# airl-iisc/MRFP

Measured on AMD Instinct MI355X. Metric: train images/sec, higher is better.
Workload: dtype bf16; 1 GPU; resnet-101 DeepLabV3+ + MRFP+ (HRFP+NP+ on, HRFP re-drawn every step), 768x768, 16 images/GPU, fwd+bwd+SGD, synthetic 19-class, random-init weights; global_batch=16, parallelism=dp1

## Files before the change

### include/mrfp_hip.h

```cpp
#ifndef MRFP_HIP_H
#define MRFP_HIP_H

#include <stdint.h>

#ifdef __cplusplus
extern "C" {
#endif

typedef enum { MRFP_F32 = 0, MRFP_BF16 = 1, MRFP_F16 = 2 } mrfp_dtype;

int mrfp_version(void);
const char* mrfp_last_error(void);

int64_t mrfp_stats_nslab(int64_t B, int64_t Ho);

int mrfp_stats_fwd(const void* x, int dtype, int64_t B, int64_t Ho, int64_t Wo, int64_t C,
                   int64_t Hs, int64_t Ws, const int32_t* tabH, const int32_t* tabW,
                   float* ws, void* stream);

int mrfp_stats_bwd(const void* dy, const void* x, const void* y, const float* mean,
                   const float* fA, const float* fS, int per_image, int dtype, int64_t B, int64_t Ho, int64_t Wo, int64_t C,
                   int64_t Hs, int64_t Ws, const int32_t* tabH, const int32_t* tabW,
                   float* ws, void* stream);
int mrfp_stats_bwd_mask(const void* dy, const void* x, const void* mask, const float* mean, int per_image, int dtype, int64_t B,
                        int64_t H, int64_t W, int64_t C, float* ws, void* stream);

int mrfp_bn_finalize(const float* ws, int64_t B, int64_t nslab, int64_t count, int64_t C,
                     const float* weight, const float* bias, float eps, float momentum,
                     float* running_mean, float* running_var,
                     float* mean, float* invstd, float* A, float* S, void* stream);
int mrfp_bn_eval_coef(int64_t C, const float* weight, const float* bias, const float* running_mean,
                      const float* running_var, float eps, float* A, float* S, void* stream);
int mrfp_bn_bwd_finalize(const float* ws, int64_t B, int64_t nslab, int64_t count, int64_t C,
                         const float* weight, const float* mean, const float* invstd,
                         float* dweight, float* dbias, float* P, float* Q, float* R, void* stream);

int mrfp_in_finalize(const float* ws, int64_t B, int64_t nslab, int64_t count, int64_t C,
                     const float* weight, const float* bias, float eps,
                     float* mean, float* invstd, float* A, float* S, void* stream);
int mrfp_in_bwd_finalize(const float* ws, int64_t B, int64_t nslab, int64_t count, int64_t C,
                         const float* weight, const float* mean, const float* invstd,
                         float* dweight, float* dbias, float* P, float* Q, float* R, void* stream);

int mrfp_np_finalize(const float* ws, int64_t B, int64_t nslab, int64_t count, int64_t C,
                     const float* alpha, const float* beta_noise,
                     float* mu, float* sigma, float* A, float* S, void* stream);
int mrfp_np_bwd_finalize(const float* ws, int64_t B, int64_t nslab, int64_t count, int64_t C,
                         const float* alpha, const float* beta_noise, const float* mu,
                         const float* sigma, float* Gtmp , float* K, void* stream);

int mrfp_mean_finalize(const float* ws, int64_t B, int64_t nslab, int64_t count, int64_t C,
                       float* tmp, void* out, int dtype, void* stream);

int mrfp_affine_fwd(const void* x, const void* res, void* y, int dtype,
                    int64_t B, int64_t Ho, int64_t Wo, int64_t C, int64_t Hs, int64_t Ws,
                    const int32_t* tabH, const int32_t* tabW,
                    const float* A, const float* S, int coef_per_image, int relu, void* stream);

int mrfp_affine_fwd_stats(const void* x, const void* res, void* y, int dtype, int64_t B, int64_t H, int64_t W, int64_t C,
                          const float* A, const float* S, int coef_per_image, int relu, float* ws, void* stream);
int mrfp_affine_bwd(const void* dy, const void* x, const void* y, void* dx, void* dres, int dtype,
                    int64_t B, int64_t Ho, int64_t Wo, int64_t C, int64_t Hs, int64_t Ws,
                    const int32_t* invH, const int32_t* invW,
                    const float* P, const float* Q, const float* R,
                    const float* fA, const float* fS, int coef_per_image, void* stream);
int mrfp_affine_fwd_relu_mask(const void* x, const void* res, void* y, void* mask, int dtype, int64_t B, int64_t H, int64_t W,
                              int64_t C, const float* A, const float* S, int coef_per_image, void* stream);
int mrfp_affine_bwd_mask(const void* dy, const void* x, const void* mask, void* dx, void* dres, int dtype, int64_t B, int64_t H,
                         int64_t W, int64_t C, const float* P, const float* Q, const float* R, int coef_per_image, void* stream);

int mrfp_copy_channels(const void* src, void* dst, int dtype, int64_t npix, int64_t C, int64_t ld_src, int64_t c0_src,
                       int64_t ld_dst, int64_t c0_dst, void* stream);

int mrfp_add(const void* a, const void* b, void* y, int dtype, int64_t n, void* stream);

int mrfp_bilinear_fwd(const void* x, const void* addend, void* y, int dtype,
                      int64_t B, int64_t Hi, int64_t Wi, int64_t Ho, int64_t Wo, int64_t C, int64_t ld_in,
                      void* stream);
int mrfp_bilinear_bwd(const void* dy, void* dx, int dtype,
                      int64_t B, int64_t Hi, int64_t Wi, int64_t Ho, int64_t Wo, int64_t C, int64_t ld_in,
                      void* stream);
int mrfp_bilinear_fwd_into(const void* x, void* y, int dtype, int64_t B, int64_t Hi, int64_t Wi, int64_t Ho, int64_t Wo,
                           int64_t C, int64_t ld_in, int64_t ld_out, void* stream);
int mrfp_bilinear_bwd_from(const void* dy, void* dx, int dtype, int64_t B, int64_t Hi, int64_t Wi, int64_t Ho, int64_t Wo,
                           int64_t C, int64_t ld_in, int64_t ld_dy, void* stream);

int mrfp_maxpool_fwd(const void* x, void* y, uint8_t* idx, int dtype,
                     int64_t B, int64_t H, int64_t W, int64_t C, void* stream);
int mrfp_maxpool_bwd(const void* dy, const uint8_t* idx, void* dx, int dtype,
                     int64_t B, int64_t H, int64_t W, int64_t C, void* stream);

int mrfp_maxpool_affine_fwd(const void* x, const float* A, const float* S, int coef_per_image, int relu, void* y, uint8_t* idx,
                            int dtype, int64_t B, int64_t H, int64_t W, int64_t C, void* stream);
int mrfp_pool_norm_bwd_stats(const void* dy, const uint8_t* idx, const void* x, const float* mean, const float* fA,
                             const float* fS, int coef_per_image, int relu, float* ws, int dtype,
                             int64_t B, int64_t H, int64_t W, int64_t C, void* stream);
int mrfp_pool_norm_bwd_apply(const void* dy, const uint8_t* idx, const void* x, const float* P, const float* Q, const float* R,
                             const float* fA, const float* fS, int coef_per_image, int relu, void* dx, int dtype,
                             int64_t B, int64_t H, int64_t W, int64_t C, void* stream);

int64_t mrfp_ce_nblocks(int64_t npix);
int mrfp_ce_fwd(const void* logits, const int64_t* target, int dtype, int64_t npix, int64_t C,
                int64_t ignore_index, float* ws, float* loss, void* stream);
int mrfp_ce_bwd(const void* logits, const int64_t* target, const float* loss, const float* gscale,
                void* dlogits, int dtype, int64_t npix, int64_t C, int64_t ignore_index, void* stream);

int mrfp_upsample_ce_fwd(const void* P, int64_t ld, const int64_t* target, int dtype, int64_t B, int64_t Hi, int64_t Wi,
                         int64_t H, int64_t W, int64_t C, int64_t ignore_index, float* ws, float* loss, void* stream);
int mrfp_upsample_ce_bwd(const void* P, int64_t ld, const int64_t* target, const float* loss, const float* gscale,
                         void* dlogits, int64_t Cd, int dtype, int64_t B, int64_t Hi, int64_t Wi, int64_t H, int64_t W,
                         int64_t C, int64_t ignore_index, void* stream);

typedef enum { MRFP_CE_MEAN = 0, MRFP_CE_SUM = 1, MRFP_CE_IMAGE_MEAN = 2 } mrfp_ce_mode;
int64_t mrfp_ce_w_nblocks(int64_t B, int64_t HW);
int64_t mrfp_ce_w_loss_floats(int64_t B, int mode);
int mrfp_ce_w_fwd(const void* logits, const int64_t* target, int dtype, int64_t B, int64_t HW, int64_t C,
                  int64_t ignore_index, const float* weight, int64_t wstride, float smoothing, int mode, float* ws,
                  float* loss, void* stream);
int mrfp_ce_w_bwd(const void* logits, const int64_t* target, const float* loss, const float* gscale, void* dlogits,
                  int dtype, int64_t B, int64_t HW, int64_t C, int64_t ignore_index, const float* weight, int64_t wstride,
                  float smoothing, int mode, void* stream);
int mrfp_upsample_ce_w_fwd(const void* P, int64_t ld, const int64_t* target, int dtype, int64_t B, int64_t Hi, int64_t Wi,
                           int64_t H, int64_t W, int64_t C, int64_t ignore_index, const float* weight, int64_t wstride,
                           float smoothing, int mode, float* ws, float* loss, void* stream);
int mrfp_upsample_ce_w_bwd(const void* P, int64_t ld, const int64_t* target, const float* loss, const float* gscale,
                           void* dlogits, int64_t Cd, int dtype, int64_t B, int64_t Hi, int64_t Wi, int64_t H, int64_t W,
                           int64_t C, int64_t ignore_index, const float* weight, int64_t wstride, float smoothing, int mode,
                           void* stream);

int mrfp_label_class_weights(const int64_t* target, int64_t B, int64_t HW, int64_t C, double upper_bound, int norm,
                             int batch, int64_t* counts_ws, float* weight_out, void* stream);

int64_t mrfp_relax_nblocks(int64_t B, int64_t H, int64_t W);
int mrfp_relax_labels(const int64_t* target, int64_t B, int64_t H, int64_t W, int64_t C, int64_t border, int strict_mask,
                      int32_t* words, int64_t* counts, void* stream);
int mrfp_multihot_pack(const uint8_t* multihot, int64_t B, int64_t HW, int64_t C, int32_t* words, int64_t* counts,
                       void* stream);
int mrfp_relax_word_counts(const int32_t* words, int64_t B, int64_t HW, int64_t C, int64_t* counts, void* stream);
int mrfp_relax_class_weights(const int64_t* counts, int64_t B, int64_t C, double upper_bound, int norm, int batch,
                             float* weight_out, void* stream);
int64_t mrfp_soft_nll_nblocks(int64_t B, int64_t HW);
int64_t mrfp_soft_nll_loss_floats(int64_t B);
int mrfp_soft_nll_fwd(const void* logits, const int32_t* words, int dtype, int64_t B, int64_t HW, int64_t C,
                      const float* weight, int64_t wstride, float* ws, float* loss, void* stream);
int mrfp_soft_nll_bwd(const void* logits, const int32_t* words, const float* loss, const float* gscale, void* dlogits,
                      int dtype, int64_t B, int64_t HW, int64_t C, const float* weight, int64_t wstride, void* stream);
int mrfp_upsample_soft_nll_fwd(const void* P, int64_t ld, const int32_t* words, int dtype, int64_t B, int64_t Hi, int64_t Wi,
                               int64_t H, int64_t W, int64_t C, const float* weight, int64_t wstride, float* ws, float* loss,
                               void* stream);
int mrfp_upsample_soft_nll_bwd(const void* P, int64_t ld, const int32_t* words, const float* loss, const float* gscale,
                               void* dlogits, int64_t Cd, int dtype, int64_t B, int64_t Hi, int64_t Wi, int64_t H, int64_t W,
                               int64_t C, const float* weight, int64_t wstride, void* stream);

int mrfp_argmax_hist(const void* logits, const int64_t* target, int dtype, int64_t npix, int64_t C,
                     int64_t* hist, uint8_t* pred, void* stream);

int mrfp_pack_weight(const float* w, void* wf, void* wd, int dtype, int64_t N, int64_t C, int64_t R, int64_t S,
                     int64_t Npad, int64_t Cpad, void* stream);
int mrfp_pack_weights_batched(const void* jobs, const int64_t* prefix, int64_t njobs, int64_t total, int dtype, void* stream);
int mrfp_conv_fwd(const void* x, const void* wpack, const float* bias, void* y, int dtype,
                  int64_t B, int64_t H, int64_t W, int64_t C, int64_t N, int64_t ldy, int64_t R, int64_t S,
                  int64_t Ho, int64_t Wo, int64_t stride, int64_t pad_h, int64_t pad_w, int64_t dil,
                  int64_t sstride, const void* addend, float* colstats, void* stream);
int mrfp_conv_fwd_act(const void* x, const void* wpack, const float* bias, void* y, int dtype,
                      int64_t B, int64_t H, int64_t W, int64_t C, int64_t N, int64_t ldy, int64_t R, int64_t S,
                      int64_t Ho, int64_t Wo, int64_t stride, int64_t pad_h, int64_t pad_w, int64_t dil,
                      int64_t sstride, const void* addend, int act, void* stream);
int mrfp_pack_weight_folded(const float* w, void* wf, const float* conv_bias, const float* bn_weight, const float* bn_bias,
                            const float* running_mean, const float* running_var, float eps, float* bias_out, int dtype,
                            int64_t N, int64_t C, int64_t R, int64_t S, int64_t Npad, int64_t Cpad, void* stream);
int mrfp_pack_weights_folded_batched(const void* jobs, const int64_t* prefix, int64_t njobs, int64_t total, int dtype, void* stream);
int mrfp_conv_stats_layout(int dtype, int64_t B, int64_t H, int64_t W, int64_t C, int64_t N, int64_t ldy, int64_t R, int64_t S,
                           int64_t Ho, int64_t Wo, int64_t stride, int64_t pad_h, int64_t pad_w, int64_t dil, int64_t sstride, int wstats,
                           int64_t* out);
int64_t mrfp_conv_stats_block_rows(int dtype, int64_t B, int64_t H, int64_t W, int64_t C, int64_t N, int64_t R, int64_t S, int64_t Ho,
                                   int64_t Wo, int64_t stride, int64_t pad_h, int64_t pad_w, int64_t dil, int64_t sstride);
int mrfp_conv_single_launch(int64_t B, int64_t image_bytes);
int mrfp_conv_fwd_wstats(const void* x, const void* wpack, const float* bias, void* y, int dtype,
                         int64_t B, int64_t H, int64_t W, int64_t C, int64_t N, int64_t ldy, int64_t R, int64_t S,
                         int64_t Ho, int64_t Wo, int64_t stride, int64_t pad_h, int64_t pad_w, int64_t dil,
                         const uint8_t* rowweight, float* colstats, void* stream);
int mrfp_conv_fwd_gated(const void* x, const void* wpack, const float* bias, void* y, int dtype,
                        int64_t B, int64_t H, int64_t W, int64_t C, int64_t N, int64_t ldy, int64_t R, int64_t S,
                        int64_t Ho, int64_t Wo, int64_t stride, int64_t pad_h, int64_t pad_w, int64_t dil,
                        int64_t sstride, const void* addend, const void* addend_mask, void* stream);
int mrfp_conv_fwd_lowrank(const void* x, const void* wpack, const float* bias, void* y, int dtype,
                          int64_t B, int64_t H, int64_t W, int64_t C, int64_t N, int64_t ldy, int64_t R, int64_t S,
                          int64_t Ho, int64_t Wo, int64_t stride, int64_t pad_h, int64_t pad_w, int64_t dil,
                          int64_t sstride, const void* addend, float* colstats, const void* lr_x, const void* lr_w, int64_t lr_k,
                          void* stream);
int mrfp_conv_lowrank_ok(int dtype, int64_t B, int64_t H, int64_t W, int64_t C, int64_t N, int64_t ldy, int64_t R, int64_t S,
                         int64_t Ho, int64_t Wo, int64_t stride, int64_t pad_h, int64_t pad_w, int64_t dil);
int mrfp_debug_clock_stamps(int family, uint64_t* out, int64_t n);
int64_t mrfp_conv_wgrad_ws_bytes(int64_t M, int64_t N, int64_t Q);
int mrfp_conv_wgrad(const void* x, const void* dy, float* dw, void* ws, int dtype,
                    int64_t B, int64_t H, int64_t W, int64_t C, int64_t Ctrue, int64_t N, int64_t ldn,
                    int64_t R, int64_t S, int64_t Ho, int64_t Wo, int64_t stride, int64_t pad_h, int64_t pad_w,
                    int64_t dil, void* stream);
int64_t mrfp_conv_wgrad_group_max(void);
int64_t mrfp_conv_wgrad_grouped_ws_bytes(int64_t M, int64_t N, int64_t Q, int64_t count);
int mrfp_conv_wgrad_plan(int dtype, int64_t B, int64_t H, int64_t W, int64_t C, int64_t N, int64_t ldn, int64_t R, int64_t S, int64_t Ho,
                         int64_t Wo, int64_t stride, int64_t pad_h, int64_t pad_w, int64_t dil, int64_t count, int64_t* out);
int mrfp_conv_wgrad_grouped(const void* const* xs, const void* const* dys, float* const* dws, int64_t count, void* ws, int dtype,
                            int64_t B, int64_t H, int64_t W, int64_t C, int64_t Ctrue, int64_t N, int64_t ldn,
                            int64_t R, int64_t S, int64_t Ho, int64_t Wo, int64_t stride, int64_t pad_h, int64_t pad_w,
                            int64_t dil, void* stream);
int mrfp_nchw_to_nhwc_pad(const float* x, void* y, int dtype, int64_t B, int64_t C, int64_t H, int64_t W,
                          int64_t Cpad, void* stream);

int mrfp_sgd_step(float* p, const float* g, float* m, int64_t n, float lr, float momentum,
                  float weight_decay, float gscale, int first, void* stream);

int64_t mrfp_grad_check_nblocks(int64_t n);
int mrfp_grad_check(const float* g, int64_t n, float gscale, void* ws, void* state, int dynamic, float growth,
                    float backoff, int growth_interval, float max_norm, void* stream);
int mrfp_sgd_step_checked(float* p, const float* g, float* m, int64_t n, float lr, float momentum,
                          float weight_decay, const void* state, void* stream);

int64_t mrfp_group_moments_ws_bytes(int64_t B, int64_t HW, int64_t C);
int mrfp_group_moments(const void* a, const void* b, float* M, float* sum_a, void* ws, int dtype, int64_t B, int64_t HW,
                       int64_t C, void* stream);
int mrfp_group_apply(const void* x, const float* Wm, const void* z, const float* Vm, const float* shift, void* y, int dtype,
                     int64_t B, int64_t HW, int64_t C, void* stream);
int mrfp_group_isqrt_fwd(const float* cov, float* wm, int64_t n, int T, void* stream);
int mrfp_group_isqrt_bwd(const float* cov, const float* dwm, float* dcov, int64_t n, int T, void* stream);

int64_t mrfp_fourier_spectrum_bytes(int64_t B, int64_t H, int64_t W, int64_t C);
int64_t mrfp_fourier_stored_bins(int64_t H, int64_t W, float radius, int high);
int mrfp_fourier_mix(const void* x, void* y, const int64_t* perm, void* S, void* S3, float* ratio, int load_ratio,
                     const void* twH, const void* twW, int dtype, int64_t B, int64_t H, int64_t W, int64_t C,
                     float radius, float lam, int high, void* stream);

int mrfp_resample_u8(const void* src, void* dst, int64_t Hin, int64_t Win, int64_t Hout, int64_t Wout, int64_t C,
                     const int32_t* bounds, const int32_t* coefs, int ksize, int vertical, int flip, void* stream);
int mrfp_input_assemble(const void* img, const void* lab, const int32_t* ytab, const int32_t* xtab, int64_t Hs, int64_t Ws,
                        int64_t Hl, int64_t Wl, int flip, int pad_x, int pad_y, int x1, int y1, int64_t Hc, int64_t Wc, int ignore,
                        float* out_img, void* out_u8, int64_t* out_lab, void* stream);
int mrfp_box_blur3_u8(const void* src, void* dst, int64_t H, int64_t W, int64_t C, int64_t ww, int64_t fw, int vertical,
// ... 53 lines not shown
```

### mrfp_amd/csrc/affine.hip

```cpp
#include "common.hpp"

namespace mrfp {

template <typename T, int VEC, bool RESIZE>
__global__ __launch_bounds__(kThreads) void affine_fwd_kernel(const T* __restrict__ x, const T* __restrict__ res,
                                                              T* __restrict__ y, RowGeom g, int ly,
                                                              const float* __restrict__ A, const float* __restrict__ S,
                                                              int coef_per_image, int relu, uint8_t* __restrict__ mask_out) {
    const int b = blockIdx.x / ly, j = blockIdx.x % ly;
    const Lanes L = make_lanes(g.C, VEC);
    const int t = threadIdx.x;
    const int tcol = t % L.colthreads, trow = t / L.colthreads;
    if (trow >= L.rowthreads) return;
    const size_t cbase = (size_t)(coef_per_image ? b : 0) * g.C;
    for (int cv = tcol; cv < L.lpr; cv += kThreads) {
        float a[VEC], s[VEC];
#pragma unroll
        for (int i = 0; i < VEC; ++i) { a[i] = 1.f; s[i] = 0.f; }
        if (A) load_coef<VEC>(A + cbase + (size_t)cv * VEC, a);
        if (S) load_coef<VEC>(S + cbase + (size_t)cv * VEC, s);
        for (int oh = j; oh < g.Ho; oh += ly) {
            const int ih = RESIZE ? g.tabH[oh] : oh;
            const T* xl = x ? x + ((size_t)b * g.Hs + ih) * g.Ws * g.C + (size_t)cv * VEC : nullptr;
            const size_t dl = ((size_t)b * g.Ho + oh) * g.Wo * g.C + (size_t)cv * VEC;
// ... 159 lines not shown
            load_coef<VEC>(fA + cbase + (size_t)cv * VEC, fa);
            load_coef<VEC>(fS + cbase + (size_t)cv * VEC, fs);
        }
        if (KR < 0) {
            for (int ih = j; ih < g.Hs; ih += ly) {
                const size_t sl = ((size_t)b * g.Hs + ih) * g.Ws * g.C + (size_t)cv * VEC;
                for (int iw0 = trow; iw0 < g.Ws; iw0 += 4 * L.rowthreads) {
                    VecT<T, VEC> dr[4], xr[4], yr[4];
                    unsigned mb[4] = {0u, 0u, 0u, 0u};
#pragma unroll
                    for (int u = 0; u < 4; ++u) {
                        const int iw = min(iw0 + u * L.rowthreads, g.Ws - 1);
                        dr[u] = load_raw_nt<T, VEC>(dy + sl + (size_t)iw * g.C);
                        if (x && (Q || remask)) xr[u] = load_raw_nt<T, VEC>(x + sl + (size_t)iw * g.C);
                        if constexpr (YM) mb[u] = reinterpret_cast<const uint8_t*>(y)[(sl + (size_t)iw * g.C) >> 3];
                        else if (y) yr[u] = load_raw_nt<T, VEC>(y + sl + (size_t)iw * g.C);
                    }
#pragma unroll
                    for (int u = 0; u < 4; ++u) {
                        const int iw = iw0 + u * L.rowthreads;
                        if (iw >= g.Ws) continue;
                        float dv[VEC], xv[VEC], o[VEC];
                        cvt_f<T, VEC>(dr[u], dv);
#pragma unroll
                        for (int i = 0; i < VEC; ++i) xv[i] = 0.f;
                        if (x && (Q || remask)) cvt_f<T, VEC>(xr[u], xv);
                        if constexpr (YM) {
#pragma unroll
                            for (int i = 0; i < VEC; ++i) dv[i] = ((mb[u] >> i) & 1u) ? dv[i] : 0.f;
                        } else if (y) {
                            float yv[VEC];
                            cvt_f<T, VEC>(yr[u], yv);
#pragma unroll
                            for (int i = 0; i < VEC; ++i) dv[i] = yv[i] > 0.f ? dv[i] : 0.f;
                        } else if (remask) {
#pragma unroll
                            for (int i = 0; i < VEC; ++i) dv[i] = (xv[i] * fa[i] + fs[i] > 0.f) ? dv[i] : 0.f;
                        }
                        if (dres) store_f<T, VEC>(dres + sl + (size_t)iw * g.C, dv);
#pragma unroll
                        for (int i = 0; i < VEC; ++i) o[i] = p[i] * dv[i] + (q[i] * xv[i] + r[i]);
                        store_f<T, VEC>(dx + sl + (size_t)iw * g.C, o);
                    }
                }
            }
            continue;
        }
        if (KR >= 0)
        for (int ih = j; ih < g.Hs; ih += ly) {
            const int oh0 = invH ? invH[2 * ih] : ih, oh1 = invH ? invH[2 * ih + 1] : ih + 1;
            const size_t sl = ((size_t)b * g.Hs + ih) * g.Ws * g.C + (size_t)cv * VEC;
            const bool need_x = x && (Q || remask);
            auto slow_pixel = [&](int iw, int ow0, int ow1) {
                float acc[VEC], xv[VEC];
#pragma unroll
                for (int i = 0; i < VEC; ++i) { acc[i] = 0.f; xv[i] = 0.f; }
                const float n = (float)((oh1 - oh0) * (ow1 - ow0));
                if (need_x) load_f<T, VEC>(x + sl + (size_t)iw * g.C, xv);
                for (int oh = oh0; oh < oh1; ++oh) {
                    const size_t dl = ((size_t)b * g.Ho + oh) * g.Wo * g.C + (size_t)cv * VEC;
                    for (int ow = ow0; ow < ow1; ++ow) {
                        float dv[VEC];
                        load_f<T, VEC>(dy + dl + (size_t)ow * g.C, dv);
                        if (y) {
                            float yv[VEC];
                            load_f<T, VEC>(y + dl + (size_t)ow * g.C, yv);
#pragma unroll
                            for (int i = 0; i < VEC; ++i) dv[i] = yv[i] > 0.f ? dv[i] : 0.f;
                        } else if (remask) {
#pragma unroll
                            for (int i = 0; i < VEC; ++i) dv[i] = (xv[i] * fa[i] + fs[i] > 0.f) ? dv[i] : 0.f;
                        }
                        if (dres) store_f<T, VEC>(dres + dl + (size_t)ow * g.C, dv);
#pragma unroll
                        for (int i = 0; i < VEC; ++i) acc[i] += dv[i];
                    }
                }
                float o[VEC];
                if (x && Q) {
#pragma unroll
                    for (int i = 0; i < VEC; ++i) o[i] = p[i] * acc[i] + n * (q[i] * xv[i] + r[i]);
                } else {
#pragma unroll
                    for (int i = 0; i < VEC; ++i) o[i] = p[i] * acc[i] + n * r[i];
                }
                store_f<T, VEC>(dx + sl + (size_t)iw * g.C, o);
            };
            if constexpr (KR > 0) {
                constexpr int U = KR == 1 ? 4 : 1;
                for (int iw0 = trow; iw0 < g.Ws; iw0 += U * L.rowthreads) {
                    int iwu[U], ow0[U], ow1[U];
                    bool fast = oh1 - oh0 <= KR;
#pragma unroll
                    for (int u = 0; u < U; ++u) {
                        iwu[u] = min(iw0 + u * L.rowthreads, g.Ws - 1);
                        ow0[u] = invW[2 * iwu[u]];
                        ow1[u] = invW[2 * iwu[u] + 1];
                        fast = fast && ow1[u] - ow0[u] <= KR;
                    }
                    if (!fast) {
#pragma unroll
                        for (int u = 0; u < U; ++u)
                            if (iw0 + u * L.rowthreads < g.Ws) slow_pixel(iwu[u], ow0[u], ow1[u]);
                        continue;
                    }
                    VecT<T, VEC> xr[U], dr[U][KR * KR];
#pragma unroll
                    for (int u = 0; u < U; ++u) {
                        if (need_x) xr[u] = KR == 1 ? load_raw_nt<T, VEC>(x + sl + (size_t)iwu[u] * g.C) : load_raw<T, VEC>(x + sl + (size_t)iwu[u] * g.C);
#pragma unroll
                        for (int kh = 0; kh < KR; ++kh) {
                            const int oh = min(oh0 + kh, g.Ho - 1);
                            const size_t dl = ((size_t)b * g.Ho + oh) * g.Wo * g.C + (size_t)cv * VEC;
#pragma unroll
                            for (int kw = 0; kw < KR; ++kw)
                                dr[u][kh * KR + kw] = KR == 1 ? load_raw_nt<T, VEC>(dy + dl + (size_t)min(ow0[u] + kw, g.Wo - 1) * g.C)
                                                              : load_raw<T, VEC>(dy + dl + (size_t)min(ow0[u] + kw, g.Wo - 1) * g.C);
                        }
                    }
#pragma unroll
                    for (int u = 0; u < U; ++u) {
                        if (iw0 + u * L.rowthreads >= g.Ws) continue;
                        float acc[VEC], xv[VEC], keep[VEC];
#pragma unroll
                        for (int i = 0; i < VEC; ++i) { acc[i] = 0.f; xv[i] = 0.f; }
                        if (need_x) cvt_f<T, VEC>(xr[u], xv);
#pragma unroll
                        for (int i = 0; i < VEC; ++i) keep[i] = (!remask || xv[i] * fa[i] + fs[i] > 0.f) ? 1.f : 0.f;
#pragma unroll
                        for (int kh = 0; kh < KR; ++kh)
#pragma unroll
                            for (int kw = 0; kw < KR; ++kw) {
                                const bool have = oh0 + kh < oh1 && ow0[u] + kw < ow1[u];
                                float dv[VEC];
                                cvt_f<T, VEC>(dr[u][kh * KR + kw], dv);
#pragma unroll
                                for (int i = 0; i < VEC; ++i) acc[i] += (have && keep[i] != 0.f) ? dv[i] : 0.f;
                            }
                        const float n = (float)((oh1 - oh0) * (ow1[u] - ow0[u]));
                        float o[VEC];
                        if (x && Q) {
#pragma unroll
                            for (int i = 0; i < VEC; ++i) o[i] = p[i] * acc[i] + n * (q[i] * xv[i] + r[i]);
                        } else {
#pragma unroll
                            for (int i = 0; i < VEC; ++i) o[i] = p[i] * acc[i] + n * r[i];
                        }
                        store_f<T, VEC>(dx + sl + (size_t)iwu[u] * g.C, o);
                    }
                }
            } else {
                for (int iw = trow; iw < g.Ws; iw += L.rowthreads)
                    slow_pixel(iw, invW ? invW[2 * iw] : iw, invW ? invW[2 * iw + 1] : iw + 1);
            }
        }
    }
}

template <typename T, int VEC>
__global__ __launch_bounds__(kThreads) void add_kernel(const T* __restrict__ a, const T* __restrict__ b,
                                                       T* __restrict__ y, int64_t nvec) {
    for (int64_t i = (int64_t)blockIdx.x * kThreads + threadIdx.x; i < nvec; i += (int64_t)gridDim.x * kThreads) {
        float u[VEC], v[VEC];
        load_f<T, VEC>(a + i * VEC, u);
        load_f<T, VEC>(b + i * VEC, v);
#pragma unroll
        for (int k = 0; k < VEC; ++k) u[k] += v[k];
        store_f<T, VEC>(y + i * VEC, u);
    }
}

template <typename T, int VEC>
__global__ __launch_bounds__(kThreads) void copy_channels_kernel(const T* __restrict__ src, T* __restrict__ dst, int64_t npix,
                                                                  int C, int lds, int c0s, int ldd, int c0d) {
    const int cpr = C / VEC;
    const int64_t total = npix * cpr;
    const int64_t stride = (int64_t)gridDim.x * kThreads;
    for (int64_t i0 = (int64_t)blockIdx.x * kThreads + threadIdx.x; i0 < total; i0 += 4 * stride) {
        VecT<T, VEC> r[4];
#pragma unroll
        for (int u = 0; u < 4; ++u) {
            const int64_t i = min(i0 + u * stride, total - 1);
            const int64_t pix = i / cpr;
            const int ch = (int)(i - pix * cpr);
            r[u] = load_raw<T, VEC>(src + pix * lds + c0s + ch * VEC);
        }
#pragma unroll
        for (int u = 0; u < 4; ++u) {
            const int64_t i = i0 + u * stride;
            if (i < total) {
                const int64_t pix = i / cpr;
                const int ch = (int)(i - pix * cpr);
                *reinterpret_cast<VecT<T, VEC>*>(dst + pix * ldd + c0d + ch * VEC) = r[u];
            }
        }
    }
}

template <typename T>
static int launch_copy_channels(const void* src, void* dst, int64_t npix, int64_t C, int64_t lds, int64_t c0s, int64_t ldd,
                                int64_t c0d, hipStream_t st) {
    const int full = FullVec<T>::value;
    const bool vec_ok = C % full == 0 && lds % full == 0 && ldd % full == 0 && c0s % full == 0 && c0d % full == 0 &&
                        aligned16(src) && aligned16(dst);
    const int64_t total = npix * (vec_ok ? C / full : C);
    int64_t blocks = (total + 4 * kThreads - 1) / (4 * kThreads);
    if (blocks > 16384) blocks = 16384;
    if (blocks < 1) blocks = 1;
    MRFP_LAUNCH_VEC(vec_ok, (copy_channels_kernel<T, FullVec<T>::value>), (copy_channels_kernel<T, 1>), dim3((unsigned)blocks), st,
                    (const T*)src, (T*)dst, npix, (int)C, (int)lds, (int)c0s, (int)ldd, (int)c0d);
    return 0;
}

template <typename T>
static int launch_affine_fwd(const void* x, const void* res, void* y, int64_t B, int64_t Ho, int64_t Wo, int64_t C,
                             int64_t Hs, int64_t Ws, const int32_t* tabH, const int32_t* tabW, const float* A,
                             const float* S, int cpi, int relu, hipStream_t st, uint8_t* mask_out = nullptr) {
    RowGeom g{(int)B, (int)Ho, (int)Wo, (int)C, (int)Hs, (int)Ws, tabH, tabW};
    const int ly = lines_per_image(B, Ho);
    dim3 grid((unsigned)(B * ly));
    const bool vec_ok = pick_vec<T>(C) > 1 && (!x || aligned16(x)) && aligned16(y) && (!res || aligned16(res)) &&
                        (!A || aligned16(A)) && (!S || aligned16(S));
    if (mask_out && !(vec_ok && FullVec<T>::value == 8)) { set_error("affine_fwd_mask: 16-bit activations with C %% 8 == 0, 16-byte aligned"); return -1; }
    const bool resize = tabH != nullptr || tabW != nullptr;
    if (resize && !(tabH && tabW)) { set_error("affine_fwd: both index tables or none"); return -1; }
    auto launch = [&](auto rs) {
        constexpr bool RS = decltype(rs)::value != 0;
        MRFP_LAUNCH_VEC(vec_ok, (affine_fwd_kernel<T, FullVec<T>::value, RS>), (affine_fwd_kernel<T, 1, RS>), grid, st, (const T*)x,
                        (const T*)res, (T*)y, g, ly, A, S, cpi, relu, mask_out);
        return 0;
    };
    return resize ? launch(Int<1>{}) : launch(Int<0>{});
}

template <typename T>
static int launch_affine_bwd(const void* dy, const void* x, const void* y, void* dx, void* dres, int64_t B, int64_t Ho,
                             int64_t Wo, int64_t C, int64_t Hs, int64_t Ws, const int32_t* invH, const int32_t* invW,
                             const float* P, const float* Q, const float* R, const float* fA, const float* fS, int cpi,
                             hipStream_t st, bool ymask = false) {
    RowGeom g{(int)B, (int)Ho, (int)Wo, (int)C, (int)Hs, (int)Ws, nullptr, nullptr};
    const int ly = lines_per_image(B, Hs);
    dim3 grid((unsigned)(B * ly));
    const bool vec_ok = pick_vec<T>(C) > 1 && aligned16(dy) && aligned16(dx) && (!x || aligned16(x)) &&
                        (!y || aligned16(y)) && (!dres || aligned16(dres)) && (!P || aligned16(P)) &&
                        (!Q || aligned16(Q)) && (!R || aligned16(R)) && (!fA || (aligned16(fA) && aligned16(fS)));
    int kr = 0;
    if (invH && invW && !y && !dres) {
        const int64_t kh = (Ho + Hs - 1) / Hs, kw = (Wo + Ws - 1) / Ws;
        const int64_t k = kh > kw ? kh : kw;
        kr = k <= 3 ? (int)k : 0;
    }
    const bool identity = !invH && !invW;
    if (ymask) {
        if constexpr (FullVec<T>::value == 8) {
            if (!(vec_ok && identity && y)) { set_error("affine_bwd_mask: 16-bit activations, C %% 8 == 0, identity geometry"); return -1; }
            hipLaunchKernelGGL((affine_bwd_kernel<T, 8, -1, true>), grid, dim3(kThreads), 0, st, (const T*)dy, (const T*)x, (const T*)y,
                               (T*)dx, (T*)dres, g, ly, invH, invW, P, Q, R, fA, fS, cpi);
            MRFP_LAUNCH_CHECK();
            return 0;
        } else {
            set_error("affine_bwd_mask: 16-bit activations only");
            return -1;
        }
    }
    auto launch = [&](auto k) {
        constexpr int KR = decltype(k)::value;
        MRFP_LAUNCH_VEC(vec_ok, (affine_bwd_kernel<T, FullVec<T>::value, KR>), (affine_bwd_kernel<T, 1, KR>), grid, st, (const T*)dy,
                        (const T*)x, (const T*)y, (T*)dx, (T*)dres, g, ly, invH, invW, P, Q, R, fA, fS, cpi);
        return 0;
    };
    if (identity) return launch(Int<-1>{});
    if (kr == 1) return launch(Int<1>{});
    if (kr == 2) return launch(Int<2>{});
    if (kr == 3) return launch(Int<3>{});
    return launch(Int<0>{});
}

template <typename T>
static int launch_add(const void* a, const void* b, void* y, int64_t n, hipStream_t st) {
    const int full = FullVec<T>::value;
    const bool vec_ok = n % full == 0 && aligned16(a) && aligned16(b) && aligned16(y);
    const int64_t nvec = vec_ok ? n / full : n;
    int64_t blocks = (nvec + kThreads - 1) / kThreads;
    if (blocks > 4096) blocks = 4096;
    if (blocks < 1) blocks = 1;
    MRFP_LAUNCH_VEC(vec_ok, (add_kernel<T, FullVec<T>::value>), (add_kernel<T, 1>), dim3((unsigned)blocks), st, (const T*)a,
                    (const T*)b, (T*)y, nvec);
    return 0;
}

}

using namespace mrfp;

extern "C" {

int mrfp_affine_fwd(const void* x, const void* res, void* y, int dtype, int64_t B, int64_t Ho, int64_t Wo, int64_t C,
                    int64_t Hs, int64_t Ws, const int32_t* tabH, const int32_t* tabW, const float* A, const float* S,
                    int coef_per_image, int relu, void* stream) {
    MRFP_CHECK(y && B > 0 && Ho > 0 && Wo > 0 && C > 0 && Hs > 0 && Ws > 0, "affine_fwd: bad arguments");
    MRFP_CHECK(x || S, "affine_fwd: neither x nor S given");
    MRFP_CHECK((tabH && tabW) || (Hs == Ho && Ws == Wo), "affine_fwd: resize geometry without index tables");
    hipStream_t st = (hipStream_t)stream;
    return by_dtype(dtype, "affine_fwd", [&](auto t) {
        using T = typename decltype(t)::type;
        return launch_affine_fwd<T>(x, res, y, B, Ho, Wo, C, Hs, Ws, tabH, tabW, A, S, coef_per_image, relu, st);
    });
}

int mrfp_affine_fwd_stats(const void* x, const void* res, void* y, int dtype, int64_t B, int64_t H, int64_t W, int64_t C,
                          const float* A, const float* S, int coef_per_image, int relu, float* ws, void* stream) {
    MRFP_CHECK(x && y && ws && B > 0 && H > 0 && W > 0 && C > 0, "affine_fwd_stats: bad arguments");
    hipStream_t st = (hipStream_t)stream;
    RowGeom g{(int)B, (int)H, (int)W, (int)C, (int)H, (int)W, nullptr, nullptr};
    const int ly = lines_per_image(B, H);
    const bool al = aligned16(x) && aligned16(y) && (!res || aligned16(res)) && (!A || aligned16(A)) && (!S || aligned16(S));
    return by_dtype(dtype, "affine_fwd_stats", [&](auto t) {
        using T = typename decltype(t)::type;
        MRFP_DISPATCH_VEC(T, C, al, affine_fwd_stats_kernel, dim3((unsigned)(B * ly)), st, (const T*)x, (const T*)res, (T*)y, g, ly, A, S,
                          coef_per_image, relu, ws);
        return 0;
    });
}

int mrfp_affine_bwd(const void* dy, const void* x, const void* y, void* dx, void* dres, int dtype, int64_t B,
                    int64_t Ho, int64_t Wo, int64_t C, int64_t Hs, int64_t Ws, const int32_t* invH, const int32_t* invW,
                    const float* P, const float* Q, const float* R, const float* fA, const float* fS, int coef_per_image,
                    void* stream) {
    MRFP_CHECK(!fA == !fS, "affine_bwd: fA and fS go together");
    MRFP_CHECK(dy && dx && B > 0 && Ho > 0 && Wo > 0 && C > 0 && Hs > 0 && Ws > 0, "affine_bwd: bad arguments");
    MRFP_CHECK((invH && invW) || (Hs == Ho && Ws == Wo), "affine_bwd: resize geometry without inverse tables");
    MRFP_CHECK(!dres || (!invH && !invW), "affine_bwd: dres is not supported behind a resize");
    hipStream_t st = (hipStream_t)stream;
    return by_dtype(dtype, "affine_bwd", [&](auto t) {
        using T = typename decltype(t)::type;
        return launch_affine_bwd<T>(dy, x, y, dx, dres, B, Ho, Wo, C, Hs, Ws, invH, invW, P, Q, R, fA, fS, coef_per_image, st);
    });
}

int mrfp_affine_fwd_relu_mask(const void* x, const void* res, void* y, void* mask, int dtype, int64_t B, int64_t H, int64_t W,
                              int64_t C, const float* A, const float* S, int coef_per_image, void* stream) {
    MRFP_CHECK(x && y && mask && A && S && B > 0 && H > 0 && W > 0 && C > 0 && (C & 7) == 0, "affine_fwd_relu_mask: bad arguments");
    hipStream_t st = (hipStream_t)stream;
    return by_dtype16(dtype, "affine_fwd_relu_mask", [&](auto t) {
        using T = typename decltype(t)::type;
        return launch_affine_fwd<T>(x, res, y, B, H, W, C, H, W, nullptr, nullptr, A, S, coef_per_image, 1, st, (uint8_t*)mask);
    });
}

int mrfp_affine_bwd_mask(const void* dy, const void* x, const void* mask, void* dx, void* dres, int dtype, int64_t B, int64_t H,
                         int64_t W, int64_t C, const float* P, const float* Q, const float* R, int coef_per_image, void* stream) {
    MRFP_CHECK(dy && dx && mask && B > 0 && H > 0 && W > 0 && C > 0 && (C & 7) == 0, "affine_bwd_mask: bad arguments");
    hipStream_t st = (hipStream_t)stream;
    return by_dtype16(dtype, "affine_bwd_mask", [&](auto t) {
        using T = typename decltype(t)::type;
        return launch_affine_bwd<T>(dy, x, mask, dx, dres, B, H, W, C, H, W, nullptr, nullptr, P, Q, R, nullptr, nullptr, coef_per_image, st, true);
    });
}

int mrfp_copy_channels(const void* src, void* dst, int dtype, int64_t npix, int64_t C, int64_t ld_src, int64_t c0_src,
                       int64_t ld_dst, int64_t c0_dst, void* stream) {
    MRFP_CHECK(src && dst && npix > 0 && C > 0 && c0_src >= 0 && c0_dst >= 0 && c0_src + C <= ld_src && c0_dst + C <= ld_dst,
               "copy_channels: bad arguments");
    hipStream_t st = (hipStream_t)stream;
    return by_dtype(dtype, "copy_channels", [&](auto t) {
        using T = typename decltype(t)::type;
        return launch_copy_channels<T>(src, dst, npix, C, ld_src, c0_src, ld_dst, c0_dst, st);
    });
}

int mrfp_add(const void* a, const void* b, void* y, int dtype, int64_t n, void* stream) {
    MRFP_CHECK(a && b && y && n > 0, "add: bad arguments");
    hipStream_t st = (hipStream_t)stream;
    return by_dtype(dtype, "add", [&](auto t) {
        using T = typename decltype(t)::type;
        return launch_add<T>(a, b, y, n, st);
    });
}

}
```

### mrfp_amd/csrc/common.hpp

```cpp
#pragma once
#include <hip/hip_runtime.h>
#include <hip/hip_bf16.h>
#include <stdint.h>
#include <stdio.h>
#include <stdarg.h>
#include <stdlib.h>
#include <type_traits>
#include "../../include/mrfp_hip.h"

namespace mrfp {

void set_error(const char* fmt, ...);

#define MRFP_CHECK(cond, ...)                      \
    do {                                           \
        if (!(cond)) {                             \
            ::mrfp::set_error(__VA_ARGS__);        \
            return -1;                             \
        }                                          \
    } while (0)

#define MRFP_LAUNCH_CHECK()                                                   \
    do {                                                                      \
        hipError_t e__ = hipGetLastError();                                   \
        if (e__ != hipSuccess) {                                              \
            ::mrfp::set_error("%s:%d launch failed: %s", __FILE__, __LINE__,  \
                              hipGetErrorString(e__));                        \
            return -2;                                                        \
        }                                                                     \
    } while (0)

typedef __hip_bfloat16 bf16;
typedef _Float16 f16;

__device__ __forceinline__ float to_f(float v) { return v; }
__device__ __forceinline__ float to_f(bf16 v) { return __bfloat162float(v); }
__device__ __forceinline__ float to_f(f16 v) { return (float)v; }
template <typename T> __device__ __forceinline__ T from_f(float v);
template <> __device__ __forceinline__ float from_f<float>(float v) { return v; }
template <> __device__ __forceinline__ bf16 from_f<bf16>(float v) { return __float2bfloat16(v); }
template <> __device__ __forceinline__ f16 from_f<f16>(float v) { return (f16)v; }
template <int ACT> __device__ __forceinline__ float act_f(float v) {
    if constexpr (ACT == 1) return fmaxf(v, 0.f);
    else if constexpr (ACT == 2) return fminf(fmaxf(v, 0.f), 6.f);
    else return v;
}

template <typename T, int VEC> struct alignas(sizeof(T) * VEC) VecT { T v[VEC]; };

template <typename T> struct FullVec { static constexpr int value = 16 / sizeof(T); };

template <typename T, int VEC>
__device__ __forceinline__ void load_f(const T* p, float (&out)[VEC]) {
    VecT<T, VEC> t = *reinterpret_cast<const VecT<T, VEC>*>(p);
#pragma unroll
    for (int i = 0; i < VEC; ++i) out[i] = to_f(t.v[i]);
}
template <typename T, int VEC>
__device__ __forceinline__ void store_f(T* p, const float (&in)[VEC]) {
    VecT<T, VEC> t;
#pragma unroll
    for (int i = 0; i < VEC; ++i) t.v[i] = from_f<T>(in[i]);
    *reinterpret_cast<VecT<T, VEC>*>(p) = t;
}
template <typename T, int VEC>
__device__ __forceinline__ VecT<T, VEC> load_raw(const T* p) { return *reinterpret_cast<const VecT<T, VEC>*>(p); }
#ifndef MRFP_NT
#define MRFP_NT 1
#endif
template <typename T, int VEC>
__device__ __forceinline__ VecT<T, VEC> load_raw_nt(const T* p) {
    if constexpr (MRFP_NT != 0 && sizeof(T) * VEC == 16) {
        typedef unsigned __attribute__((ext_vector_type(4))) nt_u32x4;
        const nt_u32x4 v = __builtin_nontemporal_load(reinterpret_cast<const nt_u32x4*>(p));
        return __builtin_bit_cast(VecT<T, VEC>, v);
    } else {
        return *reinterpret_cast<const VecT<T, VEC>*>(p);
    }
}
template <typename T, int VEC>
__device__ __forceinline__ void cvt_f(const VecT<T, VEC>& t, float (&out)[VEC]) {
#pragma unroll
    for (int i = 0; i < VEC; ++i) out[i] = to_f(t.v[i]);
}

template <int VEC>
__device__ __forceinline__ void load_coef(const float* p, float (&out)[VEC]) {
    VecT<float, VEC> t = *reinterpret_cast<const VecT<float, VEC>*>(p);
#pragma unroll
    for (int i = 0; i < VEC; ++i) out[i] = t.v[i];
}

__device__ __forceinline__ float wave_sum(float v) {
#pragma unroll
    for (int o = 32; o > 0; o >>= 1) v += __shfl_xor(v, o, 64);
    return v;
}
__device__ __forceinline__ double wave_sum(double v) {
#pragma unroll
    for (int o = 32; o > 0; o >>= 1) v += __shfl_xor(v, o, 64);
    return v;
}

struct RowGeom {
    int B, Ho, Wo, C, Hs, Ws;
    const int32_t* tabH;
    const int32_t* tabW;
};

constexpr int kThreads = 256;
constexpr int kCUs = 256;

struct Lanes {
    int lpr;
    int colthreads;
    int rowthreads;
};
__host__ __device__ inline Lanes make_lanes(int C, int VEC) {
    Lanes l;
    l.lpr = C / VEC;
    l.colthreads = l.lpr < kThreads ? l.lpr : kThreads;
    l.rowthreads = kThreads / l.colthreads;
    return l;
}

inline bool aligned16(const void* p) { return (reinterpret_cast<uintptr_t>(p) & 15) == 0; }

inline int env_switch(const char* name, int dflt) {
    const char* e = getenv(name);
    return e ? atoi(e) : dflt;
}

template <typename T> inline int pick_vec(int64_t C) {
    const int full = FullVec<T>::value;
    return (C % full == 0) ? full : 1;
}

template <typename T> struct Tag { using type = T; };
template <int V> using Int = std::integral_constant<int, V>;

inline bool dtype_known(int dtype) { return dtype == MRFP_F32 || dtype == MRFP_BF16 || dtype == MRFP_F16; }
inline int dtype_bytes(int dtype) { return dtype == MRFP_F32 ? 4 : 2; }

template <typename F> inline int by_dtype16(int dtype, const char* who, F&& f) {
    if (dtype == MRFP_BF16) return f(Tag<bf16>{});
    if (dtype == MRFP_F16) return f(Tag<f16>{});
    MRFP_CHECK(false, "%s: 16-bit activations only (dtype %d)", who, dtype);
}
template <typename F> inline int by_dtype(int dtype, const char* who, F&& f) {
    if (dtype == MRFP_F32) return f(Tag<float>{});
    if (dtype == MRFP_BF16) return f(Tag<bf16>{});
    if (dtype == MRFP_F16) return f(Tag<f16>{});
    MRFP_CHECK(false, "%s: unknown dtype %d", who, dtype);
}

#define MRFP_LAUNCH_VEC(vec, KFULL, KONE, grid, st, ...)                                \
    do {                                                                                \
        if (vec) hipLaunchKernelGGL(KFULL, grid, dim3(kThreads), 0, st, __VA_ARGS__);   \
        else hipLaunchKernelGGL(KONE, grid, dim3(kThreads), 0, st, __VA_ARGS__);        \
        MRFP_LAUNCH_CHECK();                                                            \
    } while (0)
#define MRFP_DISPATCH_VEC(T, C, ok, KERNEL, grid, st, ...) \
    MRFP_LAUNCH_VEC(pick_vec<T>(C) > 1 && (ok), (KERNEL<T, FullVec<T>::value>), (KERNEL<T, 1>), grid, st, __VA_ARGS__)

inline int lines_per_image(int64_t B, int64_t Ho) {
    static const int set = env_switch("MRFP_ROW_BLOCKS", 2048);
    const int total = set < 64 ? 2048 : set;
    int64_t cap = total / (B > 0 ? B : 1);
    if (cap < 1) cap = 1;
    if (Ho <= cap) return (int)Ho;
    const int64_t per = (Ho + cap - 1) / cap;
    return (int)((Ho + per - 1) / per);
}

}
```

### mrfp_amd/csrc/resize_pool.hip

```cpp
#include "common.hpp"

namespace mrfp {

__device__ __forceinline__ float ac_scale(int in, int out) { return out > 1 ? (float)(in - 1) / (float)(out - 1) : 0.f; }
struct Tap { int i0, i1; float l0, l1; };
__device__ __forceinline__ Tap ac_tap(float scale, int dst, int in) {
    const float src = scale * (float)dst;
    Tap t;
    t.i0 = (int)src;
    t.i1 = t.i0 + (t.i0 < in - 1 ? 1 : 0);
    t.l1 = src - (float)t.i0;
    t.l0 = 1.f - t.l1;
    return t;
}

template <typename T, int VEC>
__global__ __launch_bounds__(kThreads) void bilinear_fwd_kernel(const T* __restrict__ x, const T* __restrict__ addend,
                                                                T* __restrict__ y, int B, int Hi, int Wi, int Ho, int Wo,
                                                                int C, int ldi, int ly, int ldo) {
    const int b = blockIdx.x / ly, j = blockIdx.x % ly;
    const Lanes L = make_lanes(C, VEC);
    const int t = threadIdx.x;
    const int tcol = t % L.colthreads, trow = t / L.colthreads;
    if (trow >= L.rowthreads) return;
    const float sh = ac_scale(Hi, Ho), sw = ac_scale(Wi, Wo);
    for (int cv = tcol; cv < L.lpr; cv += kThreads) {
        for (int oh = j; oh < Ho; oh += ly) {
            const Tap th = ac_tap(sh, oh, Hi);
            const T* r0 = x + ((size_t)b * Hi + th.i0) * Wi * ldi + (size_t)cv * VEC;
            const T* r1 = x + ((size_t)b * Hi + th.i1) * Wi * ldi + (size_t)cv * VEC;
            const size_t dl = ((size_t)b * Ho + oh) * Wo * ldo + (size_t)cv * VEC;
            for (int ow0 = trow; ow0 < Wo; ow0 += 4 * L.rowthreads) {
                Tap tw[4];
                VecT<T, VEC> ra[4], rb[4], rc[4], rd[4], re[4];
#pragma unroll
                for (int u = 0; u < 4; ++u) {
                    const int ow = min(ow0 + u * L.rowthreads, Wo - 1);
                    tw[u] = ac_tap(sw, ow, Wi);
                    ra[u] = load_raw<T, VEC>(r0 + (size_t)tw[u].i0 * ldi);
                    rb[u] = load_raw<T, VEC>(r0 + (size_t)tw[u].i1 * ldi);
                    rc[u] = load_raw<T, VEC>(r1 + (size_t)tw[u].i0 * ldi);
                    rd[u] = load_raw<T, VEC>(r1 + (size_t)tw[u].i1 * ldi);
                    if (addend) re[u] = load_raw<T, VEC>(addend + dl + (size_t)ow * ldo);
                }
#pragma unroll
                for (int u = 0; u < 4; ++u) {
                    const int ow = ow0 + u * L.rowthreads;
                    if (ow >= Wo) continue;
                    float a[VEC], bb[VEC], c[VEC], d[VEC], o[VEC];
                    cvt_f<T, VEC>(ra[u], a);
                    cvt_f<T, VEC>(rb[u], bb);
                    cvt_f<T, VEC>(rc[u], c);
                    cvt_f<T, VEC>(rd[u], d);
#pragma unroll
                    for (int i = 0; i < VEC; ++i)
                        o[i] = th.l0 * (tw[u].l0 * a[i] + tw[u].l1 * bb[i]) + th.l1 * (tw[u].l0 * c[i] + tw[u].l1 * d[i]);
                    if (addend) {
                        float e[VEC];
                        cvt_f<T, VEC>(re[u], e);
#pragma unroll
                        for (int i = 0; i < VEC; ++i) o[i] += e[i];
                    }
                    store_f<T, VEC>(y + dl + (size_t)ow * ldo, o);
                }
            }
        }
    }
}

__device__ __forceinline__ float ac_weight(float scale, int dst, int in, int src) {
    const Tap t = ac_tap(scale, dst, in);
    return (t.i0 == src ? t.l0 : 0.f) + (t.i1 == src ? t.l1 : 0.f);
}
__device__ __forceinline__ void ac_range(int in, int out, int src, int& lo, int& hi) {
    if (in <= 1 || out <= 1) { lo = 0; hi = out - 1; return; }
    const long long a = in - 1, b = out - 1;
    lo = src >= 1 ? (int)(((long long)(src - 1) * b) / a) : 0;
    hi = (int)(((long long)(src + 1) * b + a - 1) / a);
    if (lo < 0) lo = 0;
    if (hi > out - 1) hi = out - 1;
}

template <typename T, int VEC, int KW, int KN = 0>
__global__ __launch_bounds__(kThreads) void bilinear_bwd_kernel(const T* __restrict__ dy, T* __restrict__ dx, int B,
                                                                int Hi, int Wi, int Ho, int Wo, int C, int ldi, int ly, int ldd) {
    const int b = blockIdx.x / ly, j = blockIdx.x % ly;
    const Lanes L = make_lanes(C, VEC);
    const int t = threadIdx.x;
    const int tcol = t % L.colthreads, trow = t / L.colthreads;
    if (trow >= L.rowthreads) return;
    const float sh = ac_scale(Hi, Ho), sw = ac_scale(Wi, Wo);
    for (int cv = tcol; cv < L.lpr; cv += kThreads) {
        for (int ih = j; ih < Hi; ih += ly) {
            int oh0, oh1;
            ac_range(Hi, Ho, ih, oh0, oh1);
            for (int iw = trow; iw < Wi; iw += L.rowthreads) {
                int ow0, ow1;
                ac_range(Wi, Wo, iw, ow0, ow1);
                float acc[VEC];
#pragma unroll
                for (int i = 0; i < VEC; ++i) acc[i] = 0.f;
                bool windowed = false;
                if constexpr (KW > 0 && KN > 0) {
                    const int kf = ac_weight(sw, ow0, Wi, iw) != 0.f ? 0 : 1;
                    float wn[KN > 0 ? KN : 1];
#pragma unroll
                    for (int k = 0; k < KN; ++k) wn[k] = (ow0 + kf + k <= ow1) ? ac_weight(sw, ow0 + kf + k, Wi, iw) : 0.f;
                    bool more = false;
#pragma unroll
                    for (int k = KN; k < KW; ++k) more = more || (ow0 + kf + k <= ow1 && ac_weight(sw, ow0 + kf + k, Wi, iw) != 0.f);
                    if (__builtin_amdgcn_ballot_w64(more) == 0) {
                        windowed = true;
                        for (int oh = oh0; oh <= oh1; ++oh) {
                            const float wh = ac_weight(sh, oh, Hi, ih);
                            if (wh == 0.f) continue;
                            const T* dl = dy + ((size_t)b * Ho + oh) * Wo * ldd + (size_t)cv * VEC;
                            VecT<T, VEC> r[KN > 0 ? KN : 1];
#pragma unroll
                            for (int k = 0; k < KN; ++k) r[k] = load_raw<T, VEC>(dl + (size_t)min(ow0 + kf + k, ow1) * ldd);
#pragma unroll
                            for (int k = 0; k < KN - 1; ++k) {
                                const float w = wh * wn[k];
                                float dv[VEC];
                                cvt_f<T, VEC>(r[k], dv);
#pragma unroll
                                for (int i = 0; i < VEC; ++i) acc[i] += (wn[k] != 0.f) ? w * dv[i] : 0.f;
                            }
                            if (wn[KN - 1] != 0.f) {
                                const float w = wh * wn[KN - 1];
                                float dv[VEC];
                                cvt_f<T, VEC>(r[KN - 1], dv);
#pragma unroll
                                for (int i = 0; i < VEC; ++i) acc[i] += w * dv[i];
                            }
                        }
                    }
                }
                if (windowed) {
                } else if (KW > 0) {
                    float ww[KW > 0 ? KW : 1];
#pragma unroll
                    for (int k = 0; k < KW; ++k) ww[k] = (ow0 + k <= ow1) ? ac_weight(sw, ow0 + k, Wi, iw) : 0.f;
                    for (int oh = oh0; oh <= oh1; ++oh) {
                        const float wh = ac_weight(sh, oh, Hi, ih);
                        if (wh == 0.f) continue;
                        const T* dl = dy + ((size_t)b * Ho + oh) * Wo * ldd + (size_t)cv * VEC;
                        VecT<T, VEC> r[KW > 0 ? KW : 1];
#pragma unroll
                        for (int k = 0; k < KW; ++k) r[k] = load_raw<T, VEC>(dl + (size_t)min(ow0 + k, ow1) * ldd);
#pragma unroll
                        for (int k = 0; k < KW; ++k) {
                            const float w = wh * ww[k];
                            float dv[VEC];
                            cvt_f<T, VEC>(r[k], dv);
#pragma unroll
                            for (int i = 0; i < VEC; ++i) acc[i] += (ww[k] != 0.f) ? w * dv[i] : 0.f;
                        }
                    }
                } else {
                    for (int oh = oh0; oh <= oh1; ++oh) {
                        const float wh = ac_weight(sh, oh, Hi, ih);
                        if (wh == 0.f) continue;
                        const T* dl = dy + ((size_t)b * Ho + oh) * Wo * ldd + (size_t)cv * VEC;
                        for (int ow = ow0; ow <= ow1; ++ow) {
                            const float w = wh * ac_weight(sw, ow, Wi, iw);
                            if (w == 0.f) continue;
                            float dv[VEC];
                            load_f<T, VEC>(dl + (size_t)ow * ldd, dv);
#pragma unroll
                            for (int i = 0; i < VEC; ++i) acc[i] += w * dv[i];
                        }
                    }
                }
                store_f<T, VEC>(dx + (((size_t)b * Hi + ih) * Wi + iw) * ldi + (size_t)cv * VEC, acc);
            }
        }
    }
}

template <typename T, int VEC>
__global__ __launch_bounds__(kThreads) void maxpool_fwd_kernel(const T* __restrict__ x, T* __restrict__ y,
                                                               uint8_t* __restrict__ idx, int B, int H, int W, int Ho,
                                                               int Wo, int C, int ly, const float* __restrict__ A,
                                                               const float* __restrict__ S, int coef_per_image, int relu) {
    const int b = blockIdx.x / ly, j = blockIdx.x % ly;
    const Lanes L = make_lanes(C, VEC);
    const int t = threadIdx.x;
    const int tcol = t % L.colthreads, trow = t / L.colthreads;
    if (trow >= L.rowthreads) return;
    const bool aff = A != nullptr;
    const size_t cbase = (size_t)(coef_per_image ? b : 0) * C;
    for (int cv = tcol; cv < L.lpr; cv += kThreads) {
        float ca[VEC], cs[VEC];
#pragma unroll
        for (int i = 0; i < VEC; ++i) { ca[i] = 1.f; cs[i] = 0.f; }
        if (aff) {
            load_coef<VEC>(A + cbase + (size_t)cv * VEC, ca);
            load_coef<VEC>(S + cbase + (size_t)cv * VEC, cs);
        }
        for (int oh = j; oh < Ho; oh += ly) {
            for (int op = trow; 2 * op < Wo; op += L.rowthreads) {
                const int ow0 = 2 * op;
                float best[2][VEC];
                uint8_t bi[2][VEC];
#pragma unroll
                for (int q = 0; q < 2; ++q)
#pragma unroll
                    for (int i = 0; i < VEC; ++i) { best[q][i] = -INFINITY; bi[q][i] = 0; }
                VecT<T, VEC> win[15];
#pragma unroll
                for (int r = 0; r < 3; ++r) {
                    const int ih = min(max(2 * oh - 1 + r, 0), H - 1);
#pragma unroll
                    for (int s = 0; s < 5; ++s) {
                        const int iw = min(max(2 * ow0 - 1 + s, 0), W - 1);
                        win[r * 5 + s] = load_raw<T, VEC>(x + (((size_t)b * H + ih) * W + iw) * C + (size_t)cv * VEC);
// ... 51 lines not shown
    const int iw0 = 2 * ip;
    const int owa = min(ip, Wo - 1), owb = min(ip + 1, Wo - 1);
    VecT<T, VEC> dr[2][2];
    VecT<uint8_t, VEC> pr[2][2];
#pragma unroll
    for (int rr = 0; rr < 2; ++rr) {
        if (rr < nrow) {
            const size_t ol = ((size_t)b * Ho + (oh0 + rr)) * Wo * C + (size_t)cv * VEC;
            dr[rr][0] = load_raw<T, VEC>(dy + ol + (size_t)owa * C);
            dr[rr][1] = load_raw<T, VEC>(dy + ol + (size_t)owb * C);
            pr[rr][0] = *reinterpret_cast<const VecT<uint8_t, VEC>*>(idx + ol + (size_t)owa * C);
            pr[rr][1] = *reinterpret_cast<const VecT<uint8_t, VEC>*>(idx + ol + (size_t)owb * C);
        }
    }
#pragma unroll
    for (int q = 0; q < 2; ++q)
#pragma unroll
        for (int i = 0; i < VEC; ++i) acc[q][i] = 0.f;
#pragma unroll
    for (int rr = 0; rr < 2; ++rr) {
        if (rr >= nrow) continue;
        const int oh = oh0 + rr;
        const int r = ih - (2 * oh - 1);
#pragma unroll
        for (int cc = 0; cc < 2; ++cc) {
            const int ow = ip + cc;
            float dv[VEC];
            cvt_f<T, VEC>(dr[rr][cc], dv);
#pragma unroll
            for (int q = 0; q < 2; ++q) {
                const int sft = iw0 + q - (2 * ow - 1);
                const bool in_win = ow < Wo && sft >= 0 && sft <= 2 && iw0 + q < W;
                const uint8_t want = (uint8_t)(r * 3 + sft);
#pragma unroll
                for (int i = 0; i < VEC; ++i) acc[q][i] += (in_win && pr[rr][cc].v[i] == want) ? dv[i] : 0.f;
            }
        }
    }
}

template <typename T, int VEC>
__global__ __launch_bounds__(kThreads) void maxpool_bwd_kernel(const T* __restrict__ dy, const uint8_t* __restrict__ idx,
                                                               T* __restrict__ dx, int B, int H, int W, int Ho, int Wo,
                                                               int C, int ly) {
    const int b = blockIdx.x / ly, j = blockIdx.x % ly;
    const Lanes L = make_lanes(C, VEC);
    const int t = threadIdx.x;
    const int tcol = t % L.colthreads, trow = t / L.colthreads;
    if (trow >= L.rowthreads) return;
    for (int cv = tcol; cv < L.lpr; cv += kThreads) {
        for (int ih = j; ih < H; ih += ly) {
            for (int ip = trow; 2 * ip < W; ip += L.rowthreads) {
                float acc[2][VEC];
                pool_grad_pair<T, VEC>(dy, idx, b, ih, ip, W, Ho, Wo, C, cv, acc);
#pragma unroll
                for (int q = 0; q < 2; ++q)
                    if (2 * ip + q < W) store_f<T, VEC>(dx + (((size_t)b * H + ih) * W + 2 * ip + q) * C + (size_t)cv * VEC, acc[q]);
            }
        }
    }
}

template <typename T, int VEC, int PASS>
__global__ __launch_bounds__(kThreads) void pool_norm_bwd_kernel(const T* __restrict__ dy, const uint8_t* __restrict__ idx,
                                                                 const T* __restrict__ x, T* __restrict__ dx,
                                                                 float* __restrict__ ws, int B, int H, int W, int Ho, int Wo,
                                                                 int C, int ly, const float* __restrict__ mean,
                                                                 const float* __restrict__ fA, const float* __restrict__ fS,
                                                                 const float* __restrict__ P, const float* __restrict__ Q,
                                                                 const float* __restrict__ R, int coef_per_image, int relu) {
    __shared__ float sm[PASS == 0 ? kThreads * 2 * VEC : 1];
    const int b = blockIdx.x / ly, j = blockIdx.x % ly;
    const Lanes L = make_lanes(C, VEC);
    const int t = threadIdx.x;
    const int tcol = t % L.colthreads, trow = t / L.colthreads;
    const bool active = trow < L.rowthreads;
    const size_t cbase = (size_t)(coef_per_image ? b : 0) * C;
    for (int cv0 = 0; cv0 < L.lpr; cv0 += kThreads) {
        const int cv = cv0 + tcol;
        const bool on = active && cv < L.lpr;
        float s[VEC], q2[VEC], mu[VEC], fa[VEC], fs[VEC], p[VEC], qq[VEC], r[VEC];
#pragma unroll
        for (int i = 0; i < VEC; ++i) { s[i] = 0.f; q2[i] = 0.f; mu[i] = 0.f; fa[i] = 0.f; fs[i] = 1.f; p[i] = 1.f; qq[i] = 0.f; r[i] = 0.f; }
        if (on) {
            const size_t co = cbase + (size_t)cv * VEC;
            if (relu) { load_coef<VEC>(fA + co, fa); load_coef<VEC>(fS + co, fs); }
            if (PASS == 0) {
                load_coef<VEC>(mean + co, mu);
            } else {
                load_coef<VEC>(P + co, p);
                load_coef<VEC>(Q + co, qq);
                load_coef<VEC>(R + co, r);
            }
            for (int ih = j; ih < H; ih += ly) {
                const size_t sl = ((size_t)b * H + ih) * W * C + (size_t)cv * VEC;
                for (int ip = trow; 2 * ip < W; ip += L.rowthreads) {
                    const int iw1 = min(2 * ip + 1, W - 1);
                    VecT<T, VEC> xr[2];
                    if (PASS == 0) {
                        xr[0] = load_raw<T, VEC>(x + sl + (size_t)(2 * ip) * C);
                        xr[1] = load_raw<T, VEC>(x + sl + (size_t)iw1 * C);
                    } else {
                        xr[0] = load_raw_nt<T, VEC>(x + sl + (size_t)(2 * ip) * C);
                        xr[1] = load_raw_nt<T, VEC>(x + sl + (size_t)iw1 * C);
                    }
                    float acc[2][VEC];
                    pool_grad_pair<T, VEC>(dy, idx, b, ih, ip, W, Ho, Wo, C, cv, acc);
#pragma unroll
                    for (int qd = 0; qd < 2; ++qd) {
                        const bool inside = 2 * ip + qd < W;
                        float xv[VEC], o[VEC];
                        cvt_f<T, VEC>(xr[qd], xv);
#pragma unroll
                        for (int i = 0; i < VEC; ++i) {
                            const float gate = xv[i] * fa[i] + fs[i];
                            const float d = (inside && gate > 0.f) ? to_f(from_f<T>(acc[qd][i])) : 0.f;
                            if (PASS == 0) {
                                s[i] += d;
                                q2[i] += d * (xv[i] - mu[i]);
                            } else {
                                o[i] = p[i] * d + (qq[i] * xv[i] + r[i]);
                            }
                        }
                        if (PASS == 1 && inside) store_f<T, VEC>(dx + sl + (size_t)(2 * ip + qd) * C, o);
                    }
                }
            }
        }
        if constexpr (PASS == 0) {
            __syncthreads();
#pragma unroll
            for (int i = 0; i < VEC; ++i) {
                sm[(t * 2 + 0) * VEC + i] = s[i];
                sm[(t * 2 + 1) * VEC + i] = q2[i];
            }
            __syncthreads();
            float* out = ws + (size_t)blockIdx.x * 2 * C;
            const int nout = L.colthreads * 2 * VEC;
            for (int o = t; o < nout; o += kThreads) {
                const int oc = o / (2 * VEC), rest = o % (2 * VEC);
                if (cv0 + oc < L.lpr) {
                    float a = 0.f;
                    for (int rr = 0; rr < L.rowthreads; ++rr) a += sm[((rr * L.colthreads + oc) * 2) * VEC + rest];
                    const int stat = rest / VEC, i = rest % VEC;
                    out[(size_t)stat * C + (size_t)(cv0 + oc) * VEC + i] = a;
                }
            }
        }
    }
}

template <typename T>
static int do_bilinear_fwd(const void* x, const void* addend, void* y, int64_t B, int64_t Hi, int64_t Wi, int64_t Ho,
                           int64_t Wo, int64_t C, int64_t ldi, hipStream_t st, int64_t ldo = 0) {
    const int ly = lines_per_image(B, Ho);
    if (ldo <= 0) ldo = C;
    const bool ok = aligned16(x) && aligned16(y) && (!addend || aligned16(addend)) && ldi % FullVec<T>::value == 0 &&
                    ldo % FullVec<T>::value == 0;
    MRFP_DISPATCH_VEC(T, C, ok, bilinear_fwd_kernel, dim3((unsigned)(B * ly)), st, (const T*)x, (const T*)addend, (T*)y,
                      (int)B, (int)Hi, (int)Wi, (int)Ho, (int)Wo, (int)C, (int)ldi, ly, (int)ldo);
    return 0;
}
template <typename T>
static int do_bilinear_bwd(const void* dy, void* dx, int64_t B, int64_t Hi, int64_t Wi, int64_t Ho, int64_t Wo,
                           int64_t C, int64_t ldi, hipStream_t st, int64_t ldd = 0) {
    const int ly = lines_per_image(B, Hi);
    if (ldd <= 0) ldd = C;
    const bool ok = aligned16(dy) && aligned16(dx) && ldi % FullVec<T>::value == 0 && ldd % FullVec<T>::value == 0;
    const int64_t kw = (Wi > 1 && Wo > 1) ? (2 * (Wo - 1) + (Wi - 1) - 1) / (Wi - 1) + 2 : (int64_t)1 << 30;
    const dim3 grid((unsigned)(B * ly));
    const bool vec = ok && pick_vec<T>(C) > 1;
    auto launch = [&](auto kwv, auto knv) {
        constexpr int KW = decltype(kwv)::value, KN = decltype(knv)::value;
        MRFP_LAUNCH_VEC(vec, (bilinear_bwd_kernel<T, FullVec<T>::value, KW, KN>), (bilinear_bwd_kernel<T, 1, KW>), grid, st, (const T*)dy,
                        (T*)dx, (int)B, (int)Hi, (int)Wi, (int)Ho, (int)Wo, (int)C, (int)ldi, ly, (int)ldd);
        return 0;
    };
    static const int win = env_switch("MRFP_BILINEAR_WINDOW", 1);
    if (kw <= 4) return launch(Int<4>{}, Int<0>{});
    if (kw == 7 && win) return launch(Int<8>{}, Int<5>{});
    if (kw <= 8) return launch(Int<8>{}, Int<0>{});
    if (kw == 11 && win) return launch(Int<12>{}, Int<9>{});
    if (kw <= 12) return launch(Int<12>{}, Int<0>{});
    return launch(Int<0>{}, Int<0>{});
}
template <typename T>
static int do_maxpool_fwd(const void* x, void* y, uint8_t* idx, int64_t B, int64_t H, int64_t W, int64_t C,
                          hipStream_t st, const float* A = nullptr, const float* S = nullptr, int per_image = 0,
                          int relu = 0) {
    const int Ho = (int)((H + 2 - 3) / 2 + 1), Wo = (int)((W + 2 - 3) / 2 + 1);
    const int ly = lines_per_image(B, Ho);
    const bool ok = aligned16(x) && aligned16(y) && ((uintptr_t)idx % FullVec<T>::value) == 0 &&
                    (!A || (aligned16(A) && aligned16(S) && C % 4 == 0));
    MRFP_DISPATCH_VEC(T, C, ok, maxpool_fwd_kernel, dim3((unsigned)(B * ly)), st, (const T*)x, (T*)y, idx, (int)B, (int)H,
                      (int)W, Ho, Wo, (int)C, ly, A, S, per_image, relu);
    return 0;
}
template <typename T>
static int do_pool_norm_bwd(int pass, const void* dy, const uint8_t* idx, const void* x, void* dx, float* ws, int64_t B,
                            int64_t H, int64_t W, int64_t C, const float* mean, const float* fA, const float* fS,
                            const float* P, const float* Q, const float* R, int per_image, int relu, hipStream_t st) {
    const int Ho = (int)((H + 2 - 3) / 2 + 1), Wo = (int)((W + 2 - 3) / 2 + 1);
    const int ly = lines_per_image(B, H);
    bool ok = aligned16(dy) && aligned16(x) && (!dx || aligned16(dx)) && ((uintptr_t)idx % FullVec<T>::value) == 0 && C % 4 == 0;
    for (const float* c : {mean, fA, fS, P, Q, R}) ok = ok && (!c || aligned16(c));
    const dim3 grid((unsigned)(B * ly));
    const bool vec = pick_vec<T>(C) > 1 && ok;
    auto launch = [&](auto pv) {
        constexpr int PASS = decltype(pv)::value;
        MRFP_LAUNCH_VEC(vec, (pool_norm_bwd_kernel<T, FullVec<T>::value, PASS>), (pool_norm_bwd_kernel<T, 1, PASS>), grid, st, (const T*)dy,
                        idx, (const T*)x, (T*)dx, ws, (int)B, (int)H, (int)W, Ho, Wo, (int)C, ly, mean, fA, fS, P, Q, R, per_image, relu);
        return 0;
    };
    return pass == 0 ? launch(Int<0>{}) : launch(Int<1>{});
}
template <typename T>
static int do_maxpool_bwd(const void* dy, const uint8_t* idx, void* dx, int64_t B, int64_t H, int64_t W, int64_t C,
                          hipStream_t st) {
    const int Ho = (int)((H + 2 - 3) / 2 + 1), Wo = (int)((W + 2 - 3) / 2 + 1);
    const int ly = lines_per_image(B, H);
    const bool ok = aligned16(dy) && aligned16(dx) && ((uintptr_t)idx % FullVec<T>::value) == 0;
    MRFP_DISPATCH_VEC(T, C, ok, maxpool_bwd_kernel, dim3((unsigned)(B * ly)), st, (const T*)dy, idx, (T*)dx, (int)B, (int)H,
                      (int)W, Ho, Wo, (int)C, ly);
    return 0;
}

}

using namespace mrfp;

extern "C" {

int mrfp_bilinear_fwd(const void* x, const void* addend, void* y, int dtype, int64_t B, int64_t Hi, int64_t Wi,
                      int64_t Ho, int64_t Wo, int64_t C, int64_t ld_in, void* stream) {
    MRFP_CHECK(x && y && B > 0 && Hi > 0 && Wi > 0 && Ho > 0 && Wo > 0 && C > 0 && ld_in >= C, "bilinear_fwd: bad arguments");
    return by_dtype(dtype, "bilinear_fwd", [&](auto t) {
        using T = typename decltype(t)::type;
        return do_bilinear_fwd<T>(x, addend, y, B, Hi, Wi, Ho, Wo, C, ld_in, (hipStream_t)stream);
    });
}
int mrfp_bilinear_bwd(const void* dy, void* dx, int dtype, int64_t B, int64_t Hi, int64_t Wi, int64_t Ho, int64_t Wo,
                      int64_t C, int64_t ld_in, void* stream) {
    MRFP_CHECK(dy && dx && B > 0 && Hi > 0 && Wi > 0 && Ho > 0 && Wo > 0 && C > 0 && ld_in >= C, "bilinear_bwd: bad arguments");
    return by_dtype(dtype, "bilinear_bwd", [&](auto t) {
        using T = typename decltype(t)::type;
        return do_bilinear_bwd<T>(dy, dx, B, Hi, Wi, Ho, Wo, C, ld_in, (hipStream_t)stream);
    });
}
int mrfp_bilinear_fwd_into(const void* x, void* y, int dtype, int64_t B, int64_t Hi, int64_t Wi, int64_t Ho, int64_t Wo,
                           int64_t C, int64_t ld_in, int64_t ld_out, void* stream) {
    MRFP_CHECK(x && y && B > 0 && Hi > 0 && Wi > 0 && Ho > 0 && Wo > 0 && C > 0 && ld_in >= C && ld_out >= C, "bilinear_fwd_into: bad arguments");
    return by_dtype(dtype, "bilinear_fwd_into", [&](auto t) {
        using T = typename decltype(t)::type;
        return do_bilinear_fwd<T>(x, nullptr, y, B, Hi, Wi, Ho, Wo, C, ld_in, (hipStream_t)stream, ld_out);
    });
}
int mrfp_bilinear_bwd_from(const void* dy, void* dx, int dtype, int64_t B, int64_t Hi, int64_t Wi, int64_t Ho, int64_t Wo,
                           int64_t C, int64_t ld_in, int64_t ld_dy, void* stream) {
    MRFP_CHECK(dy && dx && B > 0 && Hi > 0 && Wi > 0 && Ho > 0 && Wo > 0 && C > 0 && ld_in >= C && ld_dy >= C, "bilinear_bwd_from: bad arguments");
    return by_dtype(dtype, "bilinear_bwd_from", [&](auto t) {
        using T = typename decltype(t)::type;
        return do_bilinear_bwd<T>(dy, dx, B, Hi, Wi, Ho, Wo, C, ld_in, (hipStream_t)stream, ld_dy);
    });
}
int mrfp_maxpool_fwd(const void* x, void* y, uint8_t* idx, int dtype, int64_t B, int64_t H, int64_t W, int64_t C,
                     void* stream) {
    MRFP_CHECK(x && y && idx && B > 0 && H > 0 && W > 0 && C > 0, "maxpool_fwd: bad arguments");
    return by_dtype(dtype, "maxpool_fwd", [&](auto t) {
        using T = typename decltype(t)::type;
        return do_maxpool_fwd<T>(x, y, idx, B, H, W, C, (hipStream_t)stream);
    });
}
int mrfp_maxpool_affine_fwd(const void* x, const float* A, const float* S, int coef_per_image, int relu, void* y, uint8_t* idx,
                            int dtype, int64_t B, int64_t H, int64_t W, int64_t C, void* stream) {
    MRFP_CHECK(x && A && S && y && idx && B > 0 && H > 0 && W > 0 && C > 0, "maxpool_affine_fwd: bad arguments");
    return by_dtype(dtype, "maxpool_affine_fwd", [&](auto t) {
        using T = typename decltype(t)::type;
        return do_maxpool_fwd<T>(x, y, idx, B, H, W, C, (hipStream_t)stream, A, S, coef_per_image, relu);
    });
}
int mrfp_pool_norm_bwd_stats(const void* dy, const uint8_t* idx, const void* x, const float* mean, const float* fA,
                             const float* fS, int coef_per_image, int relu, float* ws, int dtype, int64_t B, int64_t H,
                             int64_t W, int64_t C, void* stream) {
    MRFP_CHECK(dy && idx && x && mean && ws && (!relu || (fA && fS)) && B > 0 && H > 0 && W > 0 && C > 0,
               "pool_norm_bwd_stats: bad arguments");
    return by_dtype(dtype, "pool_norm_bwd_stats", [&](auto t) {
        using T = typename decltype(t)::type;
        return do_pool_norm_bwd<T>(0, dy, idx, x, nullptr, ws, B, H, W, C, mean, fA, fS, nullptr, nullptr, nullptr, coef_per_image, relu,
                                   (hipStream_t)stream);
    });
}
int mrfp_pool_norm_bwd_apply(const void* dy, const uint8_t* idx, const void* x, const float* P, const float* Q, const float* R,
                             const float* fA, const float* fS, int coef_per_image, int relu, void* dx, int dtype, int64_t B,
                             int64_t H, int64_t W, int64_t C, void* stream) {
    MRFP_CHECK(dy && idx && x && P && Q && R && dx && (!relu || (fA && fS)) && B > 0 && H > 0 && W > 0 && C > 0,
               "pool_norm_bwd_apply: bad arguments");
    return by_dtype(dtype, "pool_norm_bwd_apply", [&](auto t) {
        using T = typename decltype(t)::type;
        return do_pool_norm_bwd<T>(1, dy, idx, x, dx, nullptr, B, H, W, C, nullptr, fA, fS, P, Q, R, coef_per_image, relu,
                                   (hipStream_t)stream);
    });
}
int mrfp_maxpool_bwd(const void* dy, const uint8_t* idx, void* dx, int dtype, int64_t B, int64_t H, int64_t W,
                     int64_t C, void* stream) {
    MRFP_CHECK(dy && dx && idx && B > 0 && H > 0 && W > 0 && C > 0, "maxpool_bwd: bad arguments");
    return by_dtype(dtype, "maxpool_bwd", [&](auto t) {
        using T = typename decltype(t)::type;
        return do_maxpool_bwd<T>(dy, idx, dx, B, H, W, C, (hipStream_t)stream);
    });
}

}
```

### mrfp_amd/csrc/stats.hip

```cpp
#include "common.hpp"

namespace mrfp {

static thread_local char g_err[512] = "";
void set_error(const char* fmt, ...) {
    va_list ap;
    va_start(ap, fmt);
    vsnprintf(g_err, sizeof(g_err), fmt, ap);
    va_end(ap);
}

template <typename T, int VEC, int MODE, bool RESIZE, bool YM = false>
__global__ __launch_bounds__(kThreads) void stats_kernel(const T* __restrict__ x, const T* __restrict__ dy,
                                                         const T* __restrict__ y, const float* __restrict__ mean,
                                                         const float* __restrict__ fA, const float* __restrict__ fS,
                                                         int per_image, RowGeom g, int ly, float* __restrict__ ws) {
    __shared__ float sm[kThreads * 2 * VEC];
    const int b = blockIdx.x / ly, j = blockIdx.x % ly;
    const Lanes L = make_lanes(g.C, VEC);
    const int t = threadIdx.x;
    const int tcol = t % L.colthreads, trow = t / L.colthreads;
    const bool active = trow < L.rowthreads;
    float* out = ws + (size_t)blockIdx.x * 2 * g.C;

    for (int cv0 = 0; cv0 < L.lpr; cv0 += kThreads) {
        const int cv = cv0 + tcol;
        const bool on = active && cv < L.lpr;
        float s[VEC], q[VEC], mu[VEC], fa[VEC], fs[VEC];
#pragma unroll
        for (int i = 0; i < VEC; ++i) { s[i] = 0.f; q[i] = 0.f; mu[i] = 0.f; fa[i] = 0.f; fs[i] = 1.f; }
        if (MODE == 1 && on) {
            const size_t co = (size_t)(per_image ? b : 0) * g.C + (size_t)cv * VEC;
            if (mean != nullptr) {
#pragma unroll
                for (int i = 0; i < VEC; ++i) mu[i] = mean[co + i];
            }
            if (fA != nullptr) {
#pragma unroll
                for (int i = 0; i < VEC; ++i) { fa[i] = fA[co + i]; fs[i] = fS[co + i]; }
            }
        }
        const bool remask = MODE == 1 && y == nullptr && fA != nullptr;
        if (on) {
            for (int oh = j; oh < g.Ho; oh += ly) {
                const int ih = RESIZE ? g.tabH[oh] : oh;
                const T* xl = x + ((size_t)b * g.Hs + ih) * g.Ws * g.C + (size_t)cv * VEC;
                const size_t dl = ((size_t)b * g.Ho + oh) * g.Wo * g.C + (size_t)cv * VEC;
                for (int ow0 = trow; ow0 < g.Wo; ow0 += 4 * L.rowthreads) {
                    VecT<T, VEC> xr[4], dr[4], yr[4];
                    unsigned mb[4] = {0u, 0u, 0u, 0u};
                    int owc[4], iwv[4];
#pragma unroll
                    for (int u = 0; u < 4; ++u) {
                        owc[u] = min(ow0 + u * L.rowthreads, g.Wo - 1);
                        iwv[u] = RESIZE ? g.tabW[owc[u]] : owc[u];
                    }
#pragma unroll
                    for (int u = 0; u < 4; ++u) {
                        xr[u] = load_raw<T, VEC>(xl + (size_t)iwv[u] * g.C);
                        if (MODE == 1) {
                            dr[u] = load_raw<T, VEC>(dy + dl + (size_t)owc[u] * g.C);
                            if constexpr (YM) mb[u] = reinterpret_cast<const uint8_t*>(y)[(dl + (size_t)owc[u] * g.C) >> 3];
                            else if (y != nullptr) yr[u] = load_raw<T, VEC>(y + dl + (size_t)owc[u] * g.C);
                        }
                    }
                    const bool use_y = MODE == 1 && y != nullptr && !YM;
#pragma unroll
                    for (int u = 0; u < 4; ++u) {
                        const bool inside = ow0 + u * L.rowthreads < g.Wo;
                        float xv[VEC];
                        cvt_f<T, VEC>(xr[u], xv);
                        if (MODE == 0) {
#pragma unroll
                            for (int i = 0; i < VEC; ++i) {
                                const float v = inside ? xv[i] : 0.f;
                                s[i] += v;
                                q[i] += v * v;
                            }
                        } else {
                            float dv[VEC], yv[VEC];
                            cvt_f<T, VEC>(dr[u], dv);
                            if (use_y) {
                                cvt_f<T, VEC>(yr[u], yv);
                            } else {
#pragma unroll
                                for (int i = 0; i < VEC; ++i) yv[i] = 1.f;
                            }
#pragma unroll
                            for (int i = 0; i < VEC; ++i) {
                                const float gate = YM ? (((mb[u] >> i) & 1u) ? 1.f : 0.f)
                                                      : use_y ? yv[i] : (remask ? xv[i] * fa[i] + fs[i] : 1.f);
                                const float d = (inside && gate > 0.f) ? dv[i] : 0.f;
                                s[i] += d;
                                q[i] += d * (xv[i] - mu[i]);
                            }
                        }
                    }
                }
            }
        }
        __syncthreads();
#pragma unroll
        for (int i = 0; i < VEC; ++i) {
            sm[(t * 2 + 0) * VEC + i] = s[i];
            sm[(t * 2 + 1) * VEC + i] = q[i];
        }
        __syncthreads();
        const int nout = L.colthreads * 2 * VEC;
        for (int o = t; o < nout; o += kThreads) {
            const int oc = o / (2 * VEC), rest = o % (2 * VEC);
            if (cv0 + oc < L.lpr) {
                float acc = 0.f;
                for (int r = 0; r < L.rowthreads; ++r) acc += sm[((r * L.colthreads + oc) * 2) * VEC + rest];
                const int stat = rest / VEC, i = rest % VEC;
                out[(size_t)stat * g.C + (size_t)(cv0 + oc) * VEC + i] = acc;
            }
        }
    }
}

template <typename T, int MODE>
static int launch_stats(const void* x, const void* dy, const void* y, const float* mean, const float* fA,
                        const float* fS, int per_image,
                        int64_t B, int64_t Ho, int64_t Wo, int64_t C, int64_t Hs, int64_t Ws,
                        const int32_t* tabH, const int32_t* tabW, float* ws, hipStream_t st, bool ymask = false) {
    RowGeom g{(int)B, (int)Ho, (int)Wo, (int)C, (int)Hs, (int)Ws, tabH, tabW};
    const int ly = lines_per_image(B, Ho);
    dim3 grid((unsigned)(B * ly));
    const bool vec_ok = pick_vec<T>(C) > 1 && aligned16(x) && (MODE == 0 || (aligned16(dy) && (y == nullptr || ymask || aligned16(y))));
    const bool resize = tabH != nullptr || tabW != nullptr;
    if (resize && !(tabH && tabW)) { set_error("stats: both index tables or none"); return -1; }
    if (ymask) {
        if constexpr (MODE == 1 && FullVec<T>::value == 8) {
            if (!(vec_ok && !resize && y)) { set_error("stats_bwd_mask: 16-bit activations, C %% 8 == 0, identity geometry"); return -1; }
            hipLaunchKernelGGL((stats_kernel<T, 8, 1, false, true>), grid, dim3(kThreads), 0, st, (const T*)x, (const T*)dy, (const T*)y, mean,
                               fA, fS, per_image, g, ly, ws);
            MRFP_LAUNCH_CHECK();
            return 0;
        } else {
            set_error("stats_bwd_mask: 16-bit activations only");
            return -1;
        }
    }
    auto launch = [&](auto rs) {
        constexpr bool RS = decltype(rs)::value != 0;
        MRFP_LAUNCH_VEC(vec_ok, (stats_kernel<T, FullVec<T>::value, MODE, RS>), (stats_kernel<T, 1, MODE, RS>), grid, st, (const T*)x,
                        (const T*)dy, (const T*)y, mean, fA, fS, per_image, g, ly, ws);
        return 0;
    };
    return resize ? launch(Int<1>{}) : launch(Int<0>{});
}

struct Red { double s, q; };

#ifndef MRFP_FC
#define MRFP_FC 8
#define MRFP_FL 128
#endif
constexpr int kFC = MRFP_FC, kFL = MRFP_FL;
constexpr int kFold = 8;
__device__ __forceinline__ Red reduce_partials(const float* ws, int64_t first, int64_t n, int64_t C, int c, bool valid,
                                               double (*sm)[2][kFC]) {
    const int ty = threadIdx.y, tx = threadIdx.x;
    double s = 0.0, q = 0.0;
    if (valid) {
        float fs[4] = {0.f, 0.f, 0.f, 0.f}, fq[4] = {0.f, 0.f, 0.f, 0.f};
        int64_t p = first + ty;
        for (; p + 3 * kFL < first + n; p += 4 * kFL) {
#pragma unroll
            for (int u = 0; u < 4; ++u) {
                fs[u] = ws[((p + u * kFL) * 2 + 0) * C + c];
                fq[u] = ws[((p + u * kFL) * 2 + 1) * C + c];
            }
#pragma unroll
            for (int u = 0; u < 4; ++u) { s += (double)fs[u]; q += (double)fq[u]; }
        }
        for (; p < first + n; p += kFL) {
            s += (double)ws[(p * 2 + 0) * C + c];
            q += (double)ws[(p * 2 + 1) * C + c];
        }
    }
    __syncthreads();
    sm[ty][0][tx] = s;
    sm[ty][1][tx] = q;
    __syncthreads();
    double s1 = 0.0, q1 = 0.0;
    if (ty < kFL / kFold) {
#pragma unroll
        for (int k = 0; k < kFold; ++k) { s1 += sm[ty * kFold + k][0][tx]; q1 += sm[ty * kFold + k][1][tx]; }
    }
    __syncthreads();
    if (ty < kFL / kFold) { sm[ty][0][tx] = s1; sm[ty][1][tx] = q1; }
    __syncthreads();
    Red r{0.0, 0.0};
    if (ty == 0) {
#pragma unroll
        for (int k = 0; k < kFL / kFold; ++k) { r.s += sm[k][0][tx]; r.q += sm[k][1][tx]; }
    }
    return r;
}

__global__ void bn_finalize_kernel(const float* ws, int64_t nparts, double count, int C, const float* weight,
                                   const float* bias, float eps, float momentum, float* running_mean,
                                   float* running_var, float* mean, float* invstd, float* A, float* S) {
    __shared__ double sm[kFL][2][kFC];
    const int c = blockIdx.x * kFC + threadIdx.x;
    const bool valid = c < C;
    Red r = reduce_partials(ws, 0, nparts, C, c, valid, sm);
    if (threadIdx.y == 0 && valid) {
        const double m = r.s / count;
        double var = r.q / count - m * m;
        if (var < 0.0) var = 0.0;
        const double is = 1.0 / sqrt(var + (double)eps);
        const float w = weight ? weight[c] : 1.f, bb = bias ? bias[c] : 0.f;
        mean[c] = (float)m;
        invstd[c] = (float)is;
        const float a = (float)(w * is);
        A[c] = a;
        S[c] = (float)(bb - m * (double)a);
        if (running_mean) {
            const double unb = count > 1.0 ? var * count / (count - 1.0) : var;
            running_mean[c] = (float)((1.0 - momentum) * running_mean[c] + momentum * m);
            running_var[c] = (float)((1.0 - momentum) * running_var[c] + momentum * unb);
        }
    }
}

__global__ void bn_eval_coef_kernel(int C, const float* weight, const float* bias, const float* rm, const float* rv,
                                    float eps, float* A, float* S) {
    const int c = blockIdx.x * blockDim.x + threadIdx.x;
    if (c >= C) return;
    const float is = 1.0f / sqrtf(rv[c] + eps);
    const float a = (weight ? weight[c] : 1.f) * is;
    A[c] = a;
    S[c] = (bias ? bias[c] : 0.f) - rm[c] * a;
}

__device__ __forceinline__ void norm_bwd_coef(double Ss, double Sq, double count, float w, float mean, float invstd,
                                              float& P, float& Q, float& R) {
    const double is = invstd;
    const double p = (double)w * is;
    const double qq = -(double)w * is * is * is * Sq / count;
    P = (float)p;
    Q = (float)qq;
    R = (float)(-p * Ss / count - qq * (double)mean);
}

__global__ void bn_bwd_finalize_kernel(const float* ws, int64_t nparts, double count, int C, const float* weight,
                                       const float* mean, const float* invstd, float* dweight, float* dbias,
                                       float* P, float* Q, float* R) {
    __shared__ double sm[kFL][2][kFC];
    const int c = blockIdx.x * kFC + threadIdx.x;
    const bool valid = c < C;
    Red r = reduce_partials(ws, 0, nparts, C, c, valid, sm);
    if (threadIdx.y == 0 && valid) {
        if (dbias) dbias[c] = (float)r.s;
        if (dweight) dweight[c] = (float)(r.q * (double)invstd[c]);
        norm_bwd_coef(r.s, r.q, count, weight ? weight[c] : 1.f, mean[c], invstd[c], P[c], Q[c], R[c]);
    }
}

__global__ void in_finalize_kernel(const float* ws, int64_t nslab, double count, int C, const float* weight,
                                   const float* bias, float eps, float* mean, float* invstd, float* A, float* S) {
    __shared__ double sm[kFL][2][kFC];
    const int c = blockIdx.x * kFC + threadIdx.x, b = blockIdx.y;
    const bool valid = c < C;
    Red r = reduce_partials(ws, (int64_t)b * nslab, nslab, C, c, valid, sm);
    if (threadIdx.y == 0 && valid) {
        const double m = r.s / count;
        double var = r.q / count - m * m;
        if (var < 0.0) var = 0.0;
        const double is = 1.0 / sqrt(var + (double)eps);
        const size_t o = (size_t)b * C + c;
        mean[o] = (float)m;
        invstd[o] = (float)is;
        const float a = (float)((weight ? weight[c] : 1.f) * is);
        A[o] = a;
        S[o] = (float)((bias ? bias[c] : 0.f) - m * (double)a);
    }
}

constexpr int kIL = 8;
__global__ void in_bwd_finalize_kernel(const float* ws, int B, int64_t nslab, double count, int C, const float* weight,
                                       const float* mean, const float* invstd, float* dweight, float* dbias,
                                       float* P, float* Q, float* R) {
    __shared__ double sm[kFL][2][kFC];
    const int tx = threadIdx.x, ty = threadIdx.y;
    const int c = blockIdx.x * kFC + tx;
    const bool valid = c < C;
    constexpr int G = kFL / kIL;
    const int gi = ty / kIL, gl = ty % kIL;
    double dw = 0.0, db = 0.0;
    for (int b0 = 0; b0 < B; b0 += G) {
        const int b = b0 + gi;
        const bool mine = valid && b < B;
        double s = 0.0, q = 0.0;
        if (mine) {
            const float* base = ws + ((size_t)b * nslab * 2) * C + c;
            int64_t p = gl;
            for (; p + 3 * kIL < nslab; p += 4 * kIL) {
                float fs[4], fq[4];
#pragma unroll
                for (int u = 0; u < 4; ++u) {
                    fs[u] = base[((p + u * kIL) * 2 + 0) * C];
                    fq[u] = base[((p + u * kIL) * 2 + 1) * C];
                }
#pragma unroll
                for (int u = 0; u < 4; ++u) { s += (double)fs[u]; q += (double)fq[u]; }
            }
            for (; p < nslab; p += kIL) {
                s += (double)base[(p * 2 + 0) * C];
                q += (double)base[(p * 2 + 1) * C];
            }
        }
        __syncthreads();
        sm[ty][0][tx] = s;
        sm[ty][1][tx] = q;
        __syncthreads();
        if (gl == 0 && mine) {
            double rs = 0.0, rq = 0.0;
#pragma unroll
            for (int k = 0; k < kIL; ++k) { rs += sm[ty + k][0][tx]; rq += sm[ty + k][1][tx]; }
            const size_t o = (size_t)b * C + c;
            norm_bwd_coef(rs, rq, count, weight ? weight[c] : 1.f, mean[o], invstd[o], P[o], Q[o], R[o]);
            sm[ty][0][tx] = rs;
            sm[ty][1][tx] = rq * (double)invstd[o];
        }
        __syncthreads();
        if (ty == 0 && valid) {
            for (int g = 0; g < G && b0 + g < B; ++g) { db += sm[g * kIL][0][tx]; dw += sm[g * kIL][1][tx]; }
        }
    }
    if (ty == 0 && valid) {
        if (dweight) dweight[c] = (float)dw;
        if (dbias) dbias[c] = (float)db;
    }
}

__global__ void plane_sum_kernel(const float* ws, int64_t nslab, double scale, int C, float* out) {
    __shared__ double sm[kFL][2][kFC];
    const int c = blockIdx.x * kFC + threadIdx.x, b = blockIdx.y;
    const bool valid = c < C;
    Red r = reduce_partials(ws, (int64_t)b * nslab, nslab, C, c, valid, sm);
    if (threadIdx.y == 0 && valid) out[(size_t)b * C + c] = (float)(r.s * scale);
}

template <typename T>
__global__ void cast_out_kernel(const float* in, T* out, int64_t n) {
    const int64_t i = (int64_t)blockIdx.x * blockDim.x + threadIdx.x;
    if (i < n) out[i] = from_f<T>(in[i]);
}

__device__ __forceinline__ float block_max(float v, float* sm) {
    const int t = threadIdx.x;
    sm[t] = v;
    __syncthreads();
    for (int s = kThreads / 2; s > 0; s >>= 1) {
        if (t < s) sm[t] = fmaxf(sm[t], sm[t + s]);
        __syncthreads();
    }
    const float r = sm[0];
    __syncthreads();
    return r;
}
__device__ __forceinline__ double block_sum(double v, double* sm) {
    const int t = threadIdx.x;
    sm[t] = v;
    __syncthreads();
    for (int s = kThreads / 2; s > 0; s >>= 1) {
        if (t < s) sm[t] += sm[t + s];
        __syncthreads();
    }
    const double r = sm[0];
    __syncthreads();
    return r;
}

__global__ __launch_bounds__(kThreads) void np_coef_kernel(int B, int C, const float* alpha, const float* beta_noise,
                                                           const float* mu, float* sigma, float* A, float* S) {
    __shared__ float smf[kThreads];
    float lmax = -INFINITY;
    for (int c = threadIdx.x; c < C; c += kThreads) {
        double m = 0.0;
        for (int b = 0; b < B; ++b) m += (double)mu[(size_t)b * C + c];
        m /= B;
        double v = 0.0;
        for (int b = 0; b < B; ++b) { const double d = (double)mu[(size_t)b * C + c] - m; v += d * d; }
        const float sg = (float)sqrt(v / (double)(B - 1));
        sigma[c] = sg;
        lmax = fmaxf(lmax, sg);
        if (sg != sg) lmax = sg;
    }
    const float M = block_max(lmax, smf);
    for (int c = threadIdx.x; c < C; c += kThreads) {
        const float scale = sigma[c] / M * 1.5f;
        for (int b = 0; b < B; ++b) {
            const size_t o = (size_t)b * C + c;
            const float beta = 1.f + beta_noise[o] * scale;
            A[o] = alpha[o];
            S[o] = (beta - alpha[o]) * mu[o];
        }
    }
}

__global__ __launch_bounds__(kThreads) void np_bwd_coef_kernel(int B, int C, double hw, const float* alpha,
                                                               const float* beta_noise, const float* mu,
                                                               const float* sigma, const float* G, float* K) {
    __shared__ float smf[kThreads];
    __shared__ double smd[kThreads];
    float lmax = -INFINITY;
    for (int c = threadIdx.x; c < C; c += kThreads) lmax = fmaxf(lmax, sigma[c]);
    const float M = block_max(lmax, smf);
    int larg = 0x7fffffff;
    for (int c = threadIdx.x; c < C; c += kThreads)
        if (sigma[c] == M && c < larg) larg = c;
    const int cstar = -(int)block_max(-(float)larg, smf);
    double lt = 0.0;
    for (int c = threadIdx.x; c < C; c += kThreads) {
        double ds = 0.0;
        for (int b = 0; b < B; ++b) {
            const size_t o = (size_t)b * C + c;
            ds += (double)mu[o] * (double)G[o] * (double)beta_noise[o];
        }
        lt += ds * (double)sigma[c];
    }
    const double T = block_sum(lt, smd);
    const double Md = (double)M;
    for (int c = threadIdx.x; c < C; c += kThreads) {
        double ds = 0.0, mbar = 0.0;
        for (int b = 0; b < B; ++b) {
            const size_t o = (size_t)b * C + c;
            ds += (double)mu[o] * (double)G[o] * (double)beta_noise[o];
            mbar += (double)mu[o];
        }
        mbar /= B;
        double dsig = 1.5 * ds / Md;
        if (c == cstar) dsig -= 1.5 * T / (Md * Md);
        const double scale = (double)sigma[c] / Md * 1.5;
        for (int b = 0; b < B; ++b) {
            const size_t o = (size_t)b * C + c;
            const double beta = 1.0 + (double)beta_noise[o] * scale;
            double dmu = (beta - (double)alpha[o]) * (double)G[o];
            dmu += dsig * ((double)mu[o] - mbar) / ((double)(B - 1) * (double)sigma[c]);
            K[o] = (float)(dmu / hw);
        }
    }
}

}

using namespace mrfp;

extern "C" {

int mrfp_version(void) { return 100; }
const char* mrfp_last_error(void) { return mrfp::g_err; }

int64_t mrfp_stats_nslab(int64_t B, int64_t Ho) { return lines_per_image(B, Ho); }

int mrfp_stats_fwd(const void* x, int dtype, int64_t B, int64_t Ho, int64_t Wo, int64_t C, int64_t Hs, int64_t Ws,
                   const int32_t* tabH, const int32_t* tabW, float* ws, void* stream) {
    MRFP_CHECK(x && ws && B > 0 && Ho > 0 && Wo > 0 && C > 0, "stats_fwd: bad arguments");
    MRFP_CHECK(C <= 65536 && B * Ho < (1LL << 31), "stats_fwd: shape out of range");
    hipStream_t st = (hipStream_t)stream;
    return by_dtype(dtype, "stats_fwd", [&](auto t) {
        using T = typename decltype(t)::type;
        return launch_stats<T, 0>(x, nullptr, nullptr, nullptr, nullptr, nullptr, 0, B, Ho, Wo, C, Hs, Ws, tabH, tabW, ws, st);
    });
}

int mrfp_stats_bwd(const void* dy, const void* x, const void* y, const float* mean, const float* fA, const float* fS,
                   int per_image, int dtype,
                   int64_t B, int64_t Ho, int64_t Wo, int64_t C, int64_t Hs, int64_t Ws, const int32_t* tabH,
                   const int32_t* tabW, float* ws, void* stream) {
    MRFP_CHECK(dy && x && ws && B > 0 && Ho > 0 && Wo > 0 && C > 0, "stats_bwd: bad arguments");
    hipStream_t st = (hipStream_t)stream;
    return by_dtype(dtype, "stats_bwd", [&](auto t) {
        using T = typename decltype(t)::type;
        return launch_stats<T, 1>(x, dy, y, mean, fA, fS, per_image, B, Ho, Wo, C, Hs, Ws, tabH, tabW, ws, st);
    });
}

int mrfp_stats_bwd_mask(const void* dy, const void* x, const void* mask, const float* mean, int per_image, int dtype, int64_t B,
                        int64_t H, int64_t W, int64_t C, float* ws, void* stream) {
    MRFP_CHECK(dy && x && mask && ws && B > 0 && H > 0 && W > 0 && C > 0 && (C & 7) == 0, "stats_bwd_mask: bad arguments");
    hipStream_t st = (hipStream_t)stream;
    return by_dtype16(dtype, "stats_bwd_mask", [&](auto t) {
        using T = typename decltype(t)::type;
        return launch_stats<T, 1>(x, dy, mask, mean, nullptr, nullptr, per_image, B, H, W, C, H, W, nullptr, nullptr, ws, st, true);
    });
}

int mrfp_bn_finalize(const float* ws, int64_t B, int64_t nslab, int64_t count, int64_t C, const float* weight,
                     const float* bias, float eps, float momentum, float* running_mean, float* running_var,
                     float* mean, float* invstd, float* A, float* S, void* stream) {
    MRFP_CHECK(ws && mean && invstd && A && S && C > 0 && count > 0, "bn_finalize: bad arguments");
    hipLaunchKernelGGL(bn_finalize_kernel, dim3((unsigned)((C + mrfp::kFC - 1) / mrfp::kFC)), dim3(mrfp::kFC, mrfp::kFL), 0, (hipStream_t)stream, ws,
                       B * nslab, (double)count, (int)C, weight, bias, eps, momentum, running_mean, running_var, mean,
                       invstd, A, S);
    MRFP_LAUNCH_CHECK();
    return 0;
}

int mrfp_bn_eval_coef(int64_t C, const float* weight, const float* bias, const float* running_mean,
                      const float* running_var, float eps, float* A, float* S, void* stream) {
    MRFP_CHECK(running_mean && running_var && A && S && C > 0, "bn_eval_coef: bad arguments");
    hipLaunchKernelGGL(bn_eval_coef_kernel, dim3((unsigned)((C + 255) / 256)), dim3(256), 0, (hipStream_t)stream, (int)C,
                       weight, bias, running_mean, running_var, eps, A, S);
    MRFP_LAUNCH_CHECK();
    return 0;
}

int mrfp_bn_bwd_finalize(const float* ws, int64_t B, int64_t nslab, int64_t count, int64_t C, const float* weight,
                         const float* mean, const float* invstd, float* dweight, float* dbias, float* P, float* Q,
                         float* R, void* stream) {
    MRFP_CHECK(ws && mean && invstd && P && Q && R && C > 0 && count > 0, "bn_bwd_finalize: bad arguments");
    hipLaunchKernelGGL(bn_bwd_finalize_kernel, dim3((unsigned)((C + mrfp::kFC - 1) / mrfp::kFC)), dim3(mrfp::kFC, mrfp::kFL), 0, (hipStream_t)stream, ws,
                       B * nslab, (double)count, (int)C, weight, mean, invstd, dweight, dbias, P, Q, R);
    MRFP_LAUNCH_CHECK();
    return 0;
}

int mrfp_in_finalize(const float* ws, int64_t B, int64_t nslab, int64_t count, int64_t C, const float* weight,
                     const float* bias, float eps, float* mean, float* invstd, float* A, float* S, void* stream) {
    MRFP_CHECK(ws && mean && invstd && A && S && C > 0 && count > 0 && B > 0 && B < 65536, "in_finalize: bad arguments");
    hipLaunchKernelGGL(in_finalize_kernel, dim3((unsigned)((C + mrfp::kFC - 1) / mrfp::kFC), (unsigned)B), dim3(mrfp::kFC, mrfp::kFL), 0,
                       (hipStream_t)stream, ws, nslab, (double)count, (int)C, weight, bias, eps, mean, invstd, A, S);
    MRFP_LAUNCH_CHECK();
    return 0;
}

int mrfp_in_bwd_finalize(const float* ws, int64_t B, int64_t nslab, int64_t count, int64_t C, const float* weight,
                         const float* mean, const float* invstd, float* dweight, float* dbias, float* P, float* Q,
                         float* R, void* stream) {
    MRFP_CHECK(ws && mean && invstd && P && Q && R && C > 0 && count > 0, "in_bwd_finalize: bad arguments");
    hipLaunchKernelGGL(in_bwd_finalize_kernel, dim3((unsigned)((C + mrfp::kFC - 1) / mrfp::kFC)), dim3(mrfp::kFC, mrfp::kFL), 0, (hipStream_t)stream, ws,
                       (int)B, nslab, (double)count, (int)C, weight, mean, invstd, dweight, dbias, P, Q, R);
    MRFP_LAUNCH_CHECK();
    return 0;
}

int mrfp_np_finalize(const float* ws, int64_t B, int64_t nslab, int64_t count, int64_t C, const float* alpha,
                     const float* beta_noise, float* mu, float* sigma, float* A, float* S, void* stream) {
    MRFP_CHECK(ws && alpha && beta_noise && mu && sigma && A && S && C > 0 && B > 0 && B < 65536, "np_finalize: bad arguments");
    hipStream_t st = (hipStream_t)stream;
    hipLaunchKernelGGL(plane_sum_kernel, dim3((unsigned)((C + mrfp::kFC - 1) / mrfp::kFC), (unsigned)B), dim3(mrfp::kFC, mrfp::kFL), 0, st, ws, nslab,
                       1.0 / (double)count, (int)C, mu);
    MRFP_LAUNCH_CHECK();
    hipLaunchKernelGGL(np_coef_kernel, dim3(1), dim3(kThreads), 0, st, (int)B, (int)C, alpha, beta_noise, mu, sigma, A, S);
    MRFP_LAUNCH_CHECK();
    return 0;
}

int mrfp_np_bwd_finalize(const float* ws, int64_t B, int64_t nslab, int64_t count, int64_t C, const float* alpha,
                         const float* beta_noise, const float* mu, const float* sigma, float* Gtmp, float* K,
                         void* stream) {
    MRFP_CHECK(ws && alpha && beta_noise && mu && sigma && Gtmp && K && C > 0 && B > 0 && B < 65536, "np_bwd_finalize: bad arguments");
    hipStream_t st = (hipStream_t)stream;
    hipLaunchKernelGGL(plane_sum_kernel, dim3((unsigned)((C + mrfp::kFC - 1) / mrfp::kFC), (unsigned)B), dim3(mrfp::kFC, mrfp::kFL), 0, st, ws, nslab, 1.0,
                       (int)C, Gtmp);
    MRFP_LAUNCH_CHECK();
    hipLaunchKernelGGL(np_bwd_coef_kernel, dim3(1), dim3(kThreads), 0, st, (int)B, (int)C, (double)count, alpha,
                       beta_noise, mu, sigma, Gtmp, K);
    MRFP_LAUNCH_CHECK();
    return 0;
}

int mrfp_mean_finalize(const float* ws, int64_t B, int64_t nslab, int64_t count, int64_t C, float* tmp, void* out,
                       int dtype, void* stream) {
    MRFP_CHECK(ws && out && tmp && C > 0 && B > 0 && B < 65536, "mean_finalize: bad arguments");
    hipStream_t st = (hipStream_t)stream;
    return by_dtype(dtype, "mean_finalize", [&](auto t) {
        using T = typename decltype(t)::type;
        constexpr bool cast = !std::is_same<T, float>::value;
        hipLaunchKernelGGL(plane_sum_kernel, dim3((unsigned)((C + mrfp::kFC - 1) / mrfp::kFC), (unsigned)B), dim3(mrfp::kFC, mrfp::kFL), 0, st, ws,
                           nslab, 1.0 / (double)count, (int)C, cast ? tmp : (float*)out);
        MRFP_LAUNCH_CHECK();
        if constexpr (cast) {
            const int64_t n = B * C;
            hipLaunchKernelGGL((cast_out_kernel<T>), dim3((unsigned)((n + 255) / 256)), dim3(256), 0, st, tmp, (T*)out, n);
            MRFP_LAUNCH_CHECK();
        }
        return 0;
    });
}

}
```

### mrfp_amd/deepv3.py

```python
from __future__ import annotations

import math
import random

import torch
from torch import nn

from . import ops
from .config import cfg
from .conv import wgrad_boundary
from .loss import fused_ce_kwargs, fused_loss
from .network import Resnet
from .network.mynn import (HipBatchNorm2d, HipConv2d, HipInstanceNorm2d, Norm2d, Upsample, conv_norm, initialize_weights,
                           initialize_weights_kaimingnormal_forOC)

__all__ = ["_AtrousSpatialPyramidPoolingModule", "MRFPPlus", "simpleDeepV3Plus", "ReferenceRandom", "InjectedRandom"]


class ReferenceRandom:

    _py = random

    def toggles(self):
        return self._py.random(), self._py.random(), self._py.random()

    def seed_toggles(self, seed):
        self._py = random.Random(seed)

    def reinit_hrfp(self, model):
        flat = _hrfp_arena(model)
        if flat is not None:
            flat[0].normal_()
            flat[0].mul_(flat[1])
        else:
            for conv, bn in model.hrfp_layers():
                initialize_weights_kaimingnormal_forOC(conv)
                initialize_weights_kaimingnormal_forOC(bn)
        from . import conv as conv_mod
        conv_mod.repack_weights([c.weight for c, _ in model.hrfp_layers()], tag="hrfp",
                                biases=[c.bias for c, _ in model.hrfp_layers()])

    def np_noise(self, which, B, C, device):
        z = torch.randn(2, B, C, 1, 1, device=device).mul_(0.75)
        alpha, beta_noise = z[0], z[1]
        alpha.add_(1.0)
        return alpha, beta_noise


_HRFP_ARENA = __import__("os").environ.get("MRFP_HRFP_ARENA", "1") != "0"


def _hrfp_arena(model):
    layers = model.hrfp_layers()
    first = layers[0][0].weight
    if not first.is_cuda or not _HRFP_ARENA:
        return None
    params, stds = [], []
    for conv, bn in layers:
        fan_in = conv.weight.shape[1] * conv.weight.shape[2] * conv.weight.shape[3]
        params += [conv.weight, conv.bias, bn.weight, bn.bias]
        stds += [math.sqrt(2.0 / fan_in), 0.0, 0.5, 0.0]
    if any(p is None or p.dtype != torch.float32 for p in params):
        return None
    st = getattr(model, "_hrfp_arena_state", None)
    if st is not None and st[0].device == first.device and st[2] == tuple(p.data_ptr() for p in params):
        return st
    offs, n = [], 0
    for p in params:
        offs.append(n)
        n += (p.numel() + 3) // 4 * 4
    flat = torch.zeros(n, dtype=torch.float32, device=first.device)
    std = torch.zeros(n, dtype=torch.float32, device=first.device)
    with torch.no_grad():
        for p, o, sd in zip(params, offs, stds):
            v = flat[o:o + p.numel()].view(p.shape)
            v.copy_(p.data)
            p.data = v
            std[o:o + p.numel()] = sd
    st = model._hrfp_arena_state = (flat, std, tuple(p.data_ptr() for p in params))
    from . import conv as conv_mod
    conv_mod.invalidate_packs()
    return st


class InjectedRandom(ReferenceRandom):

    def __init__(self, toggles=(True, True, True), noise=None, reinit=False):
        self._t, self._noise, self._reinit = toggles, noise, reinit

    def toggles(self):
        return tuple(0.25 if t else 0.75 for t in self._t)

    def reinit_hrfp(self, model):
        if self._reinit:
            super().reinit_hrfp(model)

    def np_noise(self, which, B, C, device):
        if self._noise is None:
            return super().np_noise(which, B, C, device)
        return self._noise[which + "_alpha"].to(device), self._noise[which + "_beta"].to(device)


class _ConvBnRelu(nn.Sequential):

    def __init__(self, cin, cout, k, padding=0, dilation=1):
        super().__init__(HipConv2d(cin, cout, kernel_size=k, padding=padding, dilation=dilation, bias=False),
                         Norm2d(cout), nn.ReLU(inplace=True))

    def forward(self, x):
        return conv_norm(self[0], self[1], x, relu=True)

    def forward_skip(self, x):
        return conv_norm(self[0], self[1], x, want_skip=True, relu=True)


class _AtrousSpatialPyramidPoolingModule(nn.Module):

    def __init__(self, in_dim, reduction_dim=256, output_stride=16, rates=(6, 12, 18)):
        super().__init__()
        print("output_stride = ", output_stride)
        if output_stride == 8:
            rates = [2 * r for r in rates]
        elif output_stride == 4:
            rates = [4 * r for r in rates]
        elif output_stride == 16:
            pass
        elif output_stride == 32:
            rates = [r // 2 for r in rates]
        else:
            raise TypeError("output stride of {} not supported".format(output_stride))
        feats = [_ConvBnRelu(in_dim, reduction_dim, 1)]
        feats += [_ConvBnRelu(in_dim, reduction_dim, 3, padding=r, dilation=r) for r in rates]
        self.features = nn.ModuleList(feats)
        self.img_pooling = nn.AdaptiveAvgPool2d(1)
        self.img_conv = _ConvBnRelu(in_dim, 256, 1)

    def forward(self, x):
        outs, cur = [], x
        for f in self.features:
            y, cur = f.forward_skip(cur)
            outs.append(y)
        img = self.img_conv(ops.global_avg_pool(cur))
        return ops.concat_channels([Upsample(img, x.shape[2:])] + outs)


class _DeepLabBase(nn.Module):
    def _build_trunk_and_head(self, num_classes, trunk, wt_layer):
        if trunk == "wider_resnet38_a2" and self._allow_101:
            return self._build_wrn_trunk_and_head(num_classes)
        if trunk == "resnet-50":
            resnet = Resnet.resnet50(wt_layer=wt_layer)
        elif trunk == "resnet-101" and self._allow_101:
            resnet = Resnet.resnet101(wt_layer=wt_layer)
        else:
            raise ValueError("Not a valid network arch")
        if isinstance(resnet, Resnet.ResNet3X3):
            resnet.layer0 = nn.Sequential(resnet.conv1, resnet.bn1, resnet.relu1, resnet.conv2, resnet.bn2,
                                          resnet.relu2, resnet.conv3, resnet.bn3, resnet.relu3, resnet.maxpool)
        else:
            resnet.layer0 = nn.Sequential(resnet.conv1, resnet.bn1, resnet.relu, resnet.maxpool)
        self._trunk = [resnet]
        self.layer0 = resnet.layer0
        self.layer1, self.layer2, self.layer3, self.layer4 = resnet.layer1, resnet.layer2, resnet.layer3, resnet.layer4
        if self.variant == "D16":
            for n, m in self.layer4.named_modules():
                if "conv2" in n:
                    m.dilation, m.padding, m.stride = (2, 2), (2, 2), (1, 1)
                elif "downsample.0" in n:
                    m.stride = (1, 1)
        else:
            print("Not using Dilation ")
        self.output_stride = 16
        self._build_head(num_classes, 2048)

    def _build_wrn_trunk_and_head(self, num_classes):
        from .network import wider_resnet
        wrn = wider_resnet.wider_resnet38_a2(classes=0, dilation=True)
        self._trunk = [wrn]
        for name in ("mod1", "pool2", "mod2", "pool3", "mod3", "mod4", "mod5", "mod6", "mod7", "bn_out"):
            setattr(self, name, getattr(wrn, name))
        self.output_stride = 8
        self._build_head(num_classes, 4096)

    def _build_head(self, num_classes, trunk_channels):
        self.aspp = _AtrousSpatialPyramidPoolingModule(trunk_channels, 256, output_stride=self.output_stride)
        self.bot_fine = _ConvBnRelu(256, 48, 1)
        self.bot_aspp = _ConvBnRelu(1280, 256, 1)
        self.final1 = nn.Sequential(HipConv2d(304, 256, kernel_size=3, padding=1, bias=False), Norm2d(256),
                                    nn.ReLU(inplace=True),
                                    HipConv2d(256, 256, kernel_size=3, padding=1, bias=False), Norm2d(256),
                                    nn.ReLU(inplace=True))
        self.final2 = nn.Sequential(HipConv2d(256, num_classes, kernel_size=1, bias=True))

    def _init_head(self):
        initialize_weights(self.aspp)
        initialize_weights(self.bot_aspp)
        initialize_weights(self.bot_fine)
        initialize_weights(self.final1)
        initialize_weights(self.final2)
        self.eps = 1e-5
        self.whitening = False
        self.three_input_layer = False

    _taps = None

    def _tap(self, name, t):
        if self._taps is not None:
            self._taps[name] = t.detach()

    def _stem(self, x):
        trunk = self._trunk[0]
        w_arr = []
        if not isinstance(trunk, (Resnet.ResNet, Resnet.ResNet3X3)):
            return trunk.stem(x), w_arr
        if isinstance(trunk, Resnet.ResNet3X3):
            return trunk.stem(x, w_arr), w_arr
        return Resnet._conv_norm_relu_pool(self.layer0[0], self.layer0[1], trunk.wt_layer[2], ops.as_activation(x), w_arr), w_arr

    def _low(self, t, w_arr):
        if hasattr(self, "layer1"):
            return self.layer1([wgrad_boundary(t), w_arr])[0]
        return self.mod3(wgrad_boundary(t))

    def _high(self, t, w_arr, fourier=None):
        if hasattr(self, "layer1"):
            t = self.layer2([wgrad_boundary(t), w_arr])
            if fourier is not None:
                t[0] = fourier.at("layer2", t[0])
            self._tap("layer2", t[0])
            t[0] = wgrad_boundary(t[0])
            t = self.layer3(t)
            self._tap("layer3", t[0])
            t[0] = wgrad_boundary(t[0])
            return wgrad_boundary(self.layer4(t)[0])
        t = self.mod7(self.mod6(self.mod5(wgrad_boundary(self.mod4(wgrad_boundary(t))))))
        return wgrad_boundary(self.bn_out[0].fused(t, relu=True))

    def _final1(self, d):
        d = conv_norm(self.final1[0], self.final1[1], d, relu=True)
        return conv_norm(self.final1[3], self.final1[4], d, relu=True)

    def _head(self, dec1, size, gts, training, low_res=False):
        f2 = self.final2[0]
        nc = f2.out_channels
        pitch = (nc + 31) // 32 * 32
        dec2 = ops.conv2d(dec1, f2.weight, f2.bias, f2.stride, f2.padding, f2.dilation, phys_out=pitch)
        if low_res:
            if training:
                raise ValueError("low_res is an eval-path option (training=False)")
            return dec2
        if training and cfg.MODEL.FUSE_UPSAMPLE_CE and fused_ce_kwargs(self.criterion) is not None:
            return fused_loss(self.criterion, dec2, gts, size, nc)
        main_out = ops.upsample_bilinear(dec2, size, channels=nc)
        if training:
            return self._loss(main_out, gts)
        return main_out.float()

    def _head_o2(self, dec1, oc_dec, size, gts, training):
        from . import conv
        f2 = self.final2[0]
        nc = f2.out_channels
        pitch = (nc + 31) // 32 * 32
        p_low, p_half = conv.shared_conv1x1_pair(dec1, oc_dec, f2.weight, f2.bias, pitch)
        dec2 = ops.upsample_bilinear(p_low, (oc_dec.shape[2], oc_dec.shape[3]), addend=p_half)
        if training and cfg.MODEL.FUSE_UPSAMPLE_CE and fused_ce_kwargs(self.criterion) is not None:
            return fused_loss(self.criterion, dec2, gts, size, nc)
        main_out = ops.upsample_bilinear(dec2, size, channels=nc)
        if training:
            return self._loss(main_out, gts)
        return main_out.float()

    def _loss(self, main_out, gts):
        loss = fused_loss(self.criterion, main_out, gts)
        if loss is None:
            loss = self.criterion(main_out.float(), gts)
        return loss


class MRFPPlus(_DeepLabBase):
    _allow_101 = True

    def __init__(self, num_classes, trunk="resnet-50", criterion=None, criterion_aux=None,
                 variant="D16", wt_layer=[0, 0, 4, 4, 4, 0, 0], use_wtloss=False):
        super().__init__()
        self.criterion = criterion
        self.criterion_aux = criterion_aux
        self.variant = variant
        self.wt_layer = wt_layer
        self.use_wtloss = use_wtloss
        self.trunk = trunk
        self._build_trunk_and_head(num_classes, trunk, wt_layer)

        stem_c = 64 if trunk == "resnet-50" else 128
        enc = [(stem_c, 64, 1), (64, 64, 1), (64, 128, 2), (128, 256, 2)]
        dec = [(256, 128, 1), (128, 64, 1), (64, 64, 2), (64, stem_c, 2)]
        for i, (ci, co, d) in enumerate(enc, 1):
            setattr(self, "OClayer%d" % i, HipConv2d(ci, co, kernel_size=3, stride=1, padding=d, dilation=d).requires_grad_(False))
            setattr(self, "OC%d_bn" % i, HipBatchNorm2d(co).requires_grad_(False))
        for i, (ci, co, d) in enumerate(dec, 1):
            setattr(self, "OCdeclayer%d" % i, HipConv2d(ci, co, kernel_size=3, stride=1, padding=d, dilation=d).requires_grad_(False))
            setattr(self, "OC%d_decbn" % i, HipBatchNorm2d(co).requires_grad_(False))
        for conv, bn in self.hrfp_layers():
            initialize_weights_kaimingnormal_forOC(conv)
            initialize_weights_kaimingnormal_forOC(bn)
        self._init_head()
        self.rng = ReferenceRandom()
        self.fourier_perturb = None

    def _fold_skips_hrfp(self):
        return (getattr(self, "_mrfp_fold", False) and not self.training and not torch.is_grad_enabled())

    def hrfp_layers(self):
        enc = [(getattr(self, "OClayer%d" % i), getattr(self, "OC%d_bn" % i)) for i in range(1, 5)]
        dec = [(getattr(self, "OCdeclayer%d" % i), getattr(self, "OC%d_decbn" % i)) for i in range(1, 5)]
        return enc + dec

    def Normalization_Perturbation_Plus(self, feat, which="np1", res=None):
        B, C = feat.shape[0], feat.shape[1]
        alpha, beta_noise = self.rng.np_noise(which, B, C, feat.device)
        return ops.np_plus(feat, alpha, beta_noise, res)

    def _hrfp(self, xp, h, w, need_out=True, need_dec=True):
        lazy = (cfg.MODEL.HRFP_LAZY or self._fold_skips_hrfp()) and self._taps is None
        if lazy and not (need_out or need_dec):
            return None, None, xp
        resize = [dict(scale=1.205), dict(scale=1.2), dict(scale=1.2), dict(size=(int(h / 2), int(w / 2))),
                  dict(size=(int(h / 2), int(w / 2))), dict(scale=0.838), dict(scale=0.798),
                  dict(size=(math.ceil(h / 4), math.ceil(w / 4)))]
        t, dec, xp_alias = xp, None, xp
        for i, ((conv, bn), rs) in enumerate(zip(self.hrfp_layers(), resize)):
            if i == 4 and lazy and not need_out:
                return t, None, xp_alias
            plan = ops.nearest_plan(t.shape[2], t.shape[3], device=t.device, **rs)
            stat_resize = plan if bn.training else None
            if i == 0:
                t, xp_alias = conv.forward_skip(t, stat_resize=stat_resize)
            elif i == 4:
                t, dec = conv.forward_skip(t, stat_resize=stat_resize)
            else:
                t = conv(t, stat_resize=stat_resize)
            if (plan.Hs, plan.Ws) != tuple(t.shape[2:]):
                plan = ops.nearest_plan(t.shape[2], t.shape[3], device=t.device, **rs)
            t = bn.fused(t, relu=True, plan=plan)
            self._tap("hrfp%d" % i, t)
        return dec, t, xp_alias

    def forward(self, x, gts=None, training=True, low_res=False):
        if low_res and training:
            raise ValueError("low_res is an eval-path option (training=False)")
        p, p2, p3 = self.rng.toggles()
        h, w = x.shape[2], x.shape[3]
        o1, npp, o2 = (training == True and p < 0.5), (training == True and p2 < 0.5), (training == True and p3 < 0.5)
        if o1:
            self.rng.reinit_hrfp(self)

        xp, w_arr = self._stem(x)
        fourier = None
        if training == True and self.fourier_perturb is not None:
            fp = self.fourier_perturb
            if hasattr(fp, "begin"):
                fp.begin(x.shape[0], True)
                xp = fp.at("stem", xp)
                fourier = fp
            else:
                xp = fp(xp)
        self._tap("stem", xp)
        OCout_dec, OCout, xp = self._hrfp(xp, h, w, o1, o2)
        t = xp
        if npp and o1 and self._taps is None:
            t = self.Normalization_Perturbation_Plus(xp, "np1", res=OCout)
        else:
            if npp:
                t = self.Normalization_Perturbation_Plus(xp, "np1")
                self._tap("np1", t)
            if o1:
                t = ops.add(OCout, t)
        tap = getattr(self.layer1[-1], "instance_norm_layer", None) if hasattr(self, "layer1") else None
        if isinstance(tap, HipInstanceNorm2d):
            tap._emit_plane_stats = bool(npp) and fourier is None
        t = self._low(t, w_arr)
        if fourier is not None:
            t = fourier.at("layer1", t)
        if npp:
            t = self.Normalization_Perturbation_Plus(t, "np2")
        self._tap("layer1", t)
        dec0_fine, low_level = self.bot_fine.forward_skip(t)
        t = self._high(low_level, w_arr, fourier)
        if self.use_wtloss:
            self.w_arr = w_arr
        self._tap("layer4", t)
        t = self.aspp(t)
        self._tap("aspp", t)
        dec0_up = self.bot_aspp(t)
        dec1 = self._final1(ops.concat_upsample(dec0_fine, dec0_up, low_level.shape[2:], cfg.MODEL.DECODER_PAD))
        self._tap("dec1", dec1)
        if o2:
            if cfg.MODEL.COMMUTE_O2:
                return self._head_o2(dec1, OCout_dec, (h, w), gts, training)
            dec1 = ops.upsample_bilinear(dec1, (int(h / 2), int(w / 2)), addend=OCout_dec)
        return self._head(dec1, (h, w), gts, training, low_res)


class simpleDeepV3Plus(_DeepLabBase):
    _allow_101 = False

    def __init__(self, num_classes, trunk="resnet-50", criterion=None, criterion_aux=None,
                 variant="D16", wt_layer=[0, 0, 0, 0, 0, 0, 0], use_wtloss=False):
        super().__init__()
        self.criterion = criterion
        self.criterion_aux = criterion_aux
        self.variant = variant
        self.wt_layer = wt_layer
        self.use_wtloss = use_wtloss
        self.trunk = trunk
        self._build_trunk_and_head(num_classes, trunk, wt_layer)
        self._init_head()

    def forward(self, x, gts=None, training=False, low_res=False):
        h, w = x.shape[2], x.shape[3]
        t, w_arr = self._stem(x)
        x_tuple = self.layer1([t, w_arr])
        low_level = x_tuple[0]
        x_tuple = self.layer4(self.layer3(self.layer2(x_tuple)))
        dec0_up = self.bot_aspp(self.aspp(x_tuple[0]))
        dec0_fine = self.bot_fine(low_level)
        dec1 = self._final1(ops.concat_upsample(dec0_fine, dec0_up, low_level.shape[2:], cfg.MODEL.DECODER_PAD))
        return self._head(dec1, (h, w), gts, training, low_res)
```

### mrfp_amd/ops.py

```python
from __future__ import annotations

import collections
import math
import os
import weakref
from functools import lru_cache
from typing import Optional, Tuple

import numpy as np
import torch

from . import _lib
from ._lib import call, dt, ptr, stream

CL = torch.channels_last

GRAD_NOTIFY = [None]
GRAD_DEFERRED = set()


def wgrad_workspace(M, N, Q, device, n=1):
    return torch.empty(int(_lib.lib().mrfp_conv_wgrad_grouped_ws_bytes(M, N, Q, n)), dtype=torch.uint8, device=device)


def grad_sink(param):
    if param is not None and getattr(param, "_mrfp_direct", False) and param.grad is not None \
            and param.grad.dtype == torch.float32 and param.grad.is_contiguous():
        return param.grad
    return None


def notify_grad(param):
    if GRAD_NOTIFY[0] is not None:
        GRAD_NOTIFY[0](param)


def to_cl(x: torch.Tensor) -> torch.Tensor:
    if x.dim() != 4:
        raise ValueError("expected a 4-D activation, got %s" % (tuple(x.shape),))
    return x.contiguous(memory_format=CL)


def empty_cl(B, C, H, W, dtype, device) -> torch.Tensor:
    return torch.empty((B, C, H, W), dtype=dtype, device=device, memory_format=CL)


def zeros_cl(B, C, H, W, dtype, device) -> torch.Tensor:
    return torch.zeros((B, H, W, C), dtype=dtype, device=device).permute(0, 3, 1, 2)


def _chk(x: torch.Tensor, name="x") -> torch.Tensor:
    if not x.is_cuda:
        raise _lib.MrfpHipError("%s must live on the GPU (got %s): the HIP path has no CPU fallback" % (name, x.device))
    uses = getattr(x, "_mrfp_uses", None)
    if uses is not None:
        uses[0] += 1
    if x.dim() != 4 or not x.is_contiguous(memory_format=CL):
        x = to_cl(x)
    return x


def _f32(t: Optional[torch.Tensor]) -> Optional[torch.Tensor]:
    if t is None:
        return None
    return t.detach().float().contiguous()


def nearest_out_size(in_size: int, scale: float) -> int:
    return int(math.floor(float(in_size) * scale))


def _nearest_table(in_size: int, out_size: int, scale: Optional[float]) -> np.ndarray:
    s = np.float32(1.0 / scale) if scale is not None else np.float32(in_size) / np.float32(out_size)
    src = np.floor(np.arange(out_size, dtype=np.float32) * s).astype(np.int64)
    return np.minimum(src, in_size - 1).astype(np.int32)


def _inverse_table(tab: np.ndarray, in_size: int) -> np.ndarray:
    lo = np.searchsorted(tab, np.arange(in_size), side="left")
    hi = np.searchsorted(tab, np.arange(in_size), side="right")
    return np.stack([lo, hi], 1).astype(np.int32).reshape(-1)


class NearestPlan:

    def __init__(self, Hs, Ws, Ho, Wo, scale, device):
        self.Hs, self.Ws, self.Ho, self.Wo = Hs, Ws, Ho, Wo
        th, tw = _nearest_table(Hs, Ho, scale), _nearest_table(Ws, Wo, scale)
        self.tabH = torch.from_numpy(th).to(device)
        self.tabW = torch.from_numpy(tw).to(device)
        self.invH = torch.from_numpy(_inverse_table(th, Hs)).to(device)
        self.invW = torch.from_numpy(_inverse_table(tw, Ws)).to(device)
        mh, mw = np.bincount(th, minlength=Hs), np.bincount(tw, minlength=Ws)
        self._mult = np.outer(mh, mw)
        self._mult_dev = {}

    def multiplicity(self, B):
        if B not in self._mult_dev:
            if self._mult.max() > 255:
                self._mult_dev[B] = None
            else:
                flat = np.zeros(B * self.Hs * self.Ws + 256, dtype=np.uint8)
                flat[:B * self.Hs * self.Ws] = np.tile(self._mult.astype(np.uint8).reshape(-1), B)
                self._mult_dev[B] = torch.from_numpy(flat).to(self.tabH.device)
        return self._mult_dev[B]


@lru_cache(maxsize=256)
def _plan_cached(Hs, Ws, Ho, Wo, scale, device_str):
    return NearestPlan(Hs, Ws, Ho, Wo, scale, torch.device(device_str))


def nearest_plan(Hs: int, Ws: int, *, scale: Optional[float] = None, size: Optional[Tuple[int, int]] = None,
                 device="cuda") -> NearestPlan:
    if scale is not None:
        Ho, Wo = nearest_out_size(Hs, scale), nearest_out_size(Ws, scale)
    else:
        Ho, Wo = int(size[0]), int(size[1])
    return _plan_cached(Hs, Ws, Ho, Wo, scale, str(device))


def _geom(x, plan: Optional[NearestPlan]):
    B, C, Hs, Ws = x.shape
    if plan is None:
        return B, Hs, Ws, C, Hs, Ws, None, None, None, None
    if (plan.Hs, plan.Ws) != (Hs, Ws):
        raise _lib.MrfpHipError("resize plan %dx%d does not match input %dx%d" % (plan.Hs, plan.Ws, Hs, Ws))
    return B, plan.Ho, plan.Wo, C, Hs, Ws, plan.tabH, plan.tabW, plan.invH, plan.invW


def _stats_ws(B, Ho, C, device):
    nslab = int(_lib.lib().mrfp_stats_nslab(B, Ho))
    return nslab, torch.empty(B * nslab * 2 * C, dtype=torch.float32, device=device)


def _stats_fwd(x, plan):
    B, Ho, Wo, C, Hs, Ws, tH, tW, _, _ = _geom(x, plan)
    nslab, ws = _stats_ws(B, Ho, C, x.device)
    call("mrfp_stats_fwd", ptr(x), dt(x), B, Ho, Wo, C, Hs, Ws, ptr(tH), ptr(tW), ptr(ws), stream())
    return nslab, ws


def _stats_bwd(dy, x, y, mean, per_image, plan, fA=None, fS=None):
    B, Ho, Wo, C, Hs, Ws, tH, tW, _, _ = _geom(x, plan)
    nslab, ws = _stats_ws(B, Ho, C, x.device)
    call("mrfp_stats_bwd", ptr(dy), ptr(x), ptr(y), ptr(mean), ptr(fA), ptr(fS), int(per_image), dt(x), B, Ho, Wo, C,
         Hs, Ws, ptr(tH), ptr(tW), ptr(ws), stream())
    return nslab, ws


PLANE_STATS = [os.environ.get("MRFP_PLANE_STATS", "1") != "0"]
PLANE_STATS_HITS = [0]


def _take_planestats(x):
# ... 168 lines not shown
        mean, invstd, A, S = coef[0:C], coef[C:2 * C], coef[2 * C:3 * C], coef[3 * C:4 * C]
        if training:
            fused = _serving_colstats(x, C, B * Ho * Wo, plan, False)
            if fused is not None:
                ws, nb_, nslab = fused.final, 1, fused.final_count
            else:
                nslab, ws = _stats_fwd(x, plan)
                nb_ = B
            count = B * Ho * Wo
            ctx.sync = _sync_bn_group() if may_sync else None
            if ctx.sync is not None:
                ws, count = _allreduce_stats(ws, nb_ * nslab, C, count, ctx.sync)
                nb_, nslab = 1, 2
            ctx.count = count
            call("mrfp_bn_finalize", ptr(ws), nb_, nslab, count, C, ptr(w32), ptr(b32), float(eps),
                 float(momentum), ptr(running_mean), ptr(running_var), ptr(mean), ptr(invstd), ptr(A), ptr(S), stream())
        else:
            ctx.sync, ctx.count = None, B * Ho * Wo
            call("mrfp_bn_eval_coef", C, ptr(w32), ptr(b32), ptr(running_mean), ptr(running_var), float(eps),
                 ptr(A), ptr(S), stream())
            if x.requires_grad or (weight is not None and weight.requires_grad):
                mean.copy_(running_mean)
                torch.rsqrt(running_var.float() + eps, out=invstd)
        ctx.plan, ctx.act, ctx.training, ctx.has_res = plan, act, training, res is not None
        ctx.keep_y = relu and res is not None
        ctx.remask = relu and res is None
        ctx.ymask = _keeps_sign_mask(x, relu, res, plan)
        ctx.gate_skip = bool(ctx.ymask and GATED_SKIP[0] and getattr(res, "_mrfp_skip_alias", False))
        ctx.gate_ok = bool(act == ACT_NONE and res is None and plan is None and training and x.element_size() == 2 and C % 8 == 0)
        ctx.alias_uses = getattr(res, "_mrfp_uses", None)
        keep = None
        if relu6:
            y = empty_cl(B, C, Ho, Wo, x.dtype, dev)
            keep = torch.empty((B * Ho * Wo * C + 7) // 8, dtype=torch.uint8, device=dev)
            call("mrfp_affine_fwd_relu6_mask", ptr(x), ptr(y), ptr(keep), dt(x), B * Ho * Wo, C, ptr(A), ptr(S), stream())
        elif ctx.ymask:
            y = empty_cl(B, C, Ho, Wo, x.dtype, dev)
            keep = torch.empty(B * Ho * Wo * C // 8, dtype=torch.uint8, device=dev)
            call("mrfp_affine_fwd_relu_mask", ptr(x), ptr(res), ptr(y), ptr(keep), dt(x), B, Ho, Wo, C, ptr(A), ptr(S), 0, stream())
        else:
            y = _affine_fwd(x, res, A, S, False, relu, plan, stats=stats)
            if ctx.keep_y:
                keep = y
        ctx.wparam, ctx.bparam = weight, bias
        ctx.save_for_backward(x, keep, w32, mean, invstd, A, S)
        return y

    @staticmethod
    def backward(ctx, dy):
        x, keep, w32, mean, invstd, A, S = ctx.saved_tensors
        gate = None
        cell = getattr(ctx, "_mrfp_cell", None)
        g = getattr(dy, "_mrfp_gate", None)
        if cell is not None and cell[1]:
            if g is None or g[1] != dy._version:
                raise _lib.MrfpHipError("a gated gradient reached its BatchNorm without its gate: the layer's output was also "
                                        "consumed by an operator outside mrfp_amd.ops (set MRFP_GATED_SKIP=0)")
            cell[1] = False
        if g is not None:
            if (g[1] == dy._version and ctx.gate_ok and dy.dtype == x.dtype and dy.shape == x.shape
                    and dy.is_contiguous(memory_format=CL)):
                gate = g[0]
            else:
                from .conv import ungate
                dy = ungate(dy)
        dy = _chk(dy, "dy")
        plan = ctx.plan
        B, Ho, Wo, C, *_ = _geom(x, plan)
        fA, fS = (A, S) if ctx.remask else (None, None)
        mask = y = None
        if gate is not None:
            mask = gate
            GATED_BN_HITS[0] += 1
        elif ctx.ymask:
            mask = keep
        elif ctx.act == ACT_RELU6:
            if x.element_size() == 2 and C % 8 == 0 and dy.dtype == x.dtype:
                mask = keep
            else:
                gated = torch.empty_like(dy, memory_format=CL)
                call("mrfp_mask_gate", ptr(dy), ptr(keep), ptr(gated), dt(dy), dy.numel(), stream())
                dy = gated
                RELU6_GATE_HITS[0] += 1
        else:
            y = keep
        if mask is not None:
            nslab, ws = _stats_ws(B, Ho, C, x.device)
            call("mrfp_stats_bwd_mask", ptr(dy), ptr(x), ptr(mask), ptr(mean), 0, dt(x), B, Ho, Wo, C, ptr(ws), stream())
        else:
            nslab, ws = _stats_bwd(dy, x, y, mean, False, plan, fA, fS)
        out = torch.empty(5 * C, dtype=torch.float32, device=dy.device)
        dw, db, P, Q, R = (out[i * C:(i + 1) * C] for i in range(5))
        dw = _grad_dest(ctx.wparam, ctx.needs_input_grad[1], dw)
        db = _grad_dest(ctx.bparam, ctx.needs_input_grad[2], db)
        call("mrfp_bn_bwd_finalize", ptr(ws), B, nslab, B * Ho * Wo, C, ptr(w32), ptr(mean), ptr(invstd),
             ptr(dw), ptr(db), ptr(P), ptr(Q), ptr(R), stream())
        if ctx.sync is not None:
            gws, _ = _allreduce_stats(ws, B * nslab, C, 0, ctx.sync)
            call("mrfp_bn_bwd_finalize", ptr(gws), 1, 2, ctx.count, C, ptr(w32), ptr(mean), ptr(invstd), None, None,
                 ptr(P), ptr(Q), ptr(R), stream())
        if not ctx.training:
            Q.zero_()
            R.zero_()
        if mask is not None:
            dx = empty_cl(B, C, Ho, Wo, dy.dtype, dy.device)
            dres = dres_out = None
            if ctx.ymask:
                if ctx.gate_skip and ctx.needs_input_grad[5] and ctx.alias_uses is not None and ctx.alias_uses[0] == 1:
                    dres = dy.view_as(dy)
                    dres._mrfp_gate = (mask, dres._version)
                    ctx.alias_uses[1] = True
                else:
                    dres = dres_out = empty_cl(B, C, Ho, Wo, dy.dtype, dy.device)
            call("mrfp_affine_bwd_mask", ptr(dy), ptr(x), ptr(mask), ptr(dx), ptr(dres_out), dt(dy), B, Ho, Wo, C, ptr(P), ptr(Q),
                 ptr(R), 0, stream())
        else:
            dx, dres = _affine_bwd(dy, x, y, P, Q, R, False, plan, ctx.has_res, x, fA, fS)
        return (dx, _grad_result(ctx.wparam, dw), _grad_result(ctx.bparam, db), None, None, dres) + (None,) * 7


RUNNING_STATS_EPOCH = [0]


def batch_norm_act(x, weight, bias, running_mean, running_var, *, training, momentum=0.1, eps=1e-5,
                   relu=False, res=None, plan=None, emit_stats=False):
    if training and running_mean is not None:
        RUNNING_STATS_EPOCH[0] += 1
    ps = _planestats_rows(x, emit_stats and plan is None and not _keeps_sign_mask(x, relu, res, plan))
    y = _BatchNormAct.apply(x, weight, bias, running_mean, running_var, res, training, momentum, eps,
                            ACT_RELU if relu else ACT_NONE, plan, True, ps[1] if ps is not None else None)
    _tag_planestats(y, ps)
    if (GATED_BN[0] and GATED_SKIP[0] and SIGN_MASK[0] and not relu and res is None and plan is None and training and y.grad_fn is not None
            and y.element_size() == 2 and y.shape[1] % 8 == 0):
        y._mrfp_skip_alias = True
        y._mrfp_uses = [0, False]
        y.grad_fn._mrfp_cell = y._mrfp_uses
    return y


def local_batch_norm_act(x, weight, bias, running_mean, running_var, *, training, momentum=0.1, eps=1e-5, act=None):
    if act not in (None, "relu6"):
        raise _lib.MrfpHipError("local_batch_norm_act: act must be None or 'relu6' (got %r)" % (act,))
    if training and running_mean is not None:
        RUNNING_STATS_EPOCH[0] += 1
    return _BatchNormAct.apply(x, weight, bias, running_mean, running_var, None, bool(training), momentum, eps,
                               ACT_RELU6 if act == "relu6" else ACT_NONE, None, False, None)


def batch_norm_relu6(x, weight, bias, running_mean, running_var, *, training, momentum=0.1, eps=1e-5):
    return local_batch_norm_act(x, weight, bias, running_mean, running_var, training=training, momentum=momentum, eps=eps,
                                act="relu6")


IN_FUSED_STATS = [os.environ.get("MRFP_IN_FUSED_STATS", "1") != "0"]
IN_FUSED_HITS = [0]


def _in_plane_sums(x):
    ps = _take_planestats(x)
    x = _chk(x)
    B, C, H, W = x.shape
    fused = _serving_colstats(x, C, B * H * W, None, True)
    rb = fused.block_rows if fused is not None else 0
    if rb < 0 and B * (-rb) == fused.row_blocks:
        IN_FUSED_HITS[0] += 1
        return x, -rb, fused.rows
    if rb > 0 and (H * W) % rb == 0 and B * ((H * W) // rb) <= fused.row_blocks:
        IN_FUSED_HITS[0] += 1
        return x, (H * W) // rb, fused.rows
    if ps is not None:
        return x, ps[0], ps[1]
    nslab, ws = _stats_fwd(x, None)
    return x, nslab, ws


def _in_finalize(x, nslab, ws, weight, bias, eps):
    B, C, H, W = x.shape
    w32, b32 = _f32(weight), _f32(bias)
    n = B * C
    coef = torch.empty(4 * n, dtype=torch.float32, device=x.device)
    mean, invstd, A, S = coef[0:n], coef[n:2 * n], coef[2 * n:3 * n], coef[3 * n:4 * n]
    call("mrfp_in_finalize", ptr(ws), B, nslab, H * W, C, ptr(w32), ptr(b32), float(eps), ptr(mean),
         ptr(invstd), ptr(A), ptr(S), stream())
    return w32, mean, invstd, A, S


def _in_bwd_finalize(ctx, x, nslab, ws, w32, mean, invstd):
    B, C, H, W = x.shape
    n = B * C
    pqr = torch.empty(3 * n, dtype=torch.float32, device=x.device)
    P, Q, R = pqr[0:n], pqr[n:2 * n], pqr[2 * n:3 * n]
    dwb = torch.empty(2 * C, dtype=torch.float32, device=x.device)
    dw = _grad_dest(ctx.wparam, ctx.wparam is not None, dwb[:C])
    db = _grad_dest(ctx.bparam, ctx.bparam is not None, dwb[C:])
    call("mrfp_in_bwd_finalize", ptr(ws), B, nslab, H * W, C, ptr(w32), ptr(mean), ptr(invstd), ptr(dw), ptr(db),
         ptr(P), ptr(Q), ptr(R), stream())
    return P, Q, R, dw, db


class _InstanceNormAct(torch.autograd.Function):

    @staticmethod
    def forward(ctx, x, weight, bias, eps, relu, stats):
        x, nslab, ws = _in_plane_sums(x)
        w32, mean, invstd, A, S = _in_finalize(x, nslab, ws, weight, bias, eps)
        y = _affine_fwd(x, None, A, S, True, relu, None, stats=stats)
        ctx.relu = relu
        ctx.wparam, ctx.bparam = weight, bias
        ctx.save_for_backward(x, w32, mean, invstd, A, S)
        return y

    @staticmethod
    def backward(ctx, dy):
        x, w32, mean, invstd, A, S = ctx.saved_tensors
        dy = _chk(dy, "dy")
        fA, fS = (A, S) if ctx.relu else (None, None)
        nslab, ws = _stats_bwd(dy, x, None, mean, True, None, fA, fS)
        P, Q, R, dw, db = _in_bwd_finalize(ctx, x, nslab, ws, w32, mean, invstd)
        dx, _ = _affine_bwd(dy, x, None, P, Q, R, True, None, False, x, fA, fS)
        return dx, _grad_result(ctx.wparam, dw), _grad_result(ctx.bparam, db), None, None, None


def instance_norm_act(x, weight, bias, *, eps=1e-5, relu=False, emit_stats=False):
    ps = _planestats_rows(x, emit_stats)
    return _tag_planestats(_InstanceNormAct.apply(x, weight, bias, eps, relu, ps[1] if ps is not None else None), ps)


class _NPPlus(torch.autograd.Function):

    @staticmethod
    def forward(ctx, x, alpha, beta_noise, res=None):
        ps = _take_planestats(x)
        x = _chk(x)
        res = _chk(res, "res") if res is not None else None
        B, C, H, W = x.shape
        a32 = alpha.detach().float().reshape(B, C).contiguous()
        n32 = beta_noise.detach().float().reshape(B, C).contiguous()
        buf = torch.empty(3 * B * C + C, dtype=torch.float32, device=x.device)
        n = B * C
        mu, A, S, sigma = buf[0:n], buf[n:2 * n], buf[2 * n:3 * n], buf[3 * n:3 * n + C]
        nslab, ws = ps if ps is not None else _stats_fwd(x, None)
        call("mrfp_np_finalize", ptr(ws), B, nslab, H * W, C, ptr(a32), ptr(n32), ptr(mu), ptr(sigma), ptr(A),
             ptr(S), stream())
        y = _affine_fwd(x, res, A, S, True, False, None)
        ctx.save_for_backward(a32, n32, mu, sigma)
        ctx.shape = (B, C, H, W)
        ctx.has_res = res is not None
        return y

    @staticmethod
    def backward(ctx, dy):
        a32, n32, mu, sigma = ctx.saved_tensors
        dy = _chk(dy, "dy")
        B, C, H, W = ctx.shape
        nslab, ws = _stats_bwd(dy, dy, None, None, True, None)
        tmp = torch.empty(2 * B * C, dtype=torch.float32, device=dy.device)
        G, K = tmp[:B * C], tmp[B * C:]
        call("mrfp_np_bwd_finalize", ptr(ws), B, nslab, H * W, C, ptr(a32), ptr(n32), ptr(mu), ptr(sigma),
             ptr(G), ptr(K), stream())
        dx = empty_cl(B, C, H, W, dy.dtype, dy.device)
        call("mrfp_affine_fwd", ptr(dy), None, ptr(dx), dt(dy), B, H, W, C, H, W, None, None, ptr(a32), ptr(K), 1, 0,
             stream())
        return dx, None, None, (dy if ctx.has_res else None)


def np_plus(x, alpha, beta_noise, res=None):
    return _NPPlus.apply(x, alpha, beta_noise, res)


class _Bilinear(torch.autograd.Function):

    @staticmethod
    def forward(ctx, x, addend, Ho, Wo, channels):
        x = _chk(x)
        addend = _chk(addend, "addend") if addend is not None else None
        B, ld, Hi, Wi = x.shape
        C = ld if channels is None else int(channels)
        y = empty_cl(B, C, Ho, Wo, x.dtype, x.device)
        call("mrfp_bilinear_fwd", ptr(x), ptr(addend), ptr(y), dt(x), B, Hi, Wi, Ho, Wo, C, ld, stream())
        ctx.dims = (B, C, ld, Hi, Wi, Ho, Wo)
        ctx.has_add = addend is not None
        return y

    @staticmethod
    def backward(ctx, dy):
        dy = _chk(dy, "dy")
        B, C, ld, Hi, Wi, Ho, Wo = ctx.dims
        if ld == C:
            dx = empty_cl(B, ld, Hi, Wi, dy.dtype, dy.device)
        else:
            dx = zeros_cl(B, ld, Hi, Wi, dy.dtype, dy.device)
        call("mrfp_bilinear_bwd", ptr(dy), ptr(dx), dt(dy), B, Hi, Wi, Ho, Wo, C, ld, stream())
        return dx, (dy if ctx.has_add else None), None, None, None


class _Broadcast(torch.autograd.Function):

    @staticmethod
    def forward(ctx, x, Ho, Wo):
        x = _chk(x)
        B, C = x.shape[0], x.shape[1]
        S = x.detach().float().reshape(B, C).contiguous()
        y = empty_cl(B, C, Ho, Wo, x.dtype, x.device)
        call("mrfp_affine_fwd", None, None, ptr(y), dt(x), B, Ho, Wo, C, Ho, Wo, None, None, None, ptr(S), 1, 0, stream())
        ctx.dims = (B, C, Ho, Wo)
        return y
# ... 588 lines not shown
def _chk_u8(who, name, t, dev=None):
    if not isinstance(t, torch.Tensor) or not t.is_cuda or (dev is not None and t.device != dev):
        raise _lib.MrfpHipError("%s: %s must be a uint8 tensor on the GPU%s: the HIP path has no CPU fallback"
                                % (who, name, "" if dev is None else " of pred"))
    if t.dtype != torch.uint8 or not t.is_contiguous():
        raise _lib.MrfpHipError("%s: %s must be a contiguous uint8 tensor (got %s, strides %s)" % (who, name, t.dtype, tuple(t.stride())))


def colorize(pred_u8, palette, image_u8=None, alpha=0.5, out=None):
    who = "colorize"
    _chk_u8(who, "pred_u8", pred_u8)
    dev = pred_u8.device
    _chk_u8(who, "palette", palette, dev)
    if tuple(palette.shape) != (256, 3):
        raise _lib.MrfpHipError("%s: palette must be uint8 [256,3], got %s" % (who, tuple(palette.shape)))
    shape = tuple(pred_u8.shape) + (3,)
    a = 256
    if image_u8 is not None:
        _chk_u8(who, "image_u8", image_u8, dev)
        if tuple(image_u8.shape) != shape:
            raise _lib.MrfpHipError("%s: image_u8 must be uint8 %s, got %s" % (who, shape, tuple(image_u8.shape)))
        if not 0.0 <= float(alpha) <= 1.0:
            raise ValueError("%s: alpha must be in [0, 1], got %r" % (who, alpha))
        a = int(round(float(alpha) * 256))
    if out is None:
        out = torch.empty(shape, dtype=torch.uint8, device=dev)
    else:
        _chk_u8(who, "out", out, dev)
        if tuple(out.shape) != shape:
            raise _lib.MrfpHipError("%s: out must be uint8 %s, got %s" % (who, shape, tuple(out.shape)))
        lo, hi = out.data_ptr(), out.data_ptr() + out.numel()
        for t in (pred_u8, image_u8):
            if t is not None and t.data_ptr() < hi and lo < t.data_ptr() + t.numel():
                raise _lib.MrfpHipError("%s: out overlaps an input" % who)
    if pred_u8.numel():
        call("mrfp_colorize_u8", ptr(pred_u8), ptr(palette), ptr(image_u8), ptr(out), pred_u8.numel(), a, stream())
    return out


class _ReLU(torch.autograd.Function):

    @staticmethod
    def forward(ctx, x):
        x = _chk(x)
        y = _affine_fwd(x, None, None, None, False, True, None)
        ctx.save_for_backward(y)
        return y

    @staticmethod
    def backward(ctx, dy):
        (y,) = ctx.saved_tensors
        dy = _chk(dy, "dy")
        dx, _ = _affine_bwd(dy, None, y, None, None, None, False, None, False, y)
        return dx


def relu(x):
    return _ReLU.apply(x)


def as_activation(x: torch.Tensor) -> torch.Tensor:
    from .config import cfg
    if not x.is_cuda:
        raise _lib.MrfpHipError("input must live on the GPU (got %s): the HIP path has no CPU fallback" % x.device)
    from . import conv
    return conv.pad_input_channels(x, cfg.MODEL.ACT_DTYPE)


def conv2d_skip(x, weight, bias, stride, padding, dilation, stat_resize=None):
    from . import conv
    return conv.conv2d(_chk(x), weight, bias, stride, padding, dilation, None, True, stat_resize=stat_resize)


def conv2d(x, weight, bias, stride, padding, dilation, phys_out=None, stat_resize=None):
    from . import conv
    return conv.conv2d(_chk(x), weight, bias, stride, padding, dilation, phys_out, stat_resize=stat_resize)


class _ConcatChannels(torch.autograd.Function):

    @staticmethod
    def forward(ctx, *tensors):
        ts = [_chk(t) for t in tensors]
        B, _, H, W = ts[0].shape
        Cs = [int(t.shape[1]) for t in ts]
        Ct = sum(Cs)
        y = empty_cl(B, Ct, H, W, ts[0].dtype, ts[0].device)
        c0 = 0
        for t, C in zip(ts, Cs):
            if tuple(t.shape) != (B, C, H, W) or t.dtype != y.dtype:
                raise _lib.MrfpHipError("concat_channels: shape / dtype mismatch")
            call("mrfp_copy_channels", ptr(t), ptr(y), dt(t), B * H * W, C, C, 0, Ct, c0, stream())
            c0 += C
        ctx.Cs = Cs
        return y

    @staticmethod
    def backward(ctx, dy):
        dy = _chk(dy, "dy")
        B, Ct, H, W = dy.shape
        out, c0 = [], 0
        for i, C in enumerate(ctx.Cs):
            if ctx.needs_input_grad[i]:
                g = empty_cl(B, C, H, W, dy.dtype, dy.device)
                call("mrfp_copy_channels", ptr(dy), ptr(g), dt(dy), B * H * W, C, Ct, c0, C, 0, stream())
                out.append(g)
            else:
                out.append(None)
            c0 += C
        return tuple(out)


class _ConcatUpsample(torch.autograd.Function):

    @staticmethod
    def forward(ctx, a, b, Ho, Wo, pad_to):
        a, b = _chk(a), _chk(b)
        B, Ca, H, W = a.shape
        _, Cb, Hi, Wi = b.shape
        if (H, W) != (Ho, Wo) or b.shape[0] != B or a.dtype != b.dtype:
            raise _lib.MrfpHipError("concat_upsample: shape / dtype mismatch")
        Ct = (Ca + Cb + pad_to - 1) // pad_to * pad_to
        y = empty_cl(B, Ct, H, W, a.dtype, a.device)
        esz = a.element_size()
        if Ct != Ca + Cb:
            y[:, Ca + Cb:].zero_()
        call("mrfp_copy_channels", ptr(a), ptr(y), dt(a), B * H * W, Ca, Ca, 0, Ct, 0, stream())
        call("mrfp_bilinear_fwd_into", ptr(b), y.data_ptr() + Ca * esz, dt(b), B, Hi, Wi, Ho, Wo, Cb, Cb, Ct, stream())
        ctx.dims = (B, Ca, Cb, Hi, Wi, Ho, Wo, Ct)
        return y

    @staticmethod
    def backward(ctx, dy):
        dy = _chk(dy, "dy")
        B, Ca, Cb, Hi, Wi, Ho, Wo, Ct = ctx.dims
        esz = dy.element_size()
        da = db = None
        if ctx.needs_input_grad[0]:
            da = empty_cl(B, Ca, Ho, Wo, dy.dtype, dy.device)
            call("mrfp_copy_channels", ptr(dy), ptr(da), dt(dy), B * Ho * Wo, Ca, Ct, 0, Ca, 0, stream())
        if ctx.needs_input_grad[1]:
            db = empty_cl(B, Cb, Hi, Wi, dy.dtype, dy.device)
            call("mrfp_bilinear_bwd_from", dy.data_ptr() + Ca * esz, ptr(db), dt(dy), B, Hi, Wi, Ho, Wo, Cb, Cb, Ct, stream())
        return da, db, None, None, None


def concat_upsample(a, b, size, pad_to=1):
    epc = 16 // a.element_size()
    if a.shape[1] % epc or b.shape[1] % epc or (b.shape[2] == 1 and b.shape[3] == 1):
        return concat_channels([a, upsample_bilinear(b, size)])
    return _ConcatUpsample.apply(a, b, int(size[0]), int(size[1]), int(pad_to))


def concat_channels(tensors):
    return _ConcatChannels.apply(*tensors)


class _PlaneMean(torch.autograd.Function):

    @staticmethod
    def forward(ctx, x):
        x = _chk(x)
        B, C, H, W = x.shape
        nslab, ws = _stats_fwd(x, None)
        out = torch.empty(B, C, dtype=torch.float32, device=x.device)
        call("mrfp_mean_finalize", ptr(ws), B, nslab, H * W, C, ptr(out), ptr(out), _lib.F32, stream())
        ctx.dims, ctx.dtype = (B, C, H, W), x.dtype
        return out

    @staticmethod
    def backward(ctx, g):
        B, C, H, W = ctx.dims
        S = (g.detach().float() / float(H * W)).contiguous()
        dx = empty_cl(B, C, H, W, ctx.dtype, g.device)
        call("mrfp_affine_fwd", None, None, ptr(dx), _lib._DT[ctx.dtype], B, H, W, C, H, W, None, None, None, ptr(S), 1, 0,
             stream())
        return dx


def plane_mean(x):
    return _PlaneMean.apply(x)


class _CrossGram(torch.autograd.Function):

    @staticmethod
    def forward(ctx, a, b):
        a, b = _chk(a, "a"), _chk(b, "b")
        B, Ca, H, W = a.shape
        Cb = b.shape[1]
        esz = a.element_size()
        if (Ca * esz) % 16 or (Cb * esz) % 16 or a.dtype != b.dtype or b.shape[0] != B or b.shape[2:] != a.shape[2:]:
            raise _lib.MrfpHipError("cross_gram: channel counts must make 16-byte chunks and shapes must match")
        G = torch.empty(B, Ca, Cb, dtype=torch.float32, device=a.device)
        ws = wgrad_workspace(H * W, Ca, Cb, a.device)
        abytes, bbytes = H * W * Ca * esz, H * W * Cb * esz
        for i in range(B):
            call("mrfp_conv_wgrad", b.data_ptr() + i * bbytes, a.data_ptr() + i * abytes, G.data_ptr() + i * Ca * Cb * 4,
                 ptr(ws), dt(a), 1, H, W, Cb, Cb, Ca, Ca, 1, 1, H, W, 1, 0, 0, 1, stream())
        ctx.save_for_backward(a, b)
        ctx.same = a.data_ptr() == b.data_ptr()
        return G

    @staticmethod
    def backward(ctx, dG):
        from . import conv
        a, b = ctx.saved_tensors
        B = a.shape[0]
        dG = dG.float()
        da = db = None
        if ctx.same:
            sym = dG + dG.transpose(1, 2)
            parts = [conv.conv2d(a[i:i + 1].detach(), sym[i].reshape(*sym.shape[1:], 1, 1).contiguous(), None, 1, 0, 1)
                     for i in range(B)]
            return torch.cat(parts, 0), None
        if ctx.needs_input_grad[0]:
            da = torch.cat([conv.conv2d(b[i:i + 1].detach(), dG[i].reshape(*dG.shape[1:], 1, 1).contiguous(), None, 1, 0, 1)
                            for i in range(B)], 0)
        if ctx.needs_input_grad[1]:
            dGt = dG.transpose(1, 2).contiguous()
            db = torch.cat([conv.conv2d(a[i:i + 1].detach(), dGt[i].reshape(*dGt.shape[1:], 1, 1).contiguous(), None, 1, 0, 1)
                            for i in range(B)], 0)
        return da, db


def cross_gram(a, b):
    return _CrossGram.apply(a, b)


def channel_gram(x):
    x = _chk(x)
    return _CrossGram.apply(x, x)


def per_image_matmul(x, Wm, bias=None):
    from . import conv
    x = _chk(x)
    outs = []
    for i in range(x.shape[0]):
        w = Wm[i].reshape(Wm.shape[1], Wm.shape[2], 1, 1)
        outs.append(conv.conv2d(x[i:i + 1], w, None if bias is None else bias[i], 1, 0, 1))
    return torch.cat(outs, 0)


def _gm_call(a, b, want_sum=True):
    B, C, H, W = a.shape
    dev = a.device
    M = torch.empty(B, C // 16, 16, 16, dtype=torch.float32, device=dev)
    s = torch.empty(B, C, dtype=torch.float32, device=dev) if want_sum else None
    nbytes = int(_lib.lib().mrfp_group_moments_ws_bytes(B, H * W, C))
    if nbytes <= 0:
        raise _lib.MrfpHipError("group_moments: unsupported shape %s (C %% 16 == 0, C <= 1024)" % (tuple(a.shape),))
    ws = torch.empty(nbytes, dtype=torch.uint8, device=dev)
    call("mrfp_group_moments", ptr(a), ptr(b), ptr(M), ptr(s), ptr(ws), dt(a), B, H * W, C, stream())
    return s, M


def _ga_call(x, Wm, z=None, Vm=None, shift=None):
    B, C, H, W = x.shape
    y = empty_cl(B, C, H, W, x.dtype, x.device)
    call("mrfp_group_apply", ptr(x), ptr(Wm), ptr(z), ptr(Vm), ptr(shift), ptr(y), dt(x), B, H * W, C, stream())
    return y


class _GroupMoments(torch.autograd.Function):

    @staticmethod
    def forward(ctx, x):
        x = _chk(x)
        ctx.save_for_backward(x)
        return _gm_call(x, x)

    @staticmethod
    def backward(ctx, ds, dM):
        (x,) = ctx.saved_tensors
        dM = dM.float()
        sym = (dM + dM.transpose(-1, -2)).contiguous()
        return _ga_call(x, sym, shift=ds.float().contiguous())


def group_moments(x):
    return _GroupMoments.apply(x)


class _GroupApply(torch.autograd.Function):

    @staticmethod
    def forward(ctx, x, Wm, shift):
        x = _chk(x)
        Wm, shift = Wm.float().contiguous(), shift.float().contiguous()
        ctx.save_for_backward(x, Wm)
        return _ga_call(x, Wm, shift=shift)

    @staticmethod
    def backward(ctx, dy):
        x, Wm = ctx.saved_tensors
        dy = _chk(dy, "dy")
        dshift, dWm = _gm_call(dy, x)
        dx = _ga_call(dy, Wm.transpose(-1, -2).contiguous())
        return dx, dWm, dshift


def group_apply(x, Wm, shift):
    return _GroupApply.apply(x, Wm, shift)


# ... 298 lines not shown
```

Before: 308.4 images/sec.

## Group ASPP branch batch-norm+ReLU into shared slice kernels writing concat buffer

Adds grouped kernels that normalise and activate up to eight same-shape branches in one launch, writing each result straight into its channel slice of a shared NHWC concat buffer. Matching grouped backward stats, finalize and affine kernels handle the gradients. It also adds an upsample-into-slice path that zero-fills the pad channels, so the separate concat copy and launch go away. The aim is fewer launches and no extra concat read/write in the ASPP and decoder, at the cost of more complex bookkeeping and a fallback path when shapes do not line up.

```diff
diff --git a/include/mrfp_hip.h b/include/mrfp_hip.h
--- a/include/mrfp_hip.h
+++ b/include/mrfp_hip.h
@@ -72,6 +72,25 @@
 int mrfp_copy_channels(const void* src, void* dst, int dtype, int64_t npix, int64_t C, int64_t ld_src, int64_t c0_src,
                        int64_t ld_dst, int64_t c0_dst, void* stream);
 
+int mrfp_affine_fwd_grouped(const void* const* xs, void* const* ys, const int64_t* pitches, const int64_t* offsets,
+                            const float* const* As, const float* const* Ss, const int32_t* coef_per_image, const int32_t* relus, int64_t G,
+                            int dtype, int64_t B, int64_t H, int64_t W, int64_t C, void* stream);
+int mrfp_stats_bwd_grouped(const void* const* dys, const int64_t* pitches, const int64_t* offsets, const void* const* xs,
+                           const float* const* means, const float* const* fAs, const float* const* fSs, float* const* wss, int64_t G,
+                           int dtype, int64_t B, int64_t H, int64_t W, int64_t C, void* stream);
+int mrfp_affine_bwd_grouped(const void* const* dys, const int64_t* pitches, const int64_t* offsets, const void* const* xs,
+                            void* const* dxs, const float* const* Ps, const float* const* Qs, const float* const* Rs,
+                            const float* const* fAs, const float* const* fSs, int64_t G, int dtype, int64_t B, int64_t H, int64_t W,
+                            int64_t C, void* stream);
+int mrfp_bn_finalize_grouped(const float* const* wss, const int64_t* nparts, int64_t G, int64_t count, int64_t C,
+                             const float* const* weights, const float* const* biases, float eps, float momentum,
+                             float* const* running_means, float* const* running_vars, float* const* means, float* const* invstds,
+                             float* const* As, float* const* Ss, void* stream);
+int mrfp_bn_bwd_finalize_grouped(const float* const* wss, const int64_t* nparts, int64_t G, int64_t count, int64_t C,
+                                 const float* const* weights, const float* const* means, const float* const* invstds,
+                                 float* const* dweights, float* const* dbiases, float* const* Ps, float* const* Qs, float* const* Rs,
+                                 void* stream);
+
 int mrfp_add(const void* a, const void* b, void* y, int dtype, int64_t n, void* stream);
 
 int mrfp_bilinear_fwd(const void* x, const void* addend, void* y, int dtype,
@@ -84,6 +103,8 @@
                            int64_t C, int64_t ld_in, int64_t ld_out, void* stream);
 int mrfp_bilinear_bwd_from(const void* dy, void* dx, int dtype, int64_t B, int64_t Hi, int64_t Wi, int64_t Ho, int64_t Wo,
                            int64_t C, int64_t ld_in, int64_t ld_dy, void* stream);
+int mrfp_bilinear_fwd_into_pad(const void* x, void* y, int dtype, int64_t B, int64_t Hi, int64_t Wi, int64_t Ho, int64_t Wo,
+                               int64_t C, int64_t ld_in, int64_t ld_out, int64_t pad, void* stream);
 
 int mrfp_maxpool_fwd(const void* x, void* y, uint8_t* idx, int dtype,
                      int64_t B, int64_t H, int64_t W, int64_t C, void* stream);
diff --git a/mrfp_amd/csrc/affine.hip b/mrfp_amd/csrc/affine.hip
--- a/mrfp_amd/csrc/affine.hip
+++ b/mrfp_amd/csrc/affine.hip
@@ -335,6 +335,126 @@
             } else {
                 for (int iw = trow; iw < g.Ws; iw += L.rowthreads)
                     slow_pixel(iw, invW ? invW[2 * iw] : iw, invW ? invW[2 * iw + 1] : iw + 1);
+            }
+        }
+    }
+}
+
+template <typename T, int VEC>
+__global__ __launch_bounds__(kThreads) void affine_fwd_grouped_kernel(RowGroup grp, int B, int H, int W, int C, int ly) {
+    const int per = B * ly;
+    const RowMember& M = grp.m[blockIdx.x / per];
+    const int rem = blockIdx.x % per;
+    const int b = rem / ly, j = rem % ly;
+    const Lanes L = make_lanes(C, VEC);
+    const int t = threadIdx.x;
+    const int tcol = t % L.colthreads, trow = t / L.colthreads;
+    if (trow >= L.rowthreads) return;
+    const T* x = (const T*)M.x;
+    T* y = (T*)M.sliced + M.off;
+    const float *A = M.c[0], *S = M.c[1];
+    const int relu = M.relu;
+    const size_t pitch = (size_t)M.pitch;
+    const size_t cbase = (size_t)(M.per_image ? b : 0) * C;
+    for (int cv = tcol; cv < L.lpr; cv += kThreads) {
+        float a[VEC], s[VEC];
+#pragma unroll
+        for (int i = 0; i < VEC; ++i) { a[i] = 1.f; s[i] = 0.f; }
+        if (A) load_coef<VEC>(A + cbase + (size_t)cv * VEC, a);
+        if (S) load_coef<VEC>(S + cbase + (size_t)cv * VEC, s);
+        for (int oh = j; oh < H; oh += ly) {
+            const size_t line = ((size_t)b * H + oh) * W;
+            const T* xl = x ? x + line * C + (size_t)cv * VEC : nullptr;
+            T* yl = y + line * pitch + (size_t)cv * VEC;
+            for (int ow0 = trow; ow0 < W; ow0 += 4 * L.rowthreads) {
+                VecT<T, VEC> xr[4];
+#pragma unroll
+                for (int u = 0; u < 4; ++u) {
+                    const int owc = min(ow0 + u * L.rowthreads, W - 1);
+                    if (xl) xr[u] = load_raw_nt<T, VEC>(xl + (size_t)owc * C);
+                }
+#pragma unroll
+                for (int u = 0; u < 4; ++u) {
+                    const int ow = ow0 + u * L.rowthreads;
+                    if (ow >= W) continue;
+                    float v[VEC];
+                    if (xl) {
+                        cvt_f<T, VEC>(xr[u], v);
+#pragma unroll
+                        for (int i = 0; i < VEC; ++i) v[i] = v[i] * a[i] + s[i];
+                    } else {
+#pragma unroll
+                        for (int i = 0; i < VEC; ++i) v[i] = s[i];
+                    }
+                    if (relu) {
+#pragma unroll
+                        for (int i = 0; i < VEC; ++i) v[i] = v[i] > 0.f ? v[i] : 0.f;
+                    }
+                    store_f<T, VEC>(yl + (size_t)ow * pitch, v);
+                }
+            }
+        }
+    }
+}
+
+template <typename T, int VEC>
+__global__ __launch_bounds__(kThreads) void affine_bwd_grouped_kernel(RowGroup grp, int B, int H, int W, int C, int ly) {
+    const int per = B * ly;
+    const RowMember& M = grp.m[blockIdx.x / per];
+    const int rem = blockIdx.x % per;
+    const int b = rem / ly, j = rem % ly;
+    const Lanes L = make_lanes(C, VEC);
+    const int t = threadIdx.x;
+    const int tcol = t % L.colthreads, trow = t / L.colthreads;
+    if (trow >= L.rowthreads) return;
+    const T* x = (const T*)M.x;
+    const T* dy = (const T*)M.sliced + M.off;
+    T* dx = (T*)M.dx;
+    const float *P = M.c[0], *Q = M.c[1], *R = M.c[2], *fA = M.c[3], *fS = M.c[4];
+    const size_t pitch = (size_t)M.pitch;
+    const size_t cbase = (size_t)(M.per_image ? b : 0) * C;
+    for (int cv = tcol; cv < L.lpr; cv += kThreads) {
+        float p[VEC], q[VEC], r[VEC], fa[VEC], fs[VEC];
+#pragma unroll
+        for (int i = 0; i < VEC; ++i) { p[i] = 1.f; q[i] = 0.f; r[i] = 0.f; fa[i] = 0.f; fs[i] = 1.f; }
+        if (P) load_coef<VEC>(P + cbase + (size_t)cv * VEC, p);
+        if (Q) load_coef<VEC>(Q + cbase + (size_t)cv * VEC, q);
+        if (R) load_coef<VEC>(R + cbase + (size_t)cv * VEC, r);
+        const bool remask = fA && x;
+        if (remask) {
+            load_coef<VEC>(fA + cbase + (size_t)cv * VEC, fa);
+            load_coef<VEC>(fS + cbase + (size_t)cv * VEC, fs);
+        }
+        const bool need_x = x && (Q || remask);
+        for (int ih = j; ih < H; ih += ly) {
+            const size_t line = ((size_t)b * H + ih) * W;
+            const size_t sl = line * C + (size_t)cv * VEC;
+            const T* dl = dy + line * pitch + (size_t)cv * VEC;
+            for (int iw0 = trow; iw0 < W; iw0 += 4 * L.rowthreads) {
+                VecT<T, VEC> dr[4], xr[4];
+#pragma unroll
+                for (int u = 0; u < 4; ++u) {
+                    const int iw = min(iw0 + u * L.rowthreads, W - 1);
+                    dr[u] = load_raw_nt<T, VEC>(dl + (size_t)iw * pitch);
+                    if (need_x) xr[u] = load_raw_nt<T, VEC>(x + sl + (size_t)iw * C);
+                }
+#pragma unroll
+                for (int u = 0; u < 4; ++u) {
+                    const int iw = iw0 + u * L.rowthreads;
+                    if (iw >= W) continue;
+                    float dv[VEC], xv[VEC], o[VEC];
+                    cvt_f<T, VEC>(dr[u], dv);
+#pragma unroll
+                    for (int i = 0; i < VEC; ++i) xv[i] = 0.f;
+                    if (need_x) cvt_f<T, VEC>(xr[u], xv);
+                    if (remask) {
+#pragma unroll
+                        for (int i = 0; i < VEC; ++i) dv[i] = (xv[i] * fa[i] + fs[i] > 0.f) ? dv[i] : 0.f;
+                    }
+#pragma unroll
+                    for (int i = 0; i < VEC; ++i) o[i] = p[i] * dv[i] + (q[i] * xv[i] + r[i]);
+                    store_f<T, VEC>(dx + sl + (size_t)iw * C, o);
+                }
             }
         }
     }
@@ -459,6 +579,26 @@
     return launch(Int<0>{});
 }
 
+static inline unsigned row_group_grid(int64_t G, int64_t B, int ly) { return (unsigned)(G * B * ly); }
+
+template <typename T>
+static int launch_affine_fwd_grouped(const RowGroup& grp, int64_t G, int64_t B, int64_t H, int64_t W, int64_t C, hipStream_t st) {
+    const int ly = lines_per_image(B, H);
+    hipLaunchKernelGGL((affine_fwd_grouped_kernel<T, FullVec<T>::value>), dim3(row_group_grid(G, B, ly)), dim3(kThreads), 0, st, grp,
+                       (int)B, (int)H, (int)W, (int)C, ly);
+    MRFP_LAUNCH_CHECK();
+    return 0;
+}
+
+template <typename T>
+static int launch_affine_bwd_grouped(const RowGroup& grp, int64_t G, int64_t B, int64_t H, int64_t W, int64_t C, hipStream_t st) {
+    const int ly = lines_per_image(B, H);
+    hipLaunchKernelGGL((affine_bwd_grouped_kernel<T, FullVec<T>::value>), dim3(row_group_grid(G, B, ly)), dim3(kThreads), 0, st, grp,
+                       (int)B, (int)H, (int)W, (int)C, ly);
+    MRFP_LAUNCH_CHECK();
+    return 0;
+}
+
 template <typename T>
 static int launch_add(const void* a, const void* b, void* y, int64_t n, hipStream_t st) {
     const int full = FullVec<T>::value;
@@ -541,6 +681,52 @@
     });
 }
 
+int mrfp_affine_fwd_grouped(const void* const* xs, void* const* ys, const int64_t* pitches, const int64_t* offsets,
+                            const float* const* As, const float* const* Ss, const int32_t* coef_per_image, const int32_t* relus, int64_t G,
+                            int dtype, int64_t B, int64_t H, int64_t W, int64_t C, void* stream) {
+    if (row_group_check("affine_fwd_grouped", dtype, G, B, H, W, C, pitches, offsets) != 0) return -1;
+    MRFP_CHECK(xs && ys && As && Ss, "affine_fwd_grouped: bad arguments");
+    RowGroup grp = {};
+    for (int64_t i = 0; i < G; ++i) {
+        MRFP_CHECK(ys[i] && (xs[i] || Ss[i]), "affine_fwd_grouped: member %lld: no y, or neither x nor S", (long long)i);
+        MRFP_CHECK(aligned16(xs[i]) && aligned16(ys[i]) && aligned16(As[i]) && aligned16(Ss[i]),
+                   "affine_fwd_grouped: member %lld: pointers must be 16-byte aligned", (long long)i);
+        RowMember& m = grp.m[i];
+        m.x = xs[i]; m.sliced = ys[i]; m.c[0] = As[i]; m.c[1] = Ss[i];
+        m.pitch = (int)pitches[i]; m.off = (int)offsets[i]; m.per_image = coef_per_image ? coef_per_image[i] : 0;
+        m.relu = relus ? relus[i] : 0;
+    }
+    hipStream_t st = (hipStream_t)stream;
+    return by_dtype(dtype, "affine_fwd_grouped", [&](auto t) {
+        using T = typename decltype(t)::type;
+        return launch_affine_fwd_grouped<T>(grp, G, B, H, W, C, st);
+    });
+}
+
+int mrfp_affine_bwd_grouped(const void* const* dys, const int64_t* pitches, const int64_t* offsets, const void* const* xs,
+                            void* const* dxs, const float* const* Ps, const float* const* Qs, const float* const* Rs,
+                            const float* const* fAs, const float* const* fSs, int64_t G, int dtype, int64_t B, int64_t H, int64_t W,
+                            int64_t C, void* stream) {
+    if (row_group_check("affine_bwd_grouped", dtype, G, B, H, W, C, pitches, offsets) != 0) return -1;
+    MRFP_CHECK(dys && xs && dxs && Ps && Qs && Rs && fAs && fSs, "affine_bwd_grouped: bad arguments");
+    RowGroup grp = {};
+    for (int64_t i = 0; i < G; ++i) {
+        MRFP_CHECK(dys[i] && dxs[i], "affine_bwd_grouped: member %lld: no dy or no dx", (long long)i);
+        MRFP_CHECK(!fAs[i] == !fSs[i], "affine_bwd_grouped: member %lld: fA and fS go together", (long long)i);
+        MRFP_CHECK(aligned16(dys[i]) && aligned16(xs[i]) && aligned16(dxs[i]) && aligned16(Ps[i]) && aligned16(Qs[i]) && aligned16(Rs[i]) &&
+                   aligned16(fAs[i]) && aligned16(fSs[i]), "affine_bwd_grouped: member %lld: pointers must be 16-byte aligned", (long long)i);
+        RowMember& m = grp.m[i];
+        m.x = xs[i]; m.sliced = const_cast<void*>(dys[i]); m.dx = dxs[i];
+        m.c[0] = Ps[i]; m.c[1] = Qs[i]; m.c[2] = Rs[i]; m.c[3] = fAs[i]; m.c[4] = fSs[i];
+        m.pitch = (int)pitches[i]; m.off = (int)offsets[i]; m.per_image = 0;
+    }
+    hipStream_t st = (hipStream_t)stream;
+    return by_dtype(dtype, "affine_bwd_grouped", [&](auto t) {
+        using T = typename decltype(t)::type;
+        return launch_affine_bwd_grouped<T>(grp, G, B, H, W, C, st);
+    });
+}
+
 int mrfp_copy_channels(const void* src, void* dst, int dtype, int64_t npix, int64_t C, int64_t ld_src, int64_t c0_src,
                        int64_t ld_dst, int64_t c0_dst, void* stream) {
     MRFP_CHECK(src && dst && npix > 0 && C > 0 && c0_src >= 0 && c0_dst >= 0 && c0_src + C <= ld_src && c0_dst + C <= ld_dst,
diff --git a/mrfp_amd/csrc/common.hpp b/mrfp_amd/csrc/common.hpp
--- a/mrfp_amd/csrc/common.hpp
+++ b/mrfp_amd/csrc/common.hpp
@@ -126,6 +126,21 @@
 
 inline bool aligned16(const void* p) { return (reinterpret_cast<uintptr_t>(p) & 15) == 0; }
 
+constexpr int kRowGroupMax = 8;
+struct RowMember {
+    const void* x;
+    void* sliced;
+    void* dx;
+    const float* c[5];
+    float* ws;
+    int pitch, off;
+    int per_image;
+    int relu;
+};
+struct RowGroup {
+    RowMember m[kRowGroupMax];
+};
+
 inline int env_switch(const char* name, int dflt) {
     const char* e = getenv(name);
     return e ? atoi(e) : dflt;
@@ -163,6 +178,22 @@
 #define MRFP_DISPATCH_VEC(T, C, ok, KERNEL, grid, st, ...) \
     MRFP_LAUNCH_VEC(pick_vec<T>(C) > 1 && (ok), (KERNEL<T, FullVec<T>::value>), (KERNEL<T, 1>), grid, st, __VA_ARGS__)
 
+inline int row_group_check(const char* who, int dtype, int64_t G, int64_t B, int64_t H, int64_t W, int64_t C, const int64_t* pitches,
+                           const int64_t* offsets) {
+    MRFP_CHECK(G >= 1 && G <= kRowGroupMax, "%s: %lld members (1..%d)", who, (long long)G, kRowGroupMax);
+    MRFP_CHECK(dtype_known(dtype), "%s: unknown dtype %d", who, dtype);
+    MRFP_CHECK(pitches && offsets && B > 0 && H > 0 && W > 0 && C > 0 && B * H < (1LL << 24) && W < (1LL << 24), "%s: bad arguments", who);
+    const int64_t vw = 16 / dtype_bytes(dtype);
+    MRFP_CHECK(C % vw == 0 && C <= 65536, "%s: C = %lld is not whole 16-byte vectors (C %% %lld)", who, (long long)C, (long long)vw);
+    for (int64_t i = 0; i < G; ++i) {
+        MRFP_CHECK(pitches[i] % vw == 0 && offsets[i] % vw == 0, "%s: member %lld: pitch %lld / offset %lld not a multiple of the vector width %lld",
+                   who, (long long)i, (long long)pitches[i], (long long)offsets[i], (long long)vw);
+        MRFP_CHECK(offsets[i] >= 0 && offsets[i] + C <= pitches[i] && pitches[i] < (1LL << 24), "%s: member %lld: channels [%lld, %lld) outside pitch %lld", who,
+                   (long long)i, (long long)offsets[i], (long long)(offsets[i] + C), (long long)pitches[i]);
+    }
+    return 0;
+}
+
 inline int lines_per_image(int64_t B, int64_t Ho) {
     static const int set = env_switch("MRFP_ROW_BLOCKS", 2048);
     const int total = set < 64 ? 2048 : set;
diff --git a/mrfp_amd/csrc/resize_pool.hip b/mrfp_amd/csrc/resize_pool.hip
--- a/mrfp_amd/csrc/resize_pool.hip
+++ b/mrfp_amd/csrc/resize_pool.hip
@@ -14,10 +14,10 @@
     return t;
 }
 
-template <typename T, int VEC>
+template <typename T, int VEC, bool PAD = false>
 __global__ __launch_bounds__(kThreads) void bilinear_fwd_kernel(const T* __restrict__ x, const T* __restrict__ addend,
                                                                 T* __restrict__ y, int B, int Hi, int Wi, int Ho, int Wo,
-                                                                int C, int ldi, int ly, int ldo) {
+                                                                int C, int ldi, int ly, int ldo, int padv) {
     const int b = blockIdx.x / ly, j = blockIdx.x % ly;
     const Lanes L = make_lanes(C, VEC);
     const int t = threadIdx.x;
@@ -62,6 +62,14 @@
                         for (int i = 0; i < VEC; ++i) o[i] += e[i];
                     }
                     store_f<T, VEC>(y + dl + (size_t)ow * ldo, o);
+                    if constexpr (PAD) {
+                        if (cv < padv) {
+                            float z[VEC];
+#pragma unroll
+                            for (int i = 0; i < VEC; ++i) z[i] = 0.f;
+                            store_f<T, VEC>(y + dl + (size_t)ow * ldo + C, z);
+                        }
+                    }
                 }
             }
         }
@@ -419,13 +427,21 @@
 
 template <typename T>
 static int do_bilinear_fwd(const void* x, const void* addend, void* y, int64_t B, int64_t Hi, int64_t Wi, int64_t Ho,
-                           int64_t Wo, int64_t C, int64_t ldi, hipStream_t st, int64_t ldo = 0) {
+                           int64_t Wo, int64_t C, int64_t ldi, hipStream_t st, int64_t ldo = 0, int64_t pad = 0) {
     const int ly = lines_per_image(B, Ho);
     if (ldo <= 0) ldo = C;
     const bool ok = aligned16(x) && aligned16(y) && (!addend || aligned16(addend)) && ldi % FullVec<T>::value == 0 &&
                     ldo % FullVec<T>::value == 0;
+    if (pad > 0) {
+        const int full = FullVec<T>::value;
+        if (!(ok && C % full == 0 && pad % full == 0 && pad <= C)) { set_error("bilinear_fwd_into_pad: whole 16-byte vectors, pad <= C"); return -1; }
+        hipLaunchKernelGGL((bilinear_fwd_kernel<T, FullVec<T>::value, true>), dim3((unsigned)(B * ly)), dim3(kThreads), 0, st, (const T*)x,
+                           (const T*)addend, (T*)y, (int)B, (int)Hi, (int)Wi, (int)Ho, (int)Wo, (int)C, (int)ldi, ly, (int)ldo, (int)(pad / full));
+        MRFP_LAUNCH_CHECK();
+        return 0;
+    }
     MRFP_DISPATCH_VEC(T, C, ok, bilinear_fwd_kernel, dim3((unsigned)(B * ly)), st, (const T*)x, (const T*)addend, (T*)y,
-                      (int)B, (int)Hi, (int)Wi, (int)Ho, (int)Wo, (int)C, (int)ldi, ly, (int)ldo);
+                      (int)B, (int)Hi, (int)Wi, (int)Ho, (int)Wo, (int)C, (int)ldi, ly, (int)ldo, 0);
     return 0;
 }
 template <typename T>
@@ -522,6 +538,15 @@
         return do_bilinear_fwd<T>(x, nullptr, y, B, Hi, Wi, Ho, Wo, C, ld_in, (hipStream_t)stream, ld_out);
     });
 }
+int mrfp_bilinear_fwd_into_pad(const void* x, void* y, int dtype, int64_t B, int64_t Hi, int64_t Wi, int64_t Ho, int64_t Wo,
+                               int64_t C, int64_t ld_in, int64_t ld_out, int64_t pad, void* stream) {
+    MRFP_CHECK(x && y && B > 0 && Hi > 0 && Wi > 0 && Ho > 0 && Wo > 0 && C > 0 && ld_in >= C && pad > 0 && ld_out >= C + pad,
+               "bilinear_fwd_into_pad: bad arguments");
+    return by_dtype(dtype, "bilinear_fwd_into_pad", [&](auto t) {
+        using T = typename decltype(t)::type;
+        return do_bilinear_fwd<T>(x, nullptr, y, B, Hi, Wi, Ho, Wo, C, ld_in, (hipStream_t)stream, ld_out, pad);
+    });
+}
 int mrfp_bilinear_bwd_from(const void* dy, void* dx, int dtype, int64_t B, int64_t Hi, int64_t Wi, int64_t Ho, int64_t Wo,
                            int64_t C, int64_t ld_in, int64_t ld_dy, void* stream) {
     MRFP_CHECK(dy && dx && B > 0 && Hi > 0 && Wi > 0 && Ho > 0 && Wo > 0 && C > 0 && ld_in >= C && ld_dy >= C, "bilinear_bwd_from: bad arguments");
diff --git a/mrfp_amd/csrc/stats.hip b/mrfp_amd/csrc/stats.hip
--- a/mrfp_amd/csrc/stats.hip
+++ b/mrfp_amd/csrc/stats.hip
@@ -149,6 +149,102 @@
         return 0;
     };
     return resize ? launch(Int<1>{}) : launch(Int<0>{});
+}
+
+template <typename T, int VEC>
+__global__ __launch_bounds__(kThreads) void stats_bwd_grouped_kernel(RowGroup grp, int B, int H, int W, int C, int ly) {
+    __shared__ float sm[kThreads * 2 * VEC];
+    const int per = B * ly;
+    const RowMember& M = grp.m[blockIdx.x / per];
+    const int rem = blockIdx.x % per;
+    const int b = rem / ly, j = rem % ly;
+    const Lanes L = make_lanes(C, VEC);
+    const int t = threadIdx.x;
+    const int tcol = t % L.colthreads, trow = t / L.colthreads;
+    const bool active = trow < L.rowthreads;
+    const T* x = (const T*)M.x;
+    const T* dy = (const T*)M.sliced + M.off;
+    const float *mean = M.c[0], *fA = M.c[1], *fS = M.c[2];
+    const size_t pitch = (size_t)M.pitch;
+    const bool plain = x == nullptr;
+    const bool remask = !plain && fA != nullptr;
+    float* out = M.ws + (size_t)rem * 2 * C;
+
+    for (int cv0 = 0; cv0 < L.lpr; cv0 += kThreads) {
+        const int cv = cv0 + tcol;
+        const bool on = active && cv < L.lpr;
+        float s[VEC], q[VEC], mu[VEC], fa[VEC], fs[VEC];
+#pragma unroll
+        for (int i = 0; i < VEC; ++i) { s[i] = 0.f; q[i] = 0.f; mu[i] = 0.f; fa[i] = 0.f; fs[i] = 1.f; }
+        if (!plain && on) {
+            const size_t co = (size_t)(M.per_image ? b : 0) * C + (size_t)cv * VEC;
+            if (mean != nullptr) {
+#pragma unroll
+                for (int i = 0; i < VEC; ++i) mu[i] = mean[co + i];
+            }
+            if (remask) {
+#pragma unroll
+                for (int i = 0; i < VEC; ++i) { fa[i] = fA[co + i]; fs[i] = fS[co + i]; }
+            }
+        }
+        if (on) {
+            for (int oh = j; oh < H; oh += ly) {
+                const size_t line = ((size_t)b * H + oh) * W;
+                const T* xl = plain ? nullptr : x + line * C + (size_t)cv * VEC;
+                const T* dl = dy + line * pitch + (size_t)cv * VEC;
+                for (int ow0 = trow; ow0 < W; ow0 += 4 * L.rowthreads) {
+                    VecT<T, VEC> xr[4], dr[4];
+#pragma unroll
+                    for (int u = 0; u < 4; ++u) {
+                        const int owc = min(ow0 + u * L.rowthreads, W - 1);
+                        dr[u] = load_raw<T, VEC>(dl + (size_t)owc * pitch);
+                        if (!plain) xr[u] = load_raw<T, VEC>(xl + (size_t)owc * C);
+                    }
+#pragma unroll
+                    for (int u = 0; u < 4; ++u) {
+                        const bool inside = ow0 + u * L.rowthreads < W;
+                        float dv[VEC];
+                        cvt_f<T, VEC>(dr[u], dv);
+                        if (plain) {
+#pragma unroll
+                            for (int i = 0; i < VEC; ++i) {
+                                const float v = inside ? dv[i] : 0.f;
+                                s[i] += v;
+                                q[i] += v * v;
+                            }
+                        } else {
+                            float xv[VEC];
+                            cvt_f<T, VEC>(xr[u], xv);
+#pragma unroll
+                            for (int i = 0; i < VEC; ++i) {
+                                const float gate = remask ? xv[i] * fa[i] + fs[i] : 1.f;
+                                const float d = (inside && gate > 0.f) ? dv[i] : 0.f;
+                                s[i] += d;
+                                q[i] += d * (xv[i] - mu[i]);
+                            }
+                        }
+                    }
+                }
+            }
+        }
+        __syncthreads();
+#pragma unroll
+        for (int i = 0; i < VEC; ++i) {
+            sm[(t * 2 + 0) * VEC + i] = s[i];
+            sm[(t * 2 + 1) * VEC + i] = q[i];
+        }
+        __syncthreads();
+        const int nout = L.colthreads * 2 * VEC;
+        for (int o = t; o < nout; o += kThreads) {
+            const int oc = o / (2 * VEC), rest = o % (2 * VEC);
+            if (cv0 + oc < L.lpr) {
+                float acc = 0.f;
+                for (int r = 0; r < L.rowthreads; ++r) acc += sm[((r * L.colthreads + oc) * 2) * VEC + rest];
+                const int stat = rest / VEC, i = rest % VEC;
+                out[(size_t)stat * C + (size_t)(cv0 + oc) * VEC + i] = acc;
+            }
+        }
+    }
 }
 
 struct Red { double s, q; };
@@ -226,6 +322,46 @@
     }
 }
 
+struct BnFinGroup {
+    const float* ws[kRowGroupMax];
+    int64_t nparts[kRowGroupMax];
+    const float* weight[kRowGroupMax];
+    const float* bias[kRowGroupMax];
+    float* running_mean[kRowGroupMax];
+    float* running_var[kRowGroupMax];
+    float* mean[kRowGroupMax];
+    float* invstd[kRowGroupMax];
+    float* A[kRowGroupMax];
+    float* S[kRowGroupMax];
+};
+__global__ void bn_finalize_grouped_kernel(BnFinGroup grp, double count, int C, float eps, float momentum) {
+    __shared__ double sm[kFL][2][kFC];
+    const int g = blockIdx.y;
+    const int c = blockIdx.x * kFC + threadIdx.x;
+    const bool valid = c < C;
+    Red r = reduce_partials(grp.ws[g], 0, grp.nparts[g], C, c, valid, sm);
+    const float *weight = grp.weight[g], *bias = grp.bias[g];
+    float *running_mean = grp.running_mean[g], *running_var = grp.running_var[g];
+    float *mean = grp.mean[g], *invstd = grp.invstd[g], *A = grp.A[g], *S = grp.S[g];
+    if (threadIdx.y == 0 && valid) {
+        const double m = r.s / count;
+        double var = r.q / count - m * m;
+        if (var < 0.0) var = 0.0;
+        const double is = 1.0 / sqrt(var + (double)eps);
+        const float w = weight ? weight[c] : 1.f, bb = bias ? bias[c] : 0.f;
+        mean[c] = (float)m;
+        invstd[c] = (float)is;
+        const float a = (float)(w * is);
+        A[c] = a;
+        S[c] = (float)(bb - m * (double)a);
+        if (running_mean) {
+            const double unb = count > 1.0 ? var * count / (count - 1.0) : var;
+            running_mean[c] = (float)((1.0 - momentum) * running_mean[c] + momentum * m);
+            running_var[c] = (float)((1.0 - momentum) * running_var[c] + momentum * unb);
+        }
+    }
+}
+
 __global__ void bn_eval_coef_kernel(int C, const float* weight, const float* bias, const float* rm, const float* rv,
                                     float eps, float* A, float* S) {
     const int c = blockIdx.x * blockDim.x + threadIdx.x;
@@ -257,6 +393,33 @@
         if (dbias) dbias[c] = (float)r.s;
         if (dweight) dweight[c] = (float)(r.q * (double)invstd[c]);
         norm_bwd_coef(r.s, r.q, count, weight ? weight[c] : 1.f, mean[c], invstd[c], P[c], Q[c], R[c]);
+    }
+}
+
+struct BnBwdFinGroup {
+    const float* ws[kRowGroupMax];
+    int64_t nparts[kRowGroupMax];
+    const float* weight[kRowGroupMax];
+    const float* mean[kRowGroupMax];
+    const float* invstd[kRowGroupMax];
+    float* dweight[kRowGroupMax];
+    float* dbias[kRowGroupMax];
+    float* P[kRowGroupMax];
+    float* Q[kRowGroupMax];
+    float* R[kRowGroupMax];
+};
+__global__ void bn_bwd_finalize_grouped_kernel(BnBwdFinGroup grp, double count, int C) {
+    __shared__ double sm[kFL][2][kFC];
+    const int g = blockIdx.y;
+    const int c = blockIdx.x * kFC + threadIdx.x;
+    const bool valid = c < C;
+    Red r = reduce_partials(grp.ws[g], 0, grp.nparts[g], C, c, valid, sm);
+    if (threadIdx.y == 0 && valid) {
+        const float* weight = grp.weight[g];
+        const float *mean = grp.mean[g], *invstd = grp.invstd[g];
+        if (grp.dbias[g]) grp.dbias[g][c] = (float)r.s;
+        if (grp.dweight[g]) grp.dweight[g][c] = (float)(r.q * (double)invstd[c]);
+        norm_bwd_coef(r.s, r.q, count, weight ? weight[c] : 1.f, mean[c], invstd[c], grp.P[g][c], grp.Q[g][c], grp.R[g][c]);
     }
 }
 
@@ -502,6 +665,72 @@
     return 0;
 }
 
+int mrfp_stats_bwd_grouped(const void* const* dys, const int64_t* pitches, const int64_t* offsets, const void* const* xs,
+                           const float* const* means, const float* const* fAs, const float* const* fSs, float* const* wss, int64_t G,
+                           int dtype, int64_t B, int64_t H, int64_t W, int64_t C, void* stream) {
+    if (row_group_check("stats_bwd_grouped", dtype, G, B, H, W, C, pitches, offsets) != 0) return -1;
+    MRFP_CHECK(dys && xs && means && fAs && fSs && wss, "stats_bwd_grouped: bad arguments");
+    RowGroup grp = {};
+    for (int64_t i = 0; i < G; ++i) {
+        MRFP_CHECK(dys[i] && wss[i], "stats_bwd_grouped: member %lld: no dy or no workspace", (long long)i);
+        MRFP_CHECK(!fAs[i] == !fSs[i], "stats_bwd_grouped: member %lld: fA and fS go together", (long long)i);
+        MRFP_CHECK(aligned16(dys[i]) && aligned16(xs[i]), "stats_bwd_grouped: member %lld: pointers must be 16-byte aligned", (long long)i);
+        RowMember& m = grp.m[i];
+        m.x = xs[i]; m.sliced = const_cast<void*>(dys[i]); m.c[0] = means[i]; m.c[1] = fAs[i]; m.c[2] = fSs[i]; m.ws = wss[i];
+        m.pitch = (int)pitches[i]; m.off = (int)offsets[i]; m.per_image = 0;
+    }
+    hipStream_t st = (hipStream_t)stream;
+    const int ly = lines_per_image(B, H);
+    return by_dtype(dtype, "stats_bwd_grouped", [&](auto t) {
+        using T = typename decltype(t)::type;
+        hipLaunchKernelGGL((stats_bwd_grouped_kernel<T, FullVec<T>::value>), dim3((unsigned)(G * B * ly)), dim3(kThreads), 0, st, grp, (int)B,
+                           (int)H, (int)W, (int)C, ly);
+        MRFP_LAUNCH_CHECK();
+        return 0;
+    });
+}
+
+int mrfp_bn_finalize_grouped(const float* const* wss, const int64_t* nparts, int64_t G, int64_t count, int64_t C,
+                             const float* const* weights, const float* const* biases, float eps, float momentum,
+                             float* const* running_means, float* const* running_vars, float* const* means, float* const* invstds,
+                             float* const* As, float* const* Ss, void* stream) {
+    MRFP_CHECK(G >= 1 && G <= mrfp::kRowGroupMax, "bn_finalize_grouped: %lld members (1..%d)", (long long)G, mrfp::kRowGroupMax);
+    MRFP_CHECK(wss && nparts && weights && biases && running_means && running_vars && means && invstds && As && Ss && C > 0 && count > 0,
+               "bn_finalize_grouped: bad arguments");
+    mrfp::BnFinGroup grp = {};
+    for (int64_t i = 0; i < G; ++i) {
+        MRFP_CHECK(wss[i] && nparts[i] > 0 && means[i] && invstds[i] && As[i] && Ss[i] && !running_means[i] == !running_vars[i],
+                   "bn_finalize_grouped: member %lld: bad arguments", (long long)i);
+        grp.ws[i] = wss[i]; grp.nparts[i] = nparts[i]; grp.weight[i] = weights[i]; grp.bias[i] = biases[i];
+        grp.running_mean[i] = running_means[i]; grp.running_var[i] = running_vars[i];
+        grp.mean[i] = means[i]; grp.invstd[i] = invstds[i]; grp.A[i] = As[i]; grp.S[i] = Ss[i];
+    }
+    hipLaunchKernelGGL(bn_finalize_grouped_kernel, dim3((unsigned)((C + mrfp::kFC - 1) / mrfp::kFC), (unsigned)G), dim3(mrfp::kFC, mrfp::kFL), 0,
+                       (hipStream_t)stream, grp, (double)count, (int)C, eps, momentum);
+    MRFP_LAUNCH_CHECK();
+    return 0;
+}
+
+int mrfp_bn_bwd_finalize_grouped(const float* const* wss, const int64_t* nparts, int64_t G, int64_t count, int64_t C,
+                                 const float* const* weights, const float* const* means, const float* const* invstds,
+                                 float* const* dweights, float* const* dbiases, float* const* Ps, float* const* Qs, float* const* Rs,
+                                 void* stream) {
+    MRFP_CHECK(G >= 1 && G <= mrfp::kRowGroupMax, "bn_bwd_finalize_grouped: %lld members (1..%d)", (long long)G, mrfp::kRowGroupMax);
+    MRFP_CHECK(wss && nparts && weights && means && invstds && dweights && dbiases && Ps && Qs && Rs && C > 0 && count > 0,
+               "bn_bwd_finalize_grouped: bad arguments");
+    mrfp::BnBwdFinGroup grp = {};
+    for (int64_t i = 0; i < G; ++i) {
+        MRFP_CHECK(wss[i] && nparts[i] > 0 && means[i] && invstds[i] && Ps[i] && Qs[i] && Rs[i], "bn_bwd_finalize_grouped: member %lld: bad arguments",
+                   (long long)i);
+        grp.ws[i] = wss[i]; grp.nparts[i] = nparts[i]; grp.weight[i] = weights[i]; grp.mean[i] = means[i]; grp.invstd[i] = invstds[i];
+        grp.dweight[i] = dweights[i]; grp.dbias[i] = dbiases[i]; grp.P[i] = Ps[i]; grp.Q[i] = Qs[i]; grp.R[i] = Rs[i];
+    }
+    hipLaunchKernelGGL(bn_bwd_finalize_grouped_kernel, dim3((unsigned)((C + mrfp::kFC - 1) / mrfp::kFC), (unsigned)G), dim3(mrfp::kFC, mrfp::kFL), 0,
+                       (hipStream_t)stream, grp, (double)count, (int)C);
+    MRFP_LAUNCH_CHECK();
+    return 0;
+}
+
 int mrfp_bn_eval_coef(int64_t C, const float* weight, const float* bias, const float* running_mean,
                       const float* running_var, float eps, float* A, float* S, void* stream) {
     MRFP_CHECK(running_mean && running_var && A && S && C > 0, "bn_eval_coef: bad arguments");
diff --git a/mrfp_amd/deepv3.py b/mrfp_amd/deepv3.py
--- a/mrfp_amd/deepv3.py
+++ b/mrfp_amd/deepv3.py
@@ -11,7 +11,7 @@
 from .conv import wgrad_boundary
 from .loss import fused_ce_kwargs, fused_loss
 from .network import Resnet
-from .network.mynn import (HipBatchNorm2d, HipConv2d, HipInstanceNorm2d, Norm2d, Upsample, conv_norm, initialize_weights,
+from .network.mynn import (HipBatchNorm2d, HipConv2d, HipInstanceNorm2d, Norm2d, Upsample, conv_norm, fold_state, initialize_weights,
                            initialize_weights_kaimingnormal_forOC)
 
 __all__ = ["_AtrousSpatialPyramidPoolingModule", "MRFPPlus", "simpleDeepV3Plus", "ReferenceRandom", "InjectedRandom"]
@@ -114,6 +114,11 @@
         return conv_norm(self[0], self[1], x, want_skip=True, relu=True)
 
 
+def _grouped_pairs(blocks, channels):
+    return ops.GROUPED_NORM[0] and all(type(f[1]) is HipBatchNorm2d and f[1].num_features == channels and not fold_state(f[0], f[1])
+                                       for f in blocks)
+
+
 class _AtrousSpatialPyramidPoolingModule(nn.Module):
 
     def __init__(self, in_dim, reduction_dim=256, output_stride=16, rates=(6, 12, 18)):
@@ -135,7 +140,17 @@
         self.img_pooling = nn.AdaptiveAvgPool2d(1)
         self.img_conv = _ConvBnRelu(in_dim, 256, 1)
 
-    def forward(self, x):
+    def forward(self, x, grouped=True):
+        C = self.img_conv[1].num_features
+        if grouped and _grouped_pairs(self.features, C):
+            raws, cur = [], x
+            for f in self.features:
+                y, cur = f[0].forward_skip(cur)
+                raws.append(y)
+            img = self.img_conv(ops.global_avg_pool(cur))
+            out = ops.empty_cl(x.shape[0], C * (1 + len(raws)), x.shape[2], x.shape[3], raws[0].dtype, x.device)
+            return ops.batch_norm_act_grouped(raws, [f[1] for f in self.features], out, [C * (1 + i) for i in range(len(raws))],
+                                              relu=True, bcast=(img, 0))
         outs, cur = [], x
         for f in self.features:
             y, cur = f.forward_skip(cur)
@@ -235,6 +250,21 @@
             return wgrad_boundary(self.layer4(t)[0])
         t = self.mod7(self.mod6(self.mod5(wgrad_boundary(self.mod4(wgrad_boundary(t))))))
         return wgrad_boundary(self.bn_out[0].fused(t, relu=True))
+
+    def _fine(self, x, want_skip=False):
+        f = self.bot_fine
+        Ca, Cb = f[1].num_features, self.bot_aspp[1].num_features
+        if self._taps is None and _grouped_pairs([f], Ca) and Ca % 8 == 0 and Cb % 8 == 0:
+            y, skip = f[0].forward_skip(x) if want_skip else (f[0](x), None)
+            buf = ops.empty_cl(x.shape[0], ops.concat_upsample_width(Ca, Cb, cfg.MODEL.DECODER_PAD), x.shape[2], x.shape[3], y.dtype, x.device)
+            fine = (ops.batch_norm_act_grouped([y], [f[1]], buf, [0], relu=True), Ca)
+            return (fine, skip) if want_skip else fine
+        return f.forward_skip(x) if want_skip else f(x)
+
+    def _decoder_cat(self, fine, up, size):
+        if isinstance(fine, tuple):
+            return ops.concat_upsample_into(fine[0], fine[1], up)
+        return ops.concat_upsample(fine, up, size, cfg.MODEL.DECODER_PAD)
 
     def _final1(self, d):
         d = conv_norm(self.final1[0], self.final1[1], d, relu=True)
@@ -384,15 +414,15 @@
         if npp:
             t = self.Normalization_Perturbation_Plus(t, "np2")
         self._tap("layer1", t)
-        dec0_fine, low_level = self.bot_fine.forward_skip(t)
+        dec0_fine, low_level = self._fine(t, want_skip=True)
         t = self._high(low_level, w_arr, fourier)
         if self.use_wtloss:
             self.w_arr = w_arr
         self._tap("layer4", t)
-        t = self.aspp(t)
+        t = self.aspp(t, grouped=self._taps is None)
         self._tap("aspp", t)
         dec0_up = self.bot_aspp(t)
-        dec1 = self._final1(ops.concat_upsample(dec0_fine, dec0_up, low_level.shape[2:], cfg.MODEL.DECODER_PAD))
+        dec1 = self._final1(self._decoder_cat(dec0_fine, dec0_up, low_level.shape[2:]))
         self._tap("dec1", dec1)
         if o2:
             if cfg.MODEL.COMMUTE_O2:
@@ -423,6 +453,6 @@
         low_level = x_tuple[0]
         x_tuple = self.layer4(self.layer3(self.layer2(x_tuple)))
         dec0_up = self.bot_aspp(self.aspp(x_tuple[0]))
-        dec0_fine = self.bot_fine(low_level)
-        dec1 = self._final1(ops.concat_upsample(dec0_fine, dec0_up, low_level.shape[2:], cfg.MODEL.DECODER_PAD))
+        dec0_fine = self._fine(low_level)
+        dec1 = self._final1(self._decoder_cat(dec0_fine, dec0_up, low_level.shape[2:]))
         return self._head(dec1, (h, w), gts, training, low_res)
diff --git a/mrfp_amd/ops.py b/mrfp_amd/ops.py
--- a/mrfp_amd/ops.py
+++ b/mrfp_amd/ops.py
@@ -1,6 +1,7 @@
 from __future__ import annotations
 
 import collections
+import ctypes
 import math
 import os
 import weakref
@@ -475,6 +476,187 @@
                                 act="relu6")
 
 
+GROUPED_NORM = [os.environ.get("MRFP_GROUPED_NORM", "1") != "0"]
+GROUPED_NORM_HITS = [0]
+GROUP_MAX = 8
+
+
+def _ptrs(ts):
+    return (ctypes.c_void_p * len(ts))(*[ptr(t) for t in ts])
+
+
+def _i64s(vals):
+    return (ctypes.c_int64 * len(vals))(*[int(v) for v in vals])
+
+
+def _i32s(vals):
+    return (ctypes.c_int32 * len(vals))(*[int(v) for v in vals])
+
+
+class _BatchNormActGrouped(torch.autograd.Function):
+
+    @staticmethod
+    def forward(ctx, out, offsets, relu, momentum, eps, running, bcast_off, *tensors):
+        G = len(offsets)
+        xs = [_chk(t) for t in tensors[:G]]
+        weights, biases = tensors[G:2 * G], tensors[2 * G:3 * G]
+        bcast = tensors[3 * G] if len(tensors) > 3 * G else None
+        B, C, H, W = xs[0].shape
+        Ct, dev, count = out.shape[1], out.device, B * H * W
+        w32, b32 = [_f32(w) for w in weights], [_f32(b) for b in biases]
+        coef = torch.empty(G, 4, C, dtype=torch.float32, device=dev)
+        wss, nparts = [], []
+        for x in xs:
+            fused = _serving_colstats(x, C, count, None, False)
+            if fused is not None:
+                wss.append(fused.final)
+                nparts.append(fused.final_count)
+            else:
+                nslab, ws = _stats_fwd(x, None)
+                wss.append(ws)
+                nparts.append(B * nslab)
+        call("mrfp_bn_finalize_grouped", _ptrs(wss), _i64s(nparts), G, count, C, _ptrs(w32), _ptrs(b32), float(eps), float(momentum),
+             _ptrs([r[0] for r in running]), _ptrs([r[1] for r in running]), _ptrs([coef[g, 0] for g in range(G)]),
+             _ptrs([coef[g, 1] for g in range(G)]), _ptrs([coef[g, 2] for g in range(G)]), _ptrs([coef[g, 3] for g in range(G)]), stream())
+        srcs, offs = list(xs), list(offsets)
+        As, Ss = [coef[g, 2] for g in range(G)], [coef[g, 3] for g in range(G)]
+        per_image, relus = [0] * G, [int(relu)] * G
+        if bcast is not None:
+            bcast = _chk(bcast, "bcast")
+            sb = bcast.detach().float().reshape(B, C).contiguous()
+            srcs.append(None); offs.append(bcast_off); As.append(None); Ss.append(sb); per_image.append(1); relus.append(0)
+        n = len(srcs)
+        call("mrfp_affine_fwd_grouped", _ptrs(srcs), _ptrs([out] * n), _i64s([Ct] * n), _i64s(offs), _ptrs(As), _ptrs(Ss), _i32s(per_image),
+             _i32s(relus), n, dt(out), B, H, W, C, stream())
+        ctx.dims = (G, B, C, H, W, Ct)
+        ctx.offsets, ctx.bcast_off, ctx.relu, ctx.has_bcast = list(offsets), bcast_off, bool(relu), bcast is not None
+        ctx.wparams, ctx.bparams = list(weights), list(biases)
+        ctx.save_for_backward(coef, *xs, *w32)
+        ctx.mark_dirty(out)
+        GROUPED_NORM_HITS[0] += 1
+        return out
+
+    @staticmethod
+    def backward(ctx, dy):
+        G, B, C, H, W, Ct = ctx.dims
+        coef, xs, w32 = ctx.saved_tensors[0], ctx.saved_tensors[1:1 + G], ctx.saved_tensors[1 + G:1 + 2 * G]
+        dy = _chk(dy, "dy")
+        dev, count = dy.device, B * H * W
+        need = ctx.needs_input_grad[7:]
+        act = [g for g in range(G) if need[g] or need[G + g] or need[2 * G + g]]
+        want_b = ctx.has_bcast and need[3 * G]
+        dxs, dws, dbs = [None] * G, [None] * G, [None] * G
+        nslab = int(_lib.lib().mrfp_stats_nslab(B, H))
+        n = len(act)
+        if n or want_b:
+            ws = torch.empty(n + 1, B * nslab * 2 * C, dtype=torch.float32, device=dev)
+            fA = [coef[g, 2] if ctx.relu else None for g in act]
+            fS = [coef[g, 3] if ctx.relu else None for g in act]
+            m = n + (1 if want_b else 0)
+            offs = [ctx.offsets[g] for g in act] + ([ctx.bcast_off] if want_b else [])
+            call("mrfp_stats_bwd_grouped", _ptrs([dy] * m), _i64s([Ct] * m), _i64s(offs), _ptrs([xs[g] for g in act] + [None] * (m - n)),
+                 _ptrs([coef[g, 0] for g in act] + [None] * (m - n)), _ptrs(fA + [None] * (m - n)), _ptrs(fS + [None] * (m - n)),
+                 _ptrs([ws[i] for i in range(m)]), m, dt(dy), B, H, W, C, stream())
+        if n:
+            outc = torch.empty(n, 5, C, dtype=torch.float32, device=dev)
+            dwd = [_grad_dest(ctx.wparams[g], need[G + g], outc[i, 0]) for i, g in enumerate(act)]
+            dbd = [_grad_dest(ctx.bparams[g], need[2 * G + g], outc[i, 1]) for i, g in enumerate(act)]
+            P, Q, R = ([outc[i, k] for i in range(n)] for k in (2, 3, 4))
+            call("mrfp_bn_bwd_finalize_grouped", _ptrs([ws[i] for i in range(n)]), _i64s([B * nslab] * n), n, count, C, _ptrs([w32[g] for g in act]),
+                 _ptrs([coef[g, 0] for g in act]), _ptrs([coef[g, 1] for g in act]), _ptrs(dwd), _ptrs(dbd), _ptrs(P), _ptrs(Q), _ptrs(R),
+                 stream())
+            dx = [empty_cl(B, C, H, W, dy.dtype, dev) for _ in act]
+            call("mrfp_affine_bwd_grouped", _ptrs([dy] * n), _i64s([Ct] * n), _i64s(offs[:n]), _ptrs([xs[g] for g in act]), _ptrs(dx), _ptrs(P),
+                 _ptrs(Q), _ptrs(R), _ptrs(fA), _ptrs(fS), n, dt(dy), B, H, W, C, stream())
+            for i, g in enumerate(act):
+                dxs[g] = dx[i] if need[g] else None
+                dws[g] = _grad_result(ctx.wparams[g], dwd[i])
+                dbs[g] = _grad_result(ctx.bparams[g], dbd[i])
+        db = None
+        if want_b:
+            db = empty_cl(B, C, 1, 1, dy.dtype, dev)
+            tmp = torch.empty(B * C, dtype=torch.float32, device=dev)
+            call("mrfp_mean_finalize", ptr(ws[n]), B, nslab, 1, C, ptr(tmp), ptr(db), dt(dy), stream())
+        return (None,) * 7 + tuple(dxs) + tuple(dws) + tuple(dbs) + ((db,) if ctx.has_bcast else ())
+
+
+class _CopyIntoSlices(torch.autograd.Function):
+
+    @staticmethod
+    def forward(ctx, out, offsets, *tensors):
+        ts = [_chk(t) for t in tensors]
+        B, Ct, H, W = out.shape
+        for t, off in zip(ts, offsets):
+            if t.shape[0] != B or tuple(t.shape[2:]) != (H, W) or t.dtype != out.dtype:
+                raise _lib.MrfpHipError("batch_norm_act_grouped: shape / dtype mismatch")
+            call("mrfp_copy_channels", ptr(t), ptr(out), dt(t), B * H * W, t.shape[1], t.shape[1], 0, Ct, off, stream())
+        ctx.offsets, ctx.Cs = list(offsets), [int(t.shape[1]) for t in ts]
+        ctx.mark_dirty(out)
+        return out
+
+    @staticmethod
+    def backward(ctx, dy):
+        dy = _chk(dy, "dy")
+        B, Ct, H, W = dy.shape
+        grads = []
+        for i, (off, C) in enumerate(zip(ctx.offsets, ctx.Cs)):
+            g = None
+            if ctx.needs_input_grad[2 + i]:
+                g = empty_cl(B, C, H, W, dy.dtype, dy.device)
+                call("mrfp_copy_channels", ptr(dy), ptr(g), dt(dy), B * H * W, C, Ct, off, C, 0, stream())
+            grads.append(g)
+        return (None, None) + tuple(grads)
+
+
+def _grouped_norm_ok(xs, bns, out, offsets, bcast):
+    if not GROUPED_NORM[0] or not 1 <= len(xs) + (bcast is not None) <= GROUP_MAX:
+        return False
+    x0 = xs[0]
+    vw = 16 // x0.element_size()
+    if out.dtype != x0.dtype or x0.shape[1] % vw or out.shape[1] % vw or any(o % vw for o in offsets):
+        return False
+    if any(tuple(x.shape) != tuple(x0.shape) or x.dtype != x0.dtype for x in xs):
+        return False
+    if any(not (bn.training or bn.running_mean is None) or (bn.momentum, bn.eps) != (bns[0].momentum, bns[0].eps) or bn.momentum is None
+           or bn.weight is None or bn.bias is None for bn in bns):
+        return False
+    if bcast is not None and (bcast[0].dtype != x0.dtype or tuple(bcast[0].shape) != (x0.shape[0], x0.shape[1], 1, 1) or bcast[1] % vw):
+        return False
+    return _sync_bn_group() is None
+
+
+def batch_norm_act_grouped(xs, bns, out, offsets, relu=True, bcast=None):
+    xs, bns, offsets = list(xs), list(bns), [int(o) for o in offsets]
+    if not (len(xs) == len(bns) == len(offsets)) or not xs:
+        raise _lib.MrfpHipError("batch_norm_act_grouped: one module and one offset per input")
+    B, Ct, H, W = out.shape
+    if out.dim() != 4 or not out.is_contiguous(memory_format=CL) or out.requires_grad:
+        raise _lib.MrfpHipError("batch_norm_act_grouped: out must be a dense NHWC buffer outside the autograd graph")
+    spans = sorted([(o, o + x.shape[1]) for o, x in zip(offsets, xs)] + ([(int(bcast[1]), int(bcast[1]) + bcast[0].shape[1])] if bcast else []))
+    if spans[0][0] < 0 or spans[-1][1] > Ct or any(a[1] > b[0] for a, b in zip(spans, spans[1:])):
+        raise _lib.MrfpHipError("batch_norm_act_grouped: slices overlap or leave the buffer (%s in %d channels)" % (spans, Ct))
+    if any(tuple(x.shape[2:]) != (H, W) or x.shape[0] != B for x in xs):
+        raise _lib.MrfpHipError("batch_norm_act_grouped: shape mismatch")
+    if not _grouped_norm_ok(xs, bns, out, offsets, bcast):
+        ys = [bn.fused(x, relu=relu) for bn, x in zip(bns, xs)]
+        offs = list(offsets)
+        if bcast is not None:
+            ys.append(upsample_bilinear(bcast[0], (H, W)))
+            offs.append(int(bcast[1]))
+        return _CopyIntoSlices.apply(out, offs, *ys)
+    running = []
+    for bn in bns:
+        track = bn.track_running_stats and bn.running_mean is not None
+        if track:
+            RUNNING_STATS_EPOCH[0] += 1
+            if bn.num_batches_tracked is not None:
+                bn._nbt_pending += 1
+        running.append((bn.running_mean, bn.running_var) if track else (None, None))
+    extra = (bcast[0],) if bcast is not None else ()
+    return _BatchNormActGrouped.apply(out, offsets, bool(relu), bns[0].momentum, bns[0].eps, running, int(bcast[1]) if bcast else 0,
+                                      *xs, *[bn.weight for bn in bns], *[bn.bias for bn in bns], *extra)
+
+
 IN_FUSED_STATS = [os.environ.get("MRFP_IN_FUSED_STATS", "1") != "0"]
 IN_FUSED_HITS = [0]
 
@@ -1369,6 +1551,53 @@
     return _ConcatUpsample.apply(a, b, int(size[0]), int(size[1]), int(pad_to))
 
 
+class _UpsampleInto(torch.autograd.Function):
+
+    @staticmethod
+    def forward(ctx, buf, b, Ca):
+        b = _chk(b)
+        B, Ct, Ho, Wo = buf.shape
+        _, Cb, Hi, Wi = b.shape
+        esz, pad = buf.element_size(), Ct - Ca - Cb
+        vw = 16 // esz
+        if pad and pad % vw == 0 and pad <= Cb and Cb % vw == 0:
+            call("mrfp_bilinear_fwd_into_pad", ptr(b), buf.data_ptr() + Ca * esz, dt(b), B, Hi, Wi, Ho, Wo, Cb, Cb, Ct, pad, stream())
+        else:
+            if pad:
+                buf.detach()[:, Ca + Cb:].zero_()
+            call("mrfp_bilinear_fwd_into", ptr(b), buf.data_ptr() + Ca * esz, dt(b), B, Hi, Wi, Ho, Wo, Cb, Cb, Ct, stream())
+        ctx.dims = (B, Ca, Cb, Hi, Wi, Ho, Wo, Ct)
+        ctx.mark_dirty(buf)
+        return buf
+
+    @staticmethod
+    def backward(ctx, dy):
+        dy = _chk(dy, "dy")
+        B, Ca, Cb, Hi, Wi, Ho, Wo, Ct = ctx.dims
+        db = None
+        if ctx.needs_input_grad[1]:
+            db = empty_cl(B, Cb, Hi, Wi, dy.dtype, dy.device)
+            call("mrfp_bilinear_bwd_from", dy.data_ptr() + Ca * dy.element_size(), ptr(db), dt(dy), B, Hi, Wi, Ho, Wo, Cb, Cb, Ct, stream())
+        return dy, db, None
+
+
+def concat_upsample_width(Ca, Cb, pad_to=1):
+    return (Ca + Cb + pad_to - 1) // pad_to * pad_to
+
+
+def concat_upsample_into(buf, Ca, b):
+    B, Ct, H, W = buf.shape
+    vw = 16 // buf.element_size()
+    if (b.shape[0] != B or b.dtype != buf.dtype or Ca + b.shape[1] > Ct or Ca % vw or b.shape[1] % vw or Ct % vw
+            or not buf.is_contiguous(memory_format=CL)):
+        raise _lib.MrfpHipError("concat_upsample_into: shape / dtype mismatch, or channel counts off the 16-byte chunk")
+    if b.shape[2] == 1 and b.shape[3] == 1:
+        if Ca + b.shape[1] != Ct:
+            buf.detach()[:, Ca + b.shape[1]:].zero_()
+        return _CopyIntoSlices.apply(buf, [int(Ca)], upsample_bilinear(b, (H, W)))
+    return _UpsampleInto.apply(buf, b, int(Ca))
+
+
 def concat_channels(tensors):
     return _ConcatChannels.apply(*tensors)
 
```

Result: slower. 304.7 images/sec (-1.2%).
